# fakufaku/diffusion-separation

Hardware: AMD Instinct MI355X
Metric: separated utterances/sec (4 s, 8 kHz, 2-spk, N=30 PC steps) (higher is better)
Workload: dtype f16; 1 GPU; configs[1]: 2-spk N=30 PC sampler (+1 ald2 corrector step), batch=16 x 4.0 s @ 8 kHz per GPU and step, NCSN++ nf=64 random-init, 60 NFE/step; 4 consecutive steps (batches) in flight per GPU; batch_per_gpu=16, samples=32000, N=30, corrector_steps=1, nf=64, graph=True, batches_in_flight=4

## Files before the change

### diffusion-separation_amd/csrc/common.h

```cpp
#pragma once
#include <hip/hip_runtime.h>
#include <stdint.h>
#include <stdio.h>

#include <string>

typedef uint16_t bf16_t;
typedef __attribute__((ext_vector_type(16))) float f32x16;
typedef __attribute__((ext_vector_type(8))) __bf16 bf16x8;

#define DS_F32 0
#define DS_BF16 1
#define DS_F32_SPLIT 2
#define DS_MAX_SRC 4

void ds_set_error(const std::string& s);
#define DS_CHECK(cond, msg)                                                            \
  do {                                                                                 \
    if (!(cond)) {                                                                     \
      ds_set_error(std::string(__FILE__) + ":" + std::to_string(__LINE__) + ": " + (msg)); \
      return 1;                                                                        \
    }                                                                                  \
  } while (0)
#define DS_HIP(expr)                                                                   \
// ... 138 lines not shown
}
__device__ inline float wave_max(float v) {
#pragma unroll
  for (int o = 32; o > 0; o >>= 1) v = fmaxf(v, __shfl_xor(v, o, 64));
  return v;
}

static inline int cdiv(long a, long b) { return (int)((a + b - 1) / b); }

struct ConvArgs {
  const void* x; long x_bs; int ldx;
  const void* x2; long x2_bs; int ldx2;
  int C1;
  const void* w; long w_bs;
  int w_chunked;
  const void* w_frag; const void* sw_frag;
  const void* ident_frag;
  const void* sx; long sx_bs; int ldsx;
  const void* sx2; long sx2_bs; int ldsx2; int sC1; int sCin;
  const void* sw; int sw_chunked;
  const float* gn_scale;
  const float* gn_shift; int gn_act;
  const float* bias;
  const float* bias_b; int bias_b_ld;
  int bias_mode;
  const float* div_b;
  const void* res; long res_bs; int ldr;
  float out_scale;
  void* y; long y_bs; int ldy;
  long long* stats_acc;
  const long long* gn_acc1; const long long* gn_acc2; const float* gn_gamma; const float* gn_beta;
  int gn_groups; float gn_inv_count; float gn_eps;
  int B, H, W;
  int Cin, Cout, taps;
  int dtype;
  int split;
  unsigned opts;
};
#define DS_OPT_NO_RW 1u
#define DS_OPT_NO_RW128 2u
#define DS_OPT_RW_SMALL 4u
#define DS_OPT_NO_RW_RES 8u
#define DS_OPT_NO_ATTN_FUSED 64u
#define DS_OPT_NO_SPLIT256 128u
#define DS_OPT_NO_STFT_FUSED 256u
#define DS_OPT_RW_QUARTER 1024u
#define DS_OPT_RW_BIG_HALF 2048u
#define DS_OPT_RW_HALF 512u
#define DS_OPT_NO_SW 4096u
#define DS_OPT_NO_SW_RW 8192u
#define DS_OPT_NO_SW_ROWS4 32768u
#define DS_OPT_SW_ROWS4 65536u
#define DS_OPT_NO_SWS 16384u
#define DS_OPT_NO_WFRAG 32u
unsigned ds_default_opts();
int ds_num_cus();
enum { DS_CLS_CONV_N64 = 0, DS_CLS_CONV_N32, DS_CLS_CONV_8X8, DS_CLS_GEMM_N64, DS_CLS_GEMM_N32, DS_CLS_GEMM_8X8, DS_CLS_WS,
       DS_CLS_SMALL, DS_CLS_RW, DS_CLS_ATTN, DS_CLS_SW, DS_CLS_SWS, DS_NCLS };
enum class ConvRoute { GENERIC, WS, THIN_IN, THIN_OUT, SMALL, RW, SW, SWS };
struct ConvPlan {
  ConvRoute route;
  int cls;
  int tile;
  int sw_rows;
  bool rw_ok;
  bool skip_ok;
};
ConvPlan ds_conv_plan(const ConvArgs& a);
int ds_launch_conv(const ConvArgs& a, hipStream_t st);
int ds_launch_conv(const ConvArgs& a, const ConvPlan& p, hipStream_t st);
const char* ds_last_conv_kernel();
void ds_set_last_conv_kernel(const char* name);
int ds_conv_chunk(int taps, int dtype);
__host__ __device__ inline long ds_rw_frag_index(int co, int tap, int ch, int taps, int Cout) {
  return (((((long)(ch / 64) * taps + tap) * 4 + (ch % 64) / 16) * (Cout / 32) + co / 32) * 64 + ((ch % 16) / 8) * 32 + co % 32) * 8 + ch % 8;
}
inline bool ds_rw_frag_shape(int taps, int Cin, int Cout) {
  return (Cout == 64 || Cout == 128) && (Cin == 64 || Cin == 128) && (taps == 1 || !(Cout == 128 && Cin == 64));
}
bool ds_conv_rw_supported(const ConvArgs& a);
int ds_launch_conv_rw(const ConvArgs& a, hipStream_t st);
inline bool ds_sw_frag_shape(int taps, int Cin, int Cout) { return (Cout == 64 || Cout == 128 || Cout == 256) && Cin % 64 == 0 && Cin >= 64 && Cin <= 512; }
bool ds_conv_sw_supported(const ConvArgs& a);
int ds_launch_conv_sw(const ConvArgs& a, int rows, hipStream_t st);
__host__ __device__ inline long ds_sws_frag_index(int co, int tap, int ch, int taps, int Cout, int plane) {
  return ((((((long)(ch / 32) * taps + tap) * 2 + (ch % 32) / 16) * 2 + plane) * (Cout / 32) + co / 32) * 64 + ((ch % 16) / 8) * 32 + co % 32) * 8 + ch % 8;
}
inline bool ds_sws_frag_shape(int taps, int Cin, int Cout) { return (Cout == 64 || Cout == 128 || Cout == 256) && Cin % 64 == 0 && Cin >= 64 && Cin <= 256; }
bool ds_conv_sws_supported(const ConvArgs& a);
int ds_launch_conv_sws(const ConvArgs& a, hipStream_t st);
bool ds_conv_ws_supported(const ConvArgs& a);
int ds_launch_conv_ws(const ConvArgs& a, hipStream_t st);
bool ds_conv_thin_in_supported(const ConvArgs& a);
int ds_launch_conv_thin_in(const ConvArgs& a, hipStream_t st);
bool ds_conv_thin_out_supported(const ConvArgs& a);
int ds_launch_conv_thin_out(const ConvArgs& a, hipStream_t st);
bool ds_conv_small_supported(const ConvArgs& a);
int ds_launch_conv_small(const ConvArgs& a, hipStream_t st);

struct AttnFusedArgs {
  const void* x; long x_bs; int ldx;
  const long long* gn_acc; const float* gn_gamma; const float* gn_beta; int gn_groups; float gn_inv_count; float gn_eps;
  const float* gn_scale; const float* gn_shift;
  const void* wqk; const void* wv; const void* wo;
  const float* bqk; const float* bv; const float* bo;
  void* y; long y_bs; int ldy;
  long long* stats;
  int B, L, C;
};
bool ds_attn_fused_eligible(int dtype, int channels, int L);
int ds_launch_attn_fused(const AttnFusedArgs& a, hipStream_t st);

long ds_gn_workspace_bytes(int B, int H, int W, int C);
int ds_launch_gn_stats(const void* x, int ldx, const void* x2, int ldx2, int C1, int B, int H, int W, int C, int groups,
                       float eps, const float* gamma, const float* beta, void* ws, float* scale, float* shift,
                       int dtype, hipStream_t st);
int ds_launch_gn_finalize_acc(const long long* a1, int C1, const long long* a2, int C2, int B, long npix, int groups,
                              float eps, const float* gamma, const float* beta, float* scale, float* shift,
                              hipStream_t st);
enum class GnRoute { APPLY = 1, BLOCK2X2, DOWN_STRIP, DOWN_TILED, UP_TILED };
struct GnPlan { GnRoute route; int rs; };
bool ds_gn_route_runs(GnRoute r, int mode, bool affine, int dtype, int H, int W, int C, int ldx, int ldy, int ldxr, bool has_xr);
GnPlan ds_gn_route(int mode, bool affine, int dtype, int B, int H, int W, int C, int ldx, int ldy, int ldxr, bool has_xr, int cus);
const char* ds_gn_kernel_name(const GnPlan& p, int mode, bool affine, int dtype);
int ds_launch_gn_apply(const void* x, int ldx, const float* scale, const float* shift, int C, void* y, int ldy,
                       void* xr, int ldxr, int B, int H, int W, int act, int mode, int dtype, hipStream_t st);
int ds_launch_gn_apply(const GnPlan& p, const void* x, int ldx, const float* scale, const float* shift, int C, void* y, int ldy,
                       void* xr, int ldxr, int B, int H, int W, int act, int mode, int dtype, hipStream_t st);
int ds_launch_concat(const void* a, int lda, int Ca, const void* b, int ldb, int Cb, void* y, int ldy, long npix,
                     int dtype, hipStream_t st);
int ds_launch_softmax(const void* x, void* y, long rows, int L, int ld, int dtype, hipStream_t st);

long ds_stft_workspace_bytes(int B, int S, long T, int n_fft, int hop);
long ds_istft_workspace_bytes(int B, int S, long T, int n_fft, int hop);
int ds_launch_stft_pack(const float* xt, const float* mix, void* y, int B, int S, long T, int n_fft, int hop,
                        float exponent, float factor, int W, int Cpad, int shift, int dtype, const float* tab,
                        float* ws, hipStream_t st, int split = 0);
int ds_launch_istft(const void* x, float* out, int B, int S, long T, int n_fft, int hop, float exponent, float factor,
                    int W, int Cpad, int dtype, const float* tab, float* ws, hipStream_t st, int split = 0,
                    const float* ow = nullptr, const float* ob = nullptr, const float* tdiv = nullptr, int ow_cin = 0);
int ds_build_stft_table(int n_fft, float** dev_tab);

struct SdeP { int kind; int ndim; float d_lambda, sigma_min, sigma_max; };
__device__ inline float sde_g_of_t(const SdeP& s, float t) {
  const float r = s.sigma_max / s.sigma_min;
  return s.sigma_min * powf(r, t) * sqrtf(2.0f * logf(r));
}
__device__ inline void mix_eig(const SdeP& s, float t, float& ev1, float& ev2) {
  const float r = s.sigma_max / s.sigma_min;
  const float logsig = logf(r);
  const float mult = s.sigma_min * s.sigma_min;
  const float srp = powf(r, 2.0f * t);
  ev1 = mult * (srp - 1.0f);
  const float ex = expf(-2.0f * s.d_lambda * t);
  const float denom = 1.0f + s.d_lambda / logsig;
  ev2 = mult * (srp - ex) / denom;
}
__device__ inline void philox_round(uint32_t& c0, uint32_t& c1, uint32_t& c2, uint32_t& c3, uint32_t k0, uint32_t k1) {
  const uint64_t p0 = (uint64_t)0xD2511F53u * c0;
  const uint64_t p1 = (uint64_t)0xCD9E8D57u * c2;
  const uint32_t n0 = (uint32_t)(p1 >> 32) ^ c1 ^ k0;
  const uint32_t n1 = (uint32_t)p1;
  const uint32_t n2 = (uint32_t)(p0 >> 32) ^ c3 ^ k1;
  const uint32_t n3 = (uint32_t)p0;
  c0 = n0; c1 = n1; c2 = n2; c3 = n3;
}
__device__ inline void philox_randn4(uint64_t q, uint64_t seed, uint64_t sid, float* v) {
  uint32_t c0 = (uint32_t)q, c1 = (uint32_t)(q >> 32), c2 = (uint32_t)sid, c3 = (uint32_t)(sid >> 32);
  uint32_t k0 = (uint32_t)seed, k1 = (uint32_t)(seed >> 32);
#pragma unroll
  for (int r = 0; r < 10; ++r) {
    philox_round(c0, c1, c2, c3, k0, k1);
    k0 += 0x9E3779B9u;
    k1 += 0xBB67AE85u;
  }
  const float u0 = ((float)(c0 >> 8) + 0.5f) * (1.0f / 16777216.0f);
  const float u1 = ((float)(c1 >> 8) + 0.5f) * (1.0f / 16777216.0f);
  const float u2 = ((float)(c2 >> 8) + 0.5f) * (1.0f / 16777216.0f);
  const float u3 = ((float)(c3 >> 8) + 0.5f) * (1.0f / 16777216.0f);
  const float r0 = sqrtf(-2.0f * logf(u0)), r1 = sqrtf(-2.0f * logf(u2));
  sincosf(6.28318530718f * u1, &v[1], &v[0]);
// ... 62 lines not shown
```

### diffusion-separation_amd/csrc/engine.hip

```cpp
#include "engine_host.h"

static thread_local std::string g_err;
void ds_set_error(const std::string& s) { g_err = s; }
extern "C" const char* diffsep_last_error(void) { return g_err.c_str(); }
extern "C" const char* diffsep_version(void) {
#ifdef DS_HALF_F16
    return "diffsep-hip 0.3 (gfx950, 16-bit storage f16)";
#else
    return "diffsep-hip 0.3 (gfx950, 16-bit storage bf16)";
#endif
}

static const struct { const char* name; const char* env; unsigned bit; } kOpts[] = {
    {"no_rw", "DIFFSEP_NO_RW", DS_OPT_NO_RW},
    {"no_rw128", "DIFFSEP_NO_RW128", DS_OPT_NO_RW128},
    {"rw_small", "DIFFSEP_RW_SMALL", DS_OPT_RW_SMALL},
    {"no_rw_res", "DIFFSEP_NO_RW_RES", DS_OPT_NO_RW_RES},
    {"no_wfrag", nullptr, DS_OPT_NO_WFRAG},
    {"no_attn_fused", nullptr, DS_OPT_NO_ATTN_FUSED},
    {"no_stft_fused", "DIFFSEP_NO_STFT_FUSED", DS_OPT_NO_STFT_FUSED},
    {"rw_half", "DIFFSEP_RW_HALF", DS_OPT_RW_HALF},
    {"rw_quarter", "DIFFSEP_RW_QUARTER", DS_OPT_RW_QUARTER},
    {"rw_big_half", "DIFFSEP_RW_BIG_HALF", DS_OPT_RW_BIG_HALF},
    {"no_split256", nullptr, DS_OPT_NO_SPLIT256},
    {"no_sw", "DIFFSEP_NO_SW", DS_OPT_NO_SW},
    {"no_sws", "DIFFSEP_NO_SWS", DS_OPT_NO_SWS},
    {"no_sw_rows4", "DIFFSEP_NO_SW_ROWS4", DS_OPT_NO_SW_ROWS4},
    {"sw_rows4", nullptr, DS_OPT_SW_ROWS4},
    {"no_sw_rw", "DIFFSEP_NO_SW_RW", DS_OPT_NO_SW_RW}};
static std::atomic<unsigned> g_opts{0};
static std::once_flag g_opts_once;
unsigned ds_default_opts() {
  std::call_once(g_opts_once, [] {
    for (const auto& o : kOpts) {
      const char* v = o.env ? getenv(o.env) : nullptr;
      if (v && *v && strcmp(v, "0") != 0) g_opts |= o.bit;
    }
  });
  return g_opts;
}
int ds_num_cus() {
  static std::atomic<int> cus[32];
  int dev = 0;
  if (hipGetDevice(&dev) != hipSuccess || dev < 0 || dev >= 32) dev = 0;
  int c = cus[dev].load(std::memory_order_relaxed);
  if (c <= 0) {
    hipDeviceProp_t prop;
    c = hipGetDeviceProperties(&prop, dev) == hipSuccess ? prop.multiProcessorCount : 0;
    if (c <= 0) c = 256;
    cus[dev].store(c, std::memory_order_relaxed);
  }
  return c;
}
static int opt_bit(const char* name, unsigned* bit) {
  for (const auto& o : kOpts)
    if (!strcmp(name, o.name)) { *bit = o.bit; return 0; }
  return 1;
}
extern "C" int32_t diffsep_set_option(const char* name, int64_t value) {
  DS_CHECK(name, "set_option: null name");
  unsigned bit = 0;
  if (opt_bit(name, &bit)) { ds_set_error(std::string("set_option: unknown option '") + name + "'"); return 1; }
  ds_default_opts();
  if (value) g_opts.fetch_or(bit); else g_opts.fetch_and(~bit);
  return 0;
}

static Tn cat_view(const Tn& a, const Tn& b) {
  Tn t = a;
  t.C = a.C + b.C; t.C1 = a.C; t.p2 = b.p; t.ld2 = b.ld;
  t.sa2 = b.sa;
  return t;
}

static void* e_alloc(diffsep_engine* e, size_t bytes) {
  const size_t a = (e->top + 255) & ~(size_t)255;
  e->top = a + bytes;
  if (e->dry) return (void*)(uintptr_t)(a + 256);
  if (e->dbg_alloc) fprintf(stderr, "[diffsep alloc] %zu %zu\n", a, bytes);
  return e->arena + a;
}
static long long* e_alloc_stats(diffsep_engine* e, size_t bytes) {
// ... 90 lines not shown
  DS_CHECK(!a.sx || p.skip_ok, "internal: fused skip conv on an unsupported tile");
  if (c.want_stats && e->dbg_alloc && !e->dry)
    fprintf(stderr, "[diffsep stats] %ld Cin %d Cout %d taps %d HxW %dx%d res %d skip %d bias_b %d cfg %d\n",
            (long)((char*)y.sa - e->stats_ptr), a.Cin, c.Cout, c.taps, a.H, a.W, c.res != nullptr, c.skip != nullptr,
            c.bias_b != nullptr, p.cls);
  if (e->dry || ablated(e, a.H)) return 0;
  if (!e->prof) return ds_launch_conv(a, p, st);
  diffsep_engine::ProfRec r;
  r.flops = 2.0 * ((double)a.taps * a.Cin + (a.sx ? a.sCin : 0)) * a.Cout * (double)a.H * a.W * a.B;
  {
    const double esz = a.dtype == DS_F32 ? 4.0 : 2.0;
    r.bytes = esz * ((double)a.B * a.H * a.W *
                         ((double)a.Cin + a.Cout + (a.res ? a.Cout : 0) + (a.sx ? a.sCin : 0)) +
                     ((double)a.taps * a.Cin + (a.sx ? a.sCin : 0)) * a.Cout);
  }
  r.cls = p.cls;
  r.B = a.B; r.H = a.H; r.W = a.W; r.Cin = a.Cin; r.Cout = a.Cout; r.taps = a.taps; r.sCin = a.sx ? a.sCin : 0; r.res = a.res != nullptr;
  const int rc = prof_launch(e, st, r, [&]() { return ds_launch_conv(a, p, st); });
  e->prof_recs.back().kernel = ds_last_conv_kernel();
  return rc;
}

static int gn_stats(diffsep_engine* e, const Tn& x, const float* gamma, const float* beta, int B, GnAff& aff,
                    hipStream_t st, bool lazy = false) {
  const int groups = gn_group_count(x.C);
  aff = GnAff();
  const bool have_acc = x.sa && (!x.p2 || x.sa2);
  if (have_acc && lazy && x.C <= 512) {
    aff.acc1 = x.sa; aff.acc2 = x.sa2; aff.gamma = gamma; aff.beta = beta; aff.groups = groups;
    aff.inv_count = gn_inv_count((long)x.H * x.W, x.C, groups);
    return 0;
  }
  aff.scale = e_f32(e, (size_t)B * x.C);
  aff.shift = e_f32(e, (size_t)B * x.C);
  if (have_acc) {
    if (e->dry || (e->ablate & 16u)) return 0;
    return ds_launch_gn_finalize_acc(x.sa, x.p2 ? x.C1 : x.C, x.sa2, x.p2 ? x.C - x.C1 : 0, B, (long)x.H * x.W, groups,
                                     1e-6f, gamma, beta, aff.scale, aff.shift, st);
  }
  void* ws = e_alloc(e, (size_t)ds_gn_workspace_bytes(B, x.H, x.W, x.C));
  if (e->dry) return 0;
  return ds_launch_gn_stats(x.p, x.ld, x.p2, x.ld2, x.C1, B, x.H, x.W, x.C, groups, 1e-6f, gamma, beta, ws, aff.scale,
                            aff.shift, e->cfg.dtype, st);
}
static int gn_apply(diffsep_engine* e, const Tn& x, const GnAff* aff, const Tn* y, const Tn* xr, int B, int act,
                    int mode, hipStream_t st) {
  if (e->dry || (e->ablate & 8u)) return 0;
  const double esz = e->cfg.dtype == DS_F32 ? 4.0 : 2.0, nin = (double)B * x.H * x.W * x.C;
  const double fo = mode == 1 ? 4.0 : (mode == 2 ? 0.25 : 1.0);
  const double bytes = esz * nin * (1.0 + fo * ((y ? 1 : 0) + (xr ? 1 : 0)));
  const char* name = mode == 1 ? (aff ? "gn_fir_up (GroupNorm + SiLU + FIR x2 up of act and raw)" : "fir_up (pyramid)")
                               : (mode == 2 ? (aff ? "gn_fir_down (GroupNorm + SiLU + FIR x2 down of act and raw)" : "fir_down (pyramid)")
                                            : "gn_apply (GroupNorm affine + SiLU)");
  return prof_launch(e, st, hbm_rec(name, bytes, B, x.H, x.W, x.C), [&]() {
    return ds_launch_gn_apply(x.p, x.ld, aff ? aff->scale : nullptr, aff ? aff->shift : nullptr, x.C, y ? y->p : nullptr,
                              y ? y->ld : 0, xr ? xr->p : nullptr, xr ? xr->ld : 0, B, x.H, x.W, act, mode, e->cfg.dtype,
                              st);
  });
}

static const float kInvSqrt2 = 0.70710678118654752440f;

static int conv1_folded_skip(diffsep_engine* e, const Module& m, const Tn& h1, const Tn& skip_src, const GnAff& a1, Tn& out,
                             int B, hipStream_t st) {
  const SkipConv sk = {&skip_src, PK(e, m.pk2), weight_chunk(9, m.in_ch, m.in_c1, e->cfg.dtype), PKF(e, m.pf2)};
  Conv c(h1, PK(e, m.pk1), m.out_ch, 9);
  c.w_frag = PKF(e, m.pf1); c.gn = &a1; c.skip = &sk; c.scale = kInvSqrt2; c.want_stats = true;
  c.bias = P(e, m.conv1_b); c.bias_b = P(e, m.conv2_b);
  return conv(e, c, out, B, st);
}

int res_block(diffsep_engine* e, const Module& m, const Tn& x, const float* temb_proj, int B, Tn& out,
              hipStream_t st) {
  DS_CHECK(x.C == m.in_ch, "internal: resblock channel mismatch");
  const int mode = m.up ? 1 : (m.down ? 2 : 0);
  const int Ho = m.up ? 2 * x.H : (m.down ? x.H / 2 : x.H);
  const int Wo = m.up ? 2 * x.W : (m.down ? x.W / 2 : x.W);
  GnAff a0, a1;
  const float* temb = temb_proj + m.temb_off;
  if (e->cfg.dtype == DS_BF16 && mode == 0 && x.p2 && m.pf0a >= 0 && x.C1 == 128 && x.sa && x.sa2 &&
      x.H >= ((e->opts & DS_OPT_NO_SW) ? 128 : 256) && !(e->opts & (DS_OPT_NO_SPLIT256 | DS_OPT_NO_WFRAG))) {
    Tn xa = x, xb = x;
    xa.C = 128; xa.p2 = nullptr; xa.C1 = 0; xa.ld2 = 0; xa.sa2 = nullptr;
    xb.p = x.p2; xb.ld = x.ld2; xb.C = 128; xb.p2 = nullptr; xb.C1 = 0; xb.ld2 = 0; xb.sa = x.sa2; xb.sa2 = nullptr;
    GnAff ga, gb;
    ga.acc1 = xa.sa; ga.gamma = P(e, m.gn0_w); ga.beta = P(e, m.gn0_b);
    ga.groups = gn_group_count(x.C) / 2;
    ga.inv_count = gn_inv_count((long)x.H * x.W, x.C, gn_group_count(x.C));
    gb = ga; gb.acc1 = xb.sa; gb.gamma = ga.gamma + 128; gb.beta = ga.beta + 128;
    Conv c0a(xa, PK(e, m.pk0), m.out_ch, 9);
    c0a.w_frag = PKF(e, m.pf0a); c0a.gn = &ga; c0a.bias = P(e, m.conv0_b); c0a.bias_b = temb; c0a.bias_b_ld = e->arch.dense_total;
    Tn h1p; h1p.C = h1p.ld = m.out_ch; h1p.H = Ho; h1p.W = Wo;
    ConvArgs half = conv_args(e, c0a, h1p, B); half.opts &= ~DS_OPT_RW_SMALL;
    if (ds_conv_plan(half).rw_ok) {
      h1p = e_tensor(e, B, Ho, Wo, m.out_ch);
      Tn h1 = e_tensor(e, B, Ho, Wo, m.out_ch);
      const long half0 = 4L * 9 * m.out_ch * 32;
      if (conv(e, c0a, h1p, B, st)) return 1;
      Conv c0b(xb, PK(e, m.pk0 + half0), m.out_ch, 9);
      c0b.w_frag = PKF(e, m.pf0b); c0b.gn = &gb; c0b.res = &h1p; c0b.want_stats = true;
      if (conv(e, c0b, h1, B, st)) return 1;
      if (gn_stats(e, h1, P(e, m.gn1_w), P(e, m.gn1_b), B, a1, st, true)) return 1;
      out = e_tensor(e, B, Ho, Wo, m.out_ch);
      if (!(e->opts & DS_OPT_NO_SW) && m.pf2 >= 0) return conv1_folded_skip(e, m, h1, x, a1, out, B, st);
      Tn outp = e_tensor(e, B, Ho, Wo, m.out_ch);
      const SkipConv sk = {&xa, PK(e, m.pk2), weight_chunk(9, 128, 0, e->cfg.dtype), PKF(e, m.pf2a)};
      Conv c1(h1, PK(e, m.pk1), m.out_ch, 9);
      c1.w_frag = PKF(e, m.pf1); c1.gn = &a1; c1.skip = &sk; c1.bias = P(e, m.conv1_b); c1.bias_b = P(e, m.conv2_b);
      if (conv(e, c1, outp, B, st)) return 1;
      Conv c2b(xb, PK(e, m.pk2b), m.out_ch, 1);
      c2b.res = &outp; c2b.scale = kInvSqrt2; c2b.want_stats = true;
      return conv(e, c2b, out, B, st);
    }
  }
  if (gn_stats(e, x, P(e, m.gn0_w), P(e, m.gn0_b), B, a0, st, mode == 0)) return 1;
  Tn h1 = e_tensor(e, B, Ho, Wo, m.out_ch);
  Tn xr = x, h0m;
  if (mode) {
    DS_CHECK(x.p2 == nullptr, "internal: resampling block on a concat view");
    h0m = e_tensor(e, B, Ho, Wo, m.in_ch);
    xr = e_tensor(e, B, Ho, Wo, m.in_ch);
    if (gn_apply(e, x, &a0, &h0m, &xr, B, 1, mode, st)) return 1;
  }
  if (!m.has_conv2) DS_CHECK(xr.p2 == nullptr, "internal: identity skip on a concat view");
  Conv c0(mode ? h0m : x, PK(e, m.pk0), m.out_ch, 9);
  c0.w_frag = PKF(e, m.pf0); c0.gn = mode ? nullptr : &a0; c0.want_stats = true;
  c0.bias = P(e, m.conv0_b); c0.bias_b = temb; c0.bias_b_ld = e->arch.dense_total;
  if (conv(e, c0, h1, B, st)) return 1;
  if (gn_stats(e, h1, P(e, m.gn1_w), P(e, m.gn1_b), B, a1, st, true)) return 1;
  out = e_tensor(e, B, Ho, Wo, m.out_ch);
  if (m.has_conv2 && fuse_skip(m)) return conv1_folded_skip(e, m, h1, xr, a1, out, B, st);
  Tn skip = xr;
  if (m.has_conv2) {
    skip = e_tensor(e, B, Ho, Wo, m.out_ch);
    Conv c2(xr, PK(e, m.pk2), m.out_ch, 1);
    c2.bias = P(e, m.conv2_b);
    if (conv(e, c2, skip, B, st)) return 1;
  }
  Conv c1(h1, PK(e, m.pk1), m.out_ch, 9);
  c1.w_frag = PKF(e, m.pf1); c1.ident_frag = m.has_conv2 ? nullptr : PKF(e, m.pf_id);
  c1.gn = &a1; c1.bias = P(e, m.conv1_b); c1.res = &skip; c1.scale = kInvSqrt2; c1.want_stats = true;
  return conv(e, c1, out, B, st);
}

int attention_core(const Tn& q, const void* k, const void* vt, const Tn& o, int B, void* scores, void* probs, int dtype,
                   hipStream_t st, int split) {
  const int L = q.W, C = q.C, Lp = rup8(L);
  Tn s = q, p = q;
  s.p = scores; p.p = probs; s.ld = p.ld = Lp; p.C = Lp;
  ConvArgs a;
  memset(&a, 0, sizeof(a));
  a.dtype = dtype; a.split = split; a.B = B; a.taps = 1; a.bias_mode = 0;
  conv_input(a, q);
  a.w = k; a.w_bs = (long)L * C;
  conv_output(a, s);
  a.Cout = L;
  a.out_scale = 1.0f / sqrtf((float)C);
  if (ds_launch_conv(a, st)) return 1;
  if (ds_launch_softmax(scores, probs, (long)B * L, L, Lp, dtype, st)) return 1;
  conv_input(a, p);
  a.w = vt; a.w_bs = (long)C * Lp;
  conv_output(a, o);
  a.Cout = C;
  a.out_scale = 1.f;
  return ds_launch_conv(a, st);
}

int attn_block(diffsep_engine* e, const Module& m, const Tn& x, int B, Tn& out, hipStream_t st) {
// ... 19 lines not shown
    diffsep_engine::ProfRec r;
    r.flops = (double)B * (6.0 * L * C * C + 4.0 * (double)L * L * C);
    r.bytes = (double)e->esz * (2.0 * B * L * C + 3.0 * C * C);
    r.cls = DS_CLS_ATTN; r.B = B; r.H = x.H; r.W = x.W; r.Cin = C; r.Cout = C; r.taps = 1; r.res = 1;
    r.kernel = "attn_fused_kernel";
    return prof_launch(e, st, r, [&]() { return ds_launch_attn_fused(a, st); });
  }
  GnAff a0;
  if (gn_stats(e, x, P(e, m.gn0_w), P(e, m.gn0_b), B, a0, st)) return 1;
  Tn h = e_tensor(e, B, x.H, x.W, C);
  if (gn_apply(e, x, &a0, &h, nullptr, B, 0, 0, st)) return 1;
  Tn q = e_tensor(e, B, x.H, x.W, C), k = e_tensor(e, B, x.H, x.W, C);
  Conv cq(h, PK(e, m.pk_nin[0]), C, 1), ck(h, PK(e, m.pk_nin[1]), C, 1);
  cq.bias = P(e, m.nin_b[0]); ck.bias = P(e, m.nin_b[1]);
  if (conv(e, cq, q, B, st) || conv(e, ck, k, B, st)) return 1;
  void* vt = e_alloc(e, (size_t)B * C * Lp * e->esz);
  void* scores = e_alloc(e, (size_t)B * L * Lp * e->esz);
  void* probs = e_alloc(e, (size_t)B * L * Lp * e->esz);
  Tn o = e_tensor(e, B, x.H, x.W, C);
  out = e_tensor(e, B, x.H, x.W, C);
  if (!e->dry && !ablated(e, x.H)) {
    Tn wv, vtn;
    wv.p = const_cast<void*>(PK(e, m.pk_nin[2])); wv.C = wv.ld = C; wv.H = 1; wv.W = C;
    vtn.p = vt; vtn.ld = Lp; vtn.H = 1; vtn.W = C;
    ConvArgs a;
    memset(&a, 0, sizeof(a));
    a.dtype = e->cfg.dtype; a.split = e->split; a.B = B; a.taps = 1; a.out_scale = 1.f;
    conv_input(a, wv);
    a.x_bs = 0;
    a.w = h.p; a.w_bs = (long)L * C;
    a.bias = P(e, m.nin_b[2]); a.bias_mode = 1;
    conv_output(a, vtn);
    a.Cout = L;
    if (ds_launch_conv(a, st)) return 1;
    Tn qv = q, ov = o;
    qv.H = ov.H = 1; qv.W = ov.W = L;
    if (attention_core(qv, k.p, vt, ov, B, scores, probs, e->cfg.dtype, st, e->split)) return 1;
  }
  Conv co(o, PK(e, m.pk_nin[3]), C, 1);
  co.bias = P(e, m.nin_b[3]); co.res = &x; co.scale = kInvSqrt2; co.want_stats = true;
  return conv(e, co, out, B, st);
}

static int net_forward(diffsep_engine* e, const Tn& x0, const float* t, const Tn& y, int B, hipStream_t st,
                       Tn* pyr_out = nullptr) {
  const Arch& A = e->arch;
  const diffsep_model_config& c = e->cfg;
  const int nf = c.nf;
  size_t mi = 0;
  float* emb = e_f32(e, (size_t)B * 2 * nf);
  float* t1 = e_f32(e, (size_t)B * 4 * nf);
  float* temb = e_f32(e, (size_t)B * 4 * nf);
  float* proj = e_f32(e, (size_t)B * A.dense_total);
  const Module& mf = A.mods[mi++];
  const Module& l1 = A.mods[mi++];
  const Module& l2 = A.mods[mi++];
  if (!e->dry) {
    if (ds_launch_fourier(t, P(e, mf.w0), emb, B, nf, st)) return 1;
    if (ds_launch_linear(emb, P(e, l1.w0), P(e, l1.b0), t1, B, 2 * nf, 4 * nf, 0, st)) return 1;
    if (ds_launch_linear(t1, P(e, l2.w0), P(e, l2.b0), temb, B, 4 * nf, 4 * nf, 1, st)) return 1;
    if (ds_launch_linear_t(temb, e->d_dense_w, e->d_dense_b, proj, B, 4 * nf, A.dense_total, 1, st)) return 1;
  }
  const Module& cin = A.mods[mi++];
  std::vector<Tn> hs;
  {
    Tn h = e_tensor(e, B, x0.H, x0.W, nf);
    Conv ci(x0, PK(e, cin.pk0), nf, 9);
    ci.bias = P(e, cin.b0); ci.want_stats = true;
    if (conv(e, ci, h, B, st)) return 1;
    hs.push_back(h);
  }
  Tn pyr_in = x0;
  const int L = c.n_levels;
  Tn h;
  for (int i = 0; i < L; ++i) {
    for (int k = 0; k < c.num_res_blocks; ++k) {
      if (res_block(e, A.mods[mi++], hs.back(), proj, B, h, st)) return 1;
      if (h.H == c.attn_resolution) {
        DS_CHECK(mi < A.mods.size() && A.mods[mi].kind == MK_ATTN, "attention placement mismatch (image height)");
        Tn ha;
        if (attn_block(e, A.mods[mi++], h, B, ha, st)) return 1;
        h = ha;
      }
      hs.push_back(h);
    }
    if (i != L - 1) {
      if (res_block(e, A.mods[mi++], hs.back(), proj, B, h, st)) return 1;
      Tn pd = e_tensor(e, B, pyr_in.H / 2, pyr_in.W / 2, pyr_in.C);
      if (gn_apply(e, pyr_in, nullptr, nullptr, &pd, B, 0, 2, st)) return 1;
      pyr_in = pd;
      const Module& cm = A.mods[mi++];
      DS_CHECK(cm.kind == MK_COMBINE, "internal: expected Combine");
      Tn hc = e_tensor(e, B, h.H, h.W, h.C);
      Conv cc(pyr_in, PK(e, cm.pk0), h.C, 1);
      cc.bias = P(e, cm.b0); cc.res = &h; cc.want_stats = true;
      if (conv(e, cc, hc, B, st)) return 1;
      hs.push_back(hc);
    }
  }
  h = hs.back();
  Tn t2;
  if (res_block(e, A.mods[mi++], h, proj, B, t2, st)) return 1;
  if (attn_block(e, A.mods[mi++], t2, B, h, st)) return 1;
  if (res_block(e, A.mods[mi++], h, proj, B, t2, st)) return 1;
  h = t2;

  Tn pyramid;
  bool have_pyr = false;
  for (int i = L - 1; i >= 0; --i) {
    for (int k = 0; k < c.num_res_blocks + 1; ++k) {
      const Tn s = hs.back();
      hs.pop_back();
      const Tn cat = cat_view(h, s);
      Tn hn2;
      if (res_block(e, A.mods[mi++], cat, proj, B, hn2, st)) return 1;
      h = hn2;
    }
    if (h.H == c.attn_resolution) {
      DS_CHECK(mi < A.mods.size() && A.mods[mi].kind == MK_ATTN, "attention placement mismatch (image height)");
      Tn ha;
      if (attn_block(e, A.mods[mi++], h, B, ha, st)) return 1;
      h = ha;
    }
    const Module& g = A.mods[mi++];
    const Module& cv = A.mods[mi++];
    DS_CHECK(g.kind == MK_GN && cv.kind == MK_CONV3, "internal: expected pyramid GN + conv");
    hipStream_t sp = st;
    GnAff ga;
    if (gn_stats(e, h, P(e, g.w0), P(e, g.b0), B, ga, sp, true)) return 1;
    Tn pnew = e_tensor(e, B, h.H, h.W, A.cpad_in);
    Conv cp(h, PK(e, cv.pk0), A.chan_in, 9);
    cp.bias = P(e, cv.b0); cp.gn = &ga;
    Tn pu;
    if (have_pyr) {
      pu = e_tensor(e, B, h.H, h.W, A.cpad_in);
      if (gn_apply(e, pyramid, nullptr, nullptr, &pu, B, 0, 1, sp)) return 1;
      cp.res = &pu;
    }
    if (conv(e, cp, pnew, B, sp)) return 1;
    pyramid = pnew;
    have_pyr = true;
    if (i != 0) {
      Tn hu;
      if (res_block(e, A.mods[mi++], h, proj, B, hu, st)) return 1;
      h = hu;
    }
  }
  DS_CHECK(hs.empty() && mi == A.mods.size(), "internal: module walk did not consume all modules");
  if (pyr_out) { *pyr_out = pyramid; return 0; }
  Tn yy = y;
  Conv co(pyramid, PK(e, A.pk_out), A.chan_out, 1);
  co.bias = P(e, A.out_b); co.div_b = t;
  return conv(e, co, yy, B, st);
}

static int score_forward_impl(diffsep_engine* e, const float* xt, const float* t, const float* mix, float* out, int B,
                              long T, hipStream_t st) {
  const diffsep_model_config& c = e->cfg;
  const int W = diffsep_padded_frames(&c, T), H = c.n_fft / 2 + 1, S = c.num_sources;
  e->top = e->fwd_base;
  e->tracked.clear();
  if (stats_begin(e, st)) return 1;
  Tn x0 = e_tensor(e, B, H, W, e->arch.cpad_in);
  Tn y = e_tensor(e, B, H, W, e->arch.cpad_out);
  const int dft_split = e->split || c.dtype == DS_BF16;
  float* ws_f = (float*)e_alloc(e, (size_t)ds_stft_workspace_bytes(B, S, T, c.n_fft, c.hop));
  float* frames = (float*)e_alloc(e, (size_t)ds_istft_workspace_bytes(B, S, T, c.n_fft, c.hop));
  const double esz_t = c.dtype == DS_F32 ? 4.0 : 2.0;
  if (!e->dry && !(e->ablate & 128u))
    if (prof_launch(e, st, hbm_rec("stft (frame + real-DFT GEMM + compress / pack)",
                                   4.0 * B * (S + 1) * (double)T + esz_t * B * H * (double)W * e->arch.cpad_in, B, H, W, e->arch.cpad_in), [&]() {
          return ds_launch_stft_pack(xt, mix, x0.p, B, S, T, c.n_fft, c.hop, c.spec_abs_exponent, c.spec_factor, W,
                                     e->arch.cpad_in, 1, c.dtype, e->d_tab, ws_f, st, dft_split);
        }))
      return 1;
  Tn pyr;
  if (net_forward(e, x0, t, y, B, st, &pyr)) return 1;
  if (!e->dry && !(e->ablate & 128u))
    if (prof_launch(e, st, hbm_rec("istft (unpack / decompress + inverse-DFT GEMM + overlap-add)",
                                   esz_t * B * H * (double)W * pyr.ld + 4.0 * B * S * (double)T, B, H, W, pyr.ld), [&]() {
          return ds_launch_istft(pyr.p, out, B, S, T, c.n_fft, c.hop, c.spec_abs_exponent, c.spec_factor, W, pyr.ld, c.dtype,
                                 e->d_tab, frames, st, dft_split, P(e, e->arch.out_w), P(e, e->arch.out_b), t, e->arch.chan_in);
        }))
      return 1;
  return 0;
}

static void destroy_graph(diffsep_engine::GraphRec& r) {
  if (r.x) hipGraphExecDestroy(r.x);
  if (r.g) hipGraphDestroy(r.g);
  r.x = nullptr; r.g = nullptr;
}
static void drop_graph(diffsep_engine* e) {
  for (auto& kv : e->graphs) destroy_graph(kv.second);
  e->graphs.clear();
  e->cur_graph = nullptr;
}

static void layout_state(diffsep_engine* e, int B, long T) {
  const size_t nst = (size_t)B * e->cfg.num_sources * T;
  e->top = 0;
  e->st_x = (float*)e_alloc(e, nst * 4);
  e->st_xm = (float*)e_alloc(e, nst * 4);
  e->st_score = (float*)e_alloc(e, nst * 4);
  e->st_noise = (float*)e_alloc(e, nst * 4);
  e->st_t = (float*)e_alloc(e, (size_t)B * 4);
  e->st_mix = (float*)e_alloc(e, (size_t)B * T * 4);
  e->st_smix = (float*)e_alloc(e, (size_t)B * T * 4);
  e->st_ts = (float*)e_alloc(e, 4096 * (size_t)B * 4);
  e->st_lang = (float*)e_alloc(e, 16 * (size_t)B + 64);
  e->st_lens = (int*)e_alloc(e, (size_t)B * 4);
  e->st_seeds = (unsigned long long*)e_alloc(e, (size_t)B * 8);
}

int ensure_plan(diffsep_engine* e, int B, long T, hipStream_t st) {
  if (e->planB == B && e->planT == T && e->arena) return 0;
  DS_CHECK(B >= 1 && T >= 1, "empty batch or signal");
  e->cur_graph = nullptr;
  e->planB = -1;
  e->planT = -1;
  e->dry = true;
  layout_state(e, B, T);
  e->fwd_base = (e->top + 255) & ~(size_t)255;
  const int rc = score_forward_impl(e, nullptr, nullptr, nullptr, nullptr, B, T, st);
  e->dry = false;
  if (rc) return 1;
  const size_t need = e->top + e->stats_need + 8192;
  if (need > e->cap) {
    DS_HIP(hipStreamSynchronize(st));
    drop_graph(e);
    if (e->arena) DS_HIP(hipFree(e->arena));
    e->tracked.clear();
    e->arena = nullptr;
    e->cap = 0;
    const size_t grown = e->had_arena ? need + need / 4 : need;
    DS_HIP(hipMalloc((void**)&e->arena, grown));
    e->cap = grown;
    e->had_arena = true;
  }
  DS_HIP(hipMemsetAsync(e->arena, 0, e->cap, st));
  layout_state(e, B, T);
  e->planB = B;
  e->planT = T;
  {
    auto it = e->graphs.find(std::make_pair(B, T));
    if (it != e->graphs.end()) {
      e->cur_graph = &it->second;
      it->second.used = ++e->graph_tick;
    }
  }
  e->ts_dev.clear();
  e->warmed = true;
  return 0;
}

int run_nfe(diffsep_engine* e, int B, long T, hipStream_t st) {
  if (e->use_graph && e->warmed && !e->prof) {
    if (!e->cur_graph) {
      DS_HIP(hipStreamBeginCapture(st, hipStreamCaptureModeThreadLocal));
      const int rc = score_forward_impl(e, e->st_x, e->st_t, e->st_mix, e->st_score, B, T, st);
      diffsep_engine::GraphRec r{nullptr, nullptr, 0};
      const hipError_t ce = hipStreamEndCapture(st, &r.g);
      if (rc || ce != hipSuccess || !r.g) {
        destroy_graph(r);
        e->use_graph = 0;
        if (rc) return 1;
      } else {
        const hipError_t ie = hipGraphInstantiate(&r.x, r.g, nullptr, nullptr, 0);
        if (ie != hipSuccess) destroy_graph(r);
        DS_HIP(ie);
        if ((int)e->graphs.size() >= e->graph_cap) {
          const hipError_t se = hipDeviceSynchronize();
          if (se != hipSuccess) destroy_graph(r);
          DS_HIP(se);
          while ((int)e->graphs.size() >= e->graph_cap) {
            auto lru = e->graphs.begin();
            for (auto it = e->graphs.begin(); it != e->graphs.end(); ++it)
              if (it->second.used < lru->second.used) lru = it;
            destroy_graph(lru->second);
            e->graphs.erase(lru);
          }
        }
        r.used = ++e->graph_tick;
        e->cur_graph = &(e->graphs[std::make_pair(B, (long)T)] = r);
      }
    }
    if (e->cur_graph) {
      DS_HIP(hipGraphLaunch(e->cur_graph->x, st));
      return 0;
    }
  }
  const int rc = score_forward_impl(e, e->st_x, e->st_t, e->st_mix, e->st_score, B, T, st);
  e->warmed = true;
  return rc;
}

extern "C" int32_t diffsep_engine_create(const diffsep_model_config* cfg, const float* weights_host, int64_t n_floats,
                                         diffsep_engine** out) {
  DS_CHECK(cfg && weights_host && out, "engine_create: null argument");
  DS_CHECK(cfg->dtype == DS_F32 || cfg->dtype == DS_BF16 || cfg->dtype == DS_F32_SPLIT,
           "engine_create: dtype must be DIFFSEP_F32, DIFFSEP_BF16 or DIFFSEP_F32_SPLIT");
  std::unique_ptr<diffsep_engine> e(new diffsep_engine());
  e->cfg = *cfg;
  const DtypeSplit ds = split_dtype(cfg->dtype);
  e->cfg.dtype = ds.dtype; e->split = ds.split;
  if (build_arch(e->cfg, e->arch, e->cfg.dtype == DS_BF16 ? 1 : (e->split ? 2 : 0))) return 1;
  const Arch& A = e->arch;
  if (upload_weights(e.get(), weights_host, n_floats, "engine_create: weight blob")) return 1;
  e->weight_bytes = (int64_t)A.total * 4 + (int64_t)A.pack_total * e->esz + (int64_t)A.dense_total * (4 * cfg->nf + 1) * 4;
  if (ds_build_stft_table(cfg->n_fft, &e->d_tab)) return 1;
  if (const char* sv = getenv("DIFFSEP_DBG_ALLOC")) e->dbg_alloc = atoi(sv) != 0;
  e->opts = ds_default_opts();
  DS_HIP(hipEventCreateWithFlags(&e->ev_in, hipEventDisableTiming));
  DS_HIP(hipEventCreateWithFlags(&e->ev_out, hipEventDisableTiming));
  *out = e.release();
  return 0;
}

diffsep_engine::~diffsep_engine() {
  drop_graph(this);
  hipFree(d_blob); hipFree(d_pack); hipFree(d_dense_w); hipFree(d_dense_b); hipFree(d_attn_b); hipFree(d_tab);
  hipFree(arena); hipFree(ode_buf);
  if (own) hipStreamDestroy(own);
  if (ev_in) hipEventDestroy(ev_in);
  if (ev_out) hipEventDestroy(ev_out);
  for (auto& r : prof_recs) { hipEventDestroy(r.a); hipEventDestroy(r.b); }
  for (hipEvent_t v : ev_pool) hipEventDestroy(v);
}
extern "C" void diffsep_engine_destroy(diffsep_engine* e) { delete e; }
extern "C" int32_t diffsep_engine_reserve(diffsep_engine* e, int32_t B, int64_t T, void* stream) {
  DS_CHECK(e && B >= 1 && T >= 1, "reserve: bad argument");
  hipStream_t st = (hipStream_t)stream;
  if (ensure_plan(e, B, T, st)) return 1;
  DS_HIP(hipStreamSynchronize(st));
  return 0;
}
__global__ __launch_bounds__(256) void absmax_kernel(const void* __restrict__ p, long n, int f32, unsigned* __restrict__ out) {
  float m = 0.f;
  unsigned bad = 0;
  for (long i = (long)blockIdx.x * 256 + threadIdx.x; i < n; i += (long)gridDim.x * 256) {
    const float v = f32 ? reinterpret_cast<const float*>(p)[i] : h2f(reinterpret_cast<const bf16_t*>(p)[i]);
    if (v != v || fabsf(v) > 3.0e38f) ++bad; else m = fmaxf(m, fabsf(v));
  }
  atomicMax(out, __float_as_uint(m));
  if (bad) atomicAdd(out + 1, bad);
}
extern "C" int32_t diffsep_engine_debug_absmax(diffsep_engine* e, double* out, int32_t cap, int32_t* n) {
  DS_CHECK(e && n, "debug_absmax: null argument");
  *n = (int32_t)e->tracked.size();
  if (!out || cap <= 0) return 0;
  const int cnt = *n < cap ? *n : cap;
  unsigned* d = nullptr;
  DS_HIP(hipMalloc(&d, (size_t)cnt * 8 + 8));
  DS_HIP(hipMemset(d, 0, (size_t)cnt * 8 + 8));
  for (int i = 0; i < cnt; ++i) {
    const auto& t = e->tracked[i];
    long nb = (t.n + 255) / 256;
    if (nb > 1024) nb = 1024;
    hipLaunchKernelGGL(absmax_kernel, dim3((unsigned)nb), dim3(256), 0, nullptr, t.p, t.n, e->cfg.dtype == DS_F32 ? 1 : 0, d + 2 * i);
  }
  std::vector<unsigned> hbuf((size_t)cnt * 2);
  DS_HIP(hipDeviceSynchronize());
  DS_HIP(hipMemcpy(hbuf.data(), d, (size_t)cnt * 8, hipMemcpyDeviceToHost));
  hipFree(d);
  for (int i = 0; i < cnt; ++i) {
    float m;
    memcpy(&m, &hbuf[2 * i], 4);
    out[4 * i] = m; out[4 * i + 1] = hbuf[2 * i + 1]; out[4 * i + 2] = e->tracked[i].H; out[4 * i + 3] = e->tracked[i].C;
  }
  return 0;
}
extern "C" int32_t diffsep_engine_debug_arena(const diffsep_engine* e, void** base, int64_t* bytes, int64_t* fwd_base) {
  DS_CHECK(e && base && bytes && fwd_base, "debug_arena: null argument");
  *base = e->arena; *bytes = (int64_t)e->cap; *fwd_base = (int64_t)e->fwd_base;
  return 0;
}
extern "C" int64_t diffsep_engine_device_bytes(const diffsep_engine* e) {
  return e ? e->weight_bytes + (int64_t)e->cap + (int64_t)e->ode_cap : 0;
}
extern "C" int32_t diffsep_engine_set_graph(diffsep_engine* e, int32_t enable) {
  DS_CHECK(e, "null engine");
  e->use_graph = enable;
  if (!enable) drop_graph(e);
  return 0;
}

extern "C" int32_t diffsep_engine_set_option(diffsep_engine* e, const char* name, int64_t value) {
  DS_CHECK(e && name, "engine_set_option: null argument");
  unsigned bit = 0;
  if (!strcmp(name, "graph_cache")) {
    DS_CHECK(value >= 1 && value <= 4096, "engine_set_option: graph_cache must be in [1, 4096]");
    e->graph_cap = (int)value;
  } else if (!strcmp(name, "ablate")) {
    e->ablate = (unsigned)value;
  } else if (!strcmp(name, "dbg_alloc")) {
    e->dbg_alloc = value != 0;
    return 0;
  } else if (!strcmp(name, "no_stft_fused")) {
    ds_set_error("engine_set_option: 'no_stft_fused' is a process-level option (diffsep_set_option / DIFFSEP_NO_STFT_FUSED)");
    return 1;
  } else if (!strcmp(name, "track_tensors")) {
    e->track_tensors = value != 0;
    e->tracked.clear();
    return 0;
  } else if (!opt_bit(name, &bit)) {
    e->opts = value ? (e->opts | bit) : (e->opts & ~bit);
  } else {
    ds_set_error(std::string("engine_set_option: unknown option '") + name + "'");
    return 1;
  }
  DS_HIP(hipDeviceSynchronize());
  drop_graph(e);
  e->planB = -1;
  e->planT = -1;
  return 0;
}
extern "C" int64_t diffsep_engine_get_option(const diffsep_engine* e, const char* name) {
  if (!e || !name) return -1;
  unsigned bit = 0;
  if (!strcmp(name, "graph_cache")) return e->graph_cap;
  if (!strcmp(name, "graphs_cached")) return (int64_t)e->graphs.size();
  if (!strcmp(name, "ablate")) return e->ablate;
  if (!opt_bit(name, &bit)) return (e->opts & bit) ? 1 : 0;
  return -1;
}

extern "C" int32_t diffsep_engine_profile_begin(diffsep_engine* e) {
  DS_CHECK(e, "null engine");
  e->prof = true;
  e->prof_recs.clear();
  return 0;
}
static_assert(DS_NCLS == DIFFSEP_NUM_KERNEL_CLASSES, "header and engine agree on the number of kernel classes");
extern "C" int32_t diffsep_num_kernel_classes(void) { return DS_NCLS; }
extern "C" int32_t diffsep_engine_profile_end(diffsep_engine* e, double* flops, double* ms, int64_t* launches,
                                               double* bytes) {
  return diffsep_engine_profile_end_n(e, DS_NCLS, flops, ms, launches, bytes, nullptr);
}
extern "C" int32_t diffsep_engine_profile_end_n(diffsep_engine* e, int32_t n_classes, double* flops, double* ms,
                                                 int64_t* launches, double* bytes, int32_t* n_written) {
  DS_CHECK(e && flops && ms && launches && n_classes >= 0, "profile_end: null argument");
  DS_HIP(hipDeviceSynchronize());
  const int ncls = n_classes < DS_NCLS ? n_classes : DS_NCLS;
  if (n_written) *n_written = ncls;
  for (int i = 0; i < ncls; ++i) { flops[i] = 0; ms[i] = 0; launches[i] = 0; if (bytes) bytes[i] = 0; }
  e->prof_done.clear();
  for (auto& r : e->prof_recs) {
    float t = 0.f;
    hipEventElapsedTime(&t, r.a, r.b);
    r.ms = t;
    e->prof_done.push_back(r);
    if (r.cls >= 0 && r.cls < ncls) {
      flops[r.cls] += r.flops;
      if (bytes) bytes[r.cls] += r.bytes;
      ms[r.cls] += t;
      launches[r.cls] += 1;
    }
    e->ev_pool.push_back(r.a);
    e->ev_pool.push_back(r.b);
  }
  e->prof_recs.clear();
  e->prof = false;
  return 0;
}

extern "C" int32_t diffsep_engine_profile_records(diffsep_engine* e, diffsep_prof_record* out, int32_t cap, int32_t* n) {
  DS_CHECK(e && n, "profile_records: null argument");
  *n = (int32_t)e->prof_done.size();
  if (!out) return 0;
  for (int i = 0; i < *n && i < cap; ++i) {
    const auto& r = e->prof_done[i];
    diffsep_prof_record& o = out[i];
    memset(&o, 0, sizeof(o));
    snprintf(o.kernel, sizeof(o.kernel), "%s", r.kernel ? r.kernel : "");
    o.B = r.B; o.H = r.H; o.W = r.W; o.Cin = r.Cin; o.Cout = r.Cout; o.taps = r.taps; o.skip_cin = r.sCin; o.has_res = r.res;
// ... 38 lines not shown
```

### diffusion-separation_amd/csrc/engine_host.h

```cpp
#pragma once
#include <math.h>
#include <stdlib.h>
#include <string.h>

#include <atomic>
#include <map>
#include <memory>
#include <mutex>
#include <string>
#include <utility>
#include <vector>

#include "../../include/diffsep_hip.h"
#include "common.h"

#pragma GCC visibility push(hidden)

struct PRef { long off = -1; long numel = 0; };
struct ParamInfo { std::string name; int ndim; int64_t shape[4]; long off; };

enum ModKind { MK_FOURIER, MK_LINEAR, MK_CONV3, MK_RES, MK_ATTN, MK_COMBINE, MK_GN };

struct Module {
  ModKind kind;
// ... 172 lines not shown
}
static inline void conv_residual(ConvArgs& a, const Tn& r) { a.res = r.p; a.res_bs = image_bs(r, r.ld); a.ldr = r.ld; }
static inline void conv_output(ConvArgs& a, const Tn& y) { a.y = y.p; a.y_bs = image_bs(y, y.ld); a.ldy = y.ld; }

struct PinnedStage {
  char* p = nullptr;
  size_t cap = 0;
  hipEvent_t ev = nullptr;
  bool rec = false;
  PinnedStage() = default;
  PinnedStage(const PinnedStage&) = delete;
  ~PinnedStage() { if (ev) hipEventDestroy(ev); if (p) hipHostFree(p); }
  int wait() { if (rec) DS_HIP(hipEventSynchronize(ev)); return 0; }
  template <typename T>
  int acquire(size_t n, T** out) {
    if (wait()) return 1;
    if (n > cap) {
      if (p) DS_HIP(hipHostFree(p));
      p = nullptr;
      cap = 0;
      const size_t grown = n < 4096 ? 4096 : n;
      DS_HIP(hipHostMalloc((void**)&p, grown * sizeof(T), hipHostMallocDefault));
      cap = grown;
    }
    if (!ev) DS_HIP(hipEventCreateWithFlags(&ev, hipEventDisableTiming));
    *out = reinterpret_cast<T*>(p);
    return 0;
  }
  int record(hipStream_t st) { DS_HIP(hipEventRecord(ev, st)); rec = true; return 0; }
};

struct diffsep_engine {
  diffsep_engine() = default;
  diffsep_engine(const diffsep_engine&) = delete;
  ~diffsep_engine();
  diffsep_model_config cfg;
  Arch arch;
  int esz = 4;
  float* d_blob = nullptr;
  char* d_pack = nullptr;
  float* d_dense_w = nullptr;
  float* d_dense_b = nullptr;
  float* d_attn_b = nullptr;
  float* d_tab = nullptr;
  char* arena = nullptr;
  size_t cap = 0, top = 0, fwd_base = 0;
  size_t stats_need = 0, stats_used = 0;
  char* stats_ptr = nullptr;
  bool dry = false;
  int planB = -1;
  long planT = -1;
  float *st_x = nullptr, *st_xm = nullptr, *st_score = nullptr, *st_t = nullptr, *st_noise = nullptr,
        *st_ts = nullptr, *st_mix = nullptr, *st_smix = nullptr, *st_lang = nullptr;
  int* st_lens = nullptr;
  unsigned long long* st_seeds = nullptr;
  PinnedStage ext_pin;
  struct GraphRec { hipGraph_t g; hipGraphExec_t x; uint64_t used; };
  std::map<std::pair<int, long>, GraphRec> graphs;
  GraphRec* cur_graph = nullptr;
  int graph_cap = 12;
  uint64_t graph_tick = 0;
  int use_graph = 1;
  unsigned opts = 0;
  unsigned ablate = 0;
  bool warmed = false;
  int64_t weight_bytes = 0;
  hipStream_t own = nullptr;
  hipEvent_t ev_in = nullptr, ev_out = nullptr;
  PinnedStage ts_pin;
  std::vector<float> ts_dev;
  int ts_B = 0;
  bool had_arena = false;
  bool dbg_alloc = false;
  bool track_tensors = false;
  struct Tracked { void* p; long n; int H, W, C; };
  std::vector<Tracked> tracked;
  int split = 0;
  bool prof = false;
  struct ProfRec {
    hipEvent_t a = nullptr, b = nullptr; double flops = 0.0, bytes = 0.0; int cls = -1; const char* kernel = nullptr;
    int B = 0, H = 0, W = 0, Cin = 0, Cout = 0, taps = 0, sCin = 0, res = 0; float ms = 0.f;
  };
  std::vector<ProfRec> prof_done;
  std::vector<ProfRec> prof_recs;
  std::vector<hipEvent_t> ev_pool;
  char* ode_buf = nullptr;
  size_t ode_cap = 0;
  PinnedStage ode_pin;
};

static inline hipEvent_t prof_event(diffsep_engine* e) {
  if (!e->ev_pool.empty()) { hipEvent_t v = e->ev_pool.back(); e->ev_pool.pop_back(); return v; }
  hipEvent_t v = nullptr;
  hipEventCreate(&v);
  return v;
}
template <typename F>
static int prof_launch(diffsep_engine* e, hipStream_t st, diffsep_engine::ProfRec r, F&& body) {
  if (!e->prof) return body();
  r.a = prof_event(e); r.b = prof_event(e);
  hipEventRecord(r.a, st);
  const int rc = body();
  hipEventRecord(r.b, st);
  e->prof_recs.push_back(r);
  return rc;
}
static inline diffsep_engine::ProfRec hbm_rec(const char* name, double bytes, int B, int H, int W, int C) {
  diffsep_engine::ProfRec r;
  r.kernel = name; r.bytes = bytes; r.B = B; r.H = H; r.W = W; r.Cin = C;
  return r;
}

struct StreamScope {
  diffsep_engine* e; hipStream_t user; hipStream_t st;
  StreamScope(diffsep_engine* e_, void* s) : e(e_), user((hipStream_t)s), st((hipStream_t)s) {
    if (!user) {
      if (!e->own) hipStreamCreateWithFlags(&e->own, hipStreamNonBlocking);
      st = e->own;
      hipEventRecord(e->ev_in, nullptr);
      hipStreamWaitEvent(st, e->ev_in, 0);
    }
  }
  ~StreamScope() {
    if (!user) {
      hipEventRecord(e->ev_out, st);
      hipStreamWaitEvent(nullptr, e->ev_out, 0);
    }
  }
};

int upload_weights(diffsep_engine* e, const float* weights_host, int64_t n_floats, const char* what);
float* e_f32(diffsep_engine* e, size_t n);
int stats_begin(diffsep_engine* e, hipStream_t st);
int res_block(diffsep_engine* e, const Module& m, const Tn& x, const float* temb_proj, int B, Tn& out, hipStream_t st);
int attn_block(diffsep_engine* e, const Module& m, const Tn& x, int B, Tn& out, hipStream_t st);
int attention_core(const Tn& q, const void* k, const void* vt, const Tn& o, int B, void* scores, void* probs, int dtype,
                   hipStream_t st, int split = 0);
int ensure_plan(diffsep_engine* e, int B, long T, hipStream_t st);
int run_nfe(diffsep_engine* e, int B, long T, hipStream_t st);
int ds_launch_mask_tail(float* v, int B, int rows, long T, const int* lens, hipStream_t st);

#pragma GCC visibility pop
```

### diffusion-separation_amd/csrc/norm.hip

```cpp
#include <stdlib.h>

#include "conv_device.h"

template <typename T>
__global__ __launch_bounds__(256) void gn_stats_kernel(const T* __restrict__ x, int ldx, const T* __restrict__ x2,
                                                       int ldx2, int C1, long npix, int C, long ppb,
                                                       double* __restrict__ part) {
  __shared__ double sh[4096];
  const int ncg = C >> 3;
  const int npl = 256 / ncg;
  const int tid = threadIdx.x;
  const int cg = tid % ncg, pl = tid / ncg;
  const int b = blockIdx.y;
  const long p0 = (long)blockIdx.x * ppb;
  long p1 = p0 + ppb;
  if (p1 > npix) p1 = npix;
  double s[8], ss[8];
#pragma unroll
  for (int j = 0; j < 8; ++j) { s[j] = 0.0; ss[j] = 0.0; }
  if (pl < npl) {
    const bool second = x2 != nullptr && cg * 8 >= C1;
    const int ld = second ? ldx2 : ldx;
    const T* xb = second ? x2 + (long)b * npix * ldx2 + (cg * 8 - C1) : x + (long)b * npix * ldx + cg * 8;
    for (long p = p0 + pl; p < p1; p += npl) {
// ... 86 lines not shown
    if (var < 0.0) var = 0.0;
    const float sc = (float)(1.0 / sqrt(var + (double)eps)) * (gamma ? gamma[c] : 1.f);
    scale[(long)b * C + c] = sc;
    shift[(long)b * C + c] = (beta ? beta[c] : 0.f) - (float)mean * sc;
  }
}

int ds_launch_gn_finalize_acc(const long long* a1, int C1, const long long* a2, int C2, int B, long npix, int groups,
                              float eps, const float* gamma, const float* beta, float* scale, float* shift,
                              hipStream_t st) {
  const int C = C1 + C2;
  DS_CHECK(C % groups == 0 && groups > 0, "groupnorm(acc): bad group count");
  const double inv_count = (double)(float)(1.0 / ((double)npix * (double)(C / groups)));
  hipLaunchKernelGGL(gn_finalize_acc_kernel, dim3(B), dim3(256), 0, st, a1, C1, a2, C2, groups, inv_count, eps, gamma,
                     beta, scale, shift);
  DS_LAUNCH_CHECK();
  return 0;
}

long ds_gn_workspace_bytes(int B, int H, int W, int C) {
  const long npix = (long)H * W;
  long nblk = cdiv(npix, 64);
  if (nblk > 64) nblk = 64;
  return (long)B * nblk * C * 2 * 8 + 256;
}

int ds_launch_gn_stats(const void* x, int ldx, const void* x2, int ldx2, int C1, int B, int H, int W, int C, int groups,
                       float eps, const float* gamma, const float* beta, void* ws, float* scale, float* shift,
                       int dtype, hipStream_t st) {
  DS_CHECK(!x2 || (C1 % 8 == 0 && C1 > 0 && C1 < C), "groupnorm: bad concat split");
  DS_CHECK(C % 8 == 0 && C <= 1024 && C >= 8, "groupnorm: C must be a multiple of 8 in [8,1024]");
  DS_CHECK(groups > 0 && groups <= 256 && C % groups == 0, "groupnorm: bad group count");
  DS_CHECK((C >> 3) <= 256, "groupnorm: C too large");
  const long npix = (long)H * W;
  long nblk = cdiv(npix, 64);
  if (nblk > 64) nblk = 64;
  const long ppb = (npix + nblk - 1) / nblk;
  double* part = reinterpret_cast<double*>(ws);
  dim3 grid((unsigned)nblk, (unsigned)B);
  if (dtype == DS_F32)
    hipLaunchKernelGGL(gn_stats_kernel<float>, grid, dim3(256), 0, st, (const float*)x, ldx, (const float*)x2, ldx2,
                       C1, npix, C, ppb, part);
  else
    hipLaunchKernelGGL(gn_stats_kernel<bf16_t>, grid, dim3(256), 0, st, (const bf16_t*)x, ldx, (const bf16_t*)x2, ldx2,
                       C1, npix, C, ppb, part);
  DS_LAUNCH_CHECK();
  const double count = (double)npix * (double)(C / groups);
  hipLaunchKernelGGL(gn_finalize_kernel, dim3(B), dim3(256), 0, st, part, (int)nblk, C, groups, count, eps, gamma, beta,
                     scale, shift);
  DS_LAUNCH_CHECK();
  return 0;
}

template <typename T, int MODE, bool AFFINE>
__global__ __launch_bounds__(256) void gn_apply_kernel(const T* __restrict__ x, int ldx,
                                                       const float* __restrict__ scale,
                                                       const float* __restrict__ shift, int C, T* __restrict__ y,
                                                       int ldy, T* __restrict__ xr, int ldxr, int B, int H, int W,
                                                       int act) {
  const int Ho = MODE == 1 ? 2 * H : (MODE == 2 ? H / 2 : H);
  const int Wo = MODE == 1 ? 2 * W : (MODE == 2 ? W / 2 : W);
  const int ncg = C >> 3;
  const long total = (long)B * Ho * Wo * ncg;
  for (long i = (long)blockIdx.x * 256 + threadIdx.x; i < total; i += (long)gridDim.x * 256) {
    const int cg = (int)(i % ncg);
    long r = i / ncg;
    const int ox = (int)(r % Wo);
    r /= Wo;
    const int oy = (int)(r % Ho);
    const int b = (int)(r / Ho);
    float sc[8], sf[8];
    if (AFFINE) {
#pragma unroll
      for (int j = 0; j < 8; ++j) {
        sc[j] = scale[(long)b * C + cg * 8 + j];
        sf[j] = shift[(long)b * C + cg * 8 + j];
      }
    }
    const T* xb = x + (long)b * H * W * ldx + cg * 8;
    float ah[8], ax[8];
#pragma unroll
    for (int j = 0; j < 8; ++j) { ah[j] = 0.f; ax[j] = 0.f; }
    if (MODE == 0) {
      float f[8];
      load8<T>(xb + ((long)oy * W + ox) * ldx, f);
#pragma unroll
      for (int j = 0; j < 8; ++j) {
        float v = f[j] * sc[j] + sf[j];
        ah[j] = act ? silu_t<T>(v) : v;
      }
    } else {
      constexpr int NT = MODE == 2 ? 4 : 2;
      int iy0, ix0;
      float wy[4], wx[4];
      if (MODE == 2) {
        iy0 = 2 * oy - 1; ix0 = 2 * ox - 1;
        wy[0] = wx[0] = 0.125f; wy[1] = wx[1] = 0.375f; wy[2] = wx[2] = 0.375f; wy[3] = wx[3] = 0.125f;
      } else {
        const int ay = oy & 1, axp = ox & 1;
        iy0 = (oy >> 1) - 1 + ay; ix0 = (ox >> 1) - 1 + axp;
        wy[0] = ay ? 0.75f : 0.25f; wy[1] = ay ? 0.25f : 0.75f;
        wx[0] = axp ? 0.75f : 0.25f; wx[1] = axp ? 0.25f : 0.75f;
        wy[2] = wy[3] = wx[2] = wx[3] = 0.f;
      }
#pragma unroll
      for (int a = 0; a < NT; ++a) {
        const int iy = iy0 + a;
        if (iy < 0 || iy >= H) continue;
#pragma unroll
        for (int c = 0; c < NT; ++c) {
          const int ix = ix0 + c;
          if (ix < 0 || ix >= W) continue;
          const float wgt = wy[a] * wx[c];
          float f[8];
          load8<T>(xb + ((long)iy * W + ix) * ldx, f);
#pragma unroll
          for (int j = 0; j < 8; ++j) {
            ax[j] += wgt * f[j];
            if (AFFINE) {
              float v = f[j] * sc[j] + sf[j];
              v = act ? silu_t<T>(v) : v;
              ah[j] += wgt * v;
            }
          }
        }
      }
    }
    const long opix = ((long)b * Ho + oy) * Wo + ox;
    if (AFFINE) store8<T>(y + opix * ldy + cg * 8, ah);
    if (MODE != 0 && xr) store8<T>(xr + opix * ldxr + cg * 8, ax);
  }
}

template <typename T, int MODE>
__global__ __launch_bounds__(256) void gn_resample2x2_kernel(const T* __restrict__ x, int ldx,
                                                             const float* __restrict__ scale,
                                                             const float* __restrict__ shift, int C, T* __restrict__ y,
                                                             int ldy, T* __restrict__ xr, int ldxr, int B, int H, int W,
                                                             int act) {
  constexpr int NR = MODE == 1 ? 3 : 6;
  const int Hb = MODE == 1 ? H : H / 4, Wb = MODE == 1 ? W : W / 4;
  const int Ho = MODE == 1 ? 2 * H : H / 2, Wo = MODE == 1 ? 2 * W : W / 2;
  const int ncg = C >> 3;
  const long total = (long)B * Hb * Wb * ncg;
  for (long i = (long)blockIdx.x * 256 + threadIdx.x; i < total; i += (long)gridDim.x * 256) {
    const int cg = (int)(i % ncg);
    long r = i / ncg;
    const int bx = (int)(r % Wb);
    r /= Wb;
    const int by = (int)(r % Hb);
    const int b = (int)(r / Hb);
    float sc[8], sf[8];
#pragma unroll
    for (int j = 0; j < 8; ++j) {
      sc[j] = scale[(long)b * C + cg * 8 + j];
      sf[j] = shift[(long)b * C + cg * 8 + j];
    }
    const T* xb = x + (long)b * H * W * ldx + cg * 8;
    const int iy0 = MODE == 1 ? by - 1 : 4 * by - 1, ix0 = MODE == 1 ? bx - 1 : 4 * bx - 1;
    float oh[2][2][8], ox[2][2][8];
#pragma unroll
    for (int a = 0; a < 2; ++a)
#pragma unroll
      for (int c = 0; c < 2; ++c)
#pragma unroll
        for (int j = 0; j < 8; ++j) { oh[a][c][j] = 0.f; ox[a][c][j] = 0.f; }
#pragma unroll
    for (int ri = 0; ri < NR; ++ri) {
      const int iy = iy0 + ri;
      if (iy < 0 || iy >= H) continue;
      float hh[2][8], hx[2][8];
#pragma unroll
      for (int c = 0; c < 2; ++c)
#pragma unroll
        for (int j = 0; j < 8; ++j) { hh[c][j] = 0.f; hx[c][j] = 0.f; }
#pragma unroll
      for (int ci = 0; ci < NR; ++ci) {
        const int ix = ix0 + ci;
        const float w0 = MODE == 1 ? (ci == 0 ? 0.25f : (ci == 1 ? 0.75f : 0.f))
                                   : (ci == 0 || ci == 3 ? 0.125f : (ci == 1 || ci == 2 ? 0.375f : 0.f));
        const float w1 = MODE == 1 ? (ci == 1 ? 0.75f : (ci == 2 ? 0.25f : 0.f))
                                   : (ci == 2 || ci == 5 ? 0.125f : (ci == 3 || ci == 4 ? 0.375f : 0.f));
        if (ix < 0 || ix >= W) continue;
        float f[8];
        load8<T>(xb + ((long)iy * W + ix) * ldx, f);
#pragma unroll
        for (int j = 0; j < 8; ++j) {
          float v = f[j] * sc[j] + sf[j];
          v = act ? silu_t<T>(v) : v;
          if (w0 != 0.f) { hh[0][j] = fmaf(w0, v, hh[0][j]); hx[0][j] = fmaf(w0, f[j], hx[0][j]); }
          if (w1 != 0.f) { hh[1][j] = fmaf(w1, v, hh[1][j]); hx[1][j] = fmaf(w1, f[j], hx[1][j]); }
        }
      }
      const float v0 = MODE == 1 ? (ri == 0 ? 0.25f : (ri == 1 ? 0.75f : 0.f))
                                 : (ri == 0 || ri == 3 ? 0.125f : (ri == 1 || ri == 2 ? 0.375f : 0.f));
      const float v1 = MODE == 1 ? (ri == 1 ? 0.75f : (ri == 2 ? 0.25f : 0.f))
                                 : (ri == 2 || ri == 5 ? 0.125f : (ri == 3 || ri == 4 ? 0.375f : 0.f));
#pragma unroll
      for (int c = 0; c < 2; ++c)
#pragma unroll
        for (int j = 0; j < 8; ++j) {
          if (v0 != 0.f) { oh[0][c][j] = fmaf(v0, hh[c][j], oh[0][c][j]); ox[0][c][j] = fmaf(v0, hx[c][j], ox[0][c][j]); }
          if (v1 != 0.f) { oh[1][c][j] = fmaf(v1, hh[c][j], oh[1][c][j]); ox[1][c][j] = fmaf(v1, hx[c][j], ox[1][c][j]); }
        }
    }
#pragma unroll
    for (int a = 0; a < 2; ++a)
#pragma unroll
      for (int c = 0; c < 2; ++c) {
        const long opix = ((long)b * Ho + 2 * by + a) * Wo + 2 * bx + c;
        store8<T>(y + opix * ldy + cg * 8, oh[a][c]);
        if (xr) store8<T>(xr + opix * ldxr + cg * 8, ox[a][c]);
      }
  }
}


template <int RS>
__global__ __launch_bounds__(256) void gn_fir_down_strip_kernel(const bf16_t* __restrict__ x, int ldx,
                                                                const float* __restrict__ scale,
                                                                const float* __restrict__ shift, int C,
                                                                bf16_t* __restrict__ y, int ldy, bf16_t* __restrict__ xr,
                                                                int ldxr, int B, int H, int W, int act) {
  const int Ho = H / 2, Wo = W / 2, ncg = C >> 3, ntx = Wo / 2, nst = (Ho + RS - 1) / RS;
  const long total = (long)B * nst * ntx * ncg;
  const long i = (long)blockIdx.x * 256 + threadIdx.x;
  if (i >= total) return;
  const int cg = (int)(i % ncg);
  long r = i / ncg;
  const int tx = (int)(r % ntx);
  r /= ntx;
  const int st = (int)(r % nst), b = (int)(r / nst);
  float sc[8], sf[8];
  {
    const float4 s0 = *reinterpret_cast<const float4*>(scale + (long)b * C + cg * 8), s1 = *reinterpret_cast<const float4*>(scale + (long)b * C + cg * 8 + 4);
    const float4 h0 = *reinterpret_cast<const float4*>(shift + (long)b * C + cg * 8), h1 = *reinterpret_cast<const float4*>(shift + (long)b * C + cg * 8 + 4);
    sc[0] = s0.x; sc[1] = s0.y; sc[2] = s0.z; sc[3] = s0.w; sc[4] = s1.x; sc[5] = s1.y; sc[6] = s1.z; sc[7] = s1.w;
    sf[0] = h0.x; sf[1] = h0.y; sf[2] = h0.z; sf[3] = h0.w; sf[4] = h1.x; sf[5] = h1.y; sf[6] = h1.z; sf[7] = h1.w;
  }
  const bf16_t* xb = x + (long)b * H * W * ldx + cg * 8;
  const int ix0 = 4 * tx - 1, oy0 = st * RS, iy0 = 2 * oy0 - 1;
  bool cok[6];
#pragma unroll
  for (int c = 0; c < 6; ++c) cok[c] = ix0 + c >= 0 && ix0 + c < W;
  auto load_row = [&](int iy, uint4 (&raw)[6]) __attribute__((always_inline)) {
    const bool rok = iy >= 0 && iy < H;
#pragma unroll
    for (int c = 0; c < 6; ++c)
      raw[c] = (rok && cok[c]) ? *reinterpret_cast<const uint4*>(xb + ((long)iy * W + ix0 + c) * ldx) : make_uint4(0, 0, 0, 0);
  };
  auto hrow = [&](int iy, const uint4 (&raw)[6], float (&ha)[2][8], float (&hx)[2][8]) __attribute__((always_inline)) {
    const bool rok = iy >= 0 && iy < H;
#pragma unroll
    for (int q = 0; q < 2; ++q)
#pragma unroll
      for (int j = 0; j < 8; ++j) { ha[q][j] = 0.f; hx[q][j] = 0.f; }
#pragma unroll
    for (int c = 0; c < 6; ++c) {
      float f[8];
      f[0] = h_lo(raw[c].x); f[1] = h_hi(raw[c].x); f[2] = h_lo(raw[c].y); f[3] = h_hi(raw[c].y);
      f[4] = h_lo(raw[c].z); f[5] = h_hi(raw[c].z); f[6] = h_lo(raw[c].w); f[7] = h_hi(raw[c].w);
      const bool ok = rok && cok[c];
      const float w0 = c == 0 || c == 3 ? 0.125f : (c == 1 || c == 2 ? 0.375f : 0.f);
      const float w1 = c == 2 || c == 5 ? 0.125f : (c == 3 || c == 4 ? 0.375f : 0.f);
#pragma unroll
      for (int j = 0; j < 8; ++j) {
        float v = fmaf(f[j], sc[j], sf[j]);
        v = act ? silu_t<bf16_t>(v) : v;
        v = ok ? v : 0.f;
        if (w0 != 0.f) { ha[0][j] = fmaf(w0, v, ha[0][j]); hx[0][j] = fmaf(w0, f[j], hx[0][j]); }
        if (w1 != 0.f) { ha[1][j] = fmaf(w1, v, ha[1][j]); hx[1][j] = fmaf(w1, f[j], hx[1][j]); }
      }
    }
  };
  float pa[2][8], px[2][8], qa[2][8], qx[2][8];
#pragma unroll
  for (int q = 0; q < 2; ++q)
#pragma unroll
    for (int j = 0; j < 8; ++j) { pa[q][j] = 0.f; px[q][j] = 0.f; qa[q][j] = 0.f; qx[q][j] = 0.f; }
  uint4 cur[6], nxt[6];
  load_row(iy0, cur);
#pragma unroll
  for (int k = 0; k < 2 * RS + 2; ++k) {
    if (k + 1 < 2 * RS + 2) load_row(iy0 + k + 1, nxt);
    float ha[2][8], hx[2][8];
    hrow(iy0 + k, cur, ha, hx);
    const float wq = (k & 1) ? 0.375f : 0.125f, wp = (k & 1) ? 0.125f : 0.375f;
#pragma unroll
    for (int q = 0; q < 2; ++q)
#pragma unroll
      for (int j = 0; j < 8; ++j) {
        qa[q][j] = (k & 1) ? fmaf(wq, ha[q][j], qa[q][j]) : wq * ha[q][j];
        qx[q][j] = (k & 1) ? fmaf(wq, hx[q][j], qx[q][j]) : wq * hx[q][j];
        pa[q][j] = fmaf(wp, ha[q][j], pa[q][j]);
        px[q][j] = fmaf(wp, hx[q][j], px[q][j]);
      }
    if (k & 1) {
      const int oy = oy0 + (k >> 1) - 1;
      if (k >= 3 && oy < Ho) {
#pragma unroll
        for (int q = 0; q < 2; ++q) {
          const long opix = ((long)b * Ho + oy) * Wo + 2 * tx + q;
          store8<bf16_t>(y + opix * ldy + cg * 8, pa[q]);
          if (xr) store8<bf16_t>(xr + opix * ldxr + cg * 8, px[q]);
        }
      }
#pragma unroll
      for (int q = 0; q < 2; ++q)
#pragma unroll
        for (int j = 0; j < 8; ++j) { pa[q][j] = qa[q][j]; px[q][j] = qx[q][j]; }
    }
#pragma unroll
    for (int c = 0; c < 6; ++c) cur[c] = nxt[c];
  }
}

#ifdef DS_HALF_F16
#ifndef FD_MINW
#define FD_MINW 1
#endif
template <int RS>
__global__ __launch_bounds__(256, FD_MINW) void gn_fir_down_tiled_kernel(const bf16_t* __restrict__ x, int ldx,
                                                                const float* __restrict__ scale,
                                                                const float* __restrict__ shift, int C,
                                                                bf16_t* __restrict__ y, int ldy, bf16_t* __restrict__ xr,
                                                                int ldxr, int B, int H, int W, int act, int tiles_x, int strips) {
  constexpr int CP = 144, NCOL = 34, TB = NCOL * CP;
  __shared__ __attribute__((aligned(16))) char sm[2][2][TB];
  const int tid = threadIdx.x, cg = tid & 7, col = tid >> 3;
  const int ncgb = C >> 6;
  int bid = blockIdx.x;
  const int cgb = bid % ncgb; bid /= ncgb;
  const int tx = bid % tiles_x; bid /= tiles_x;
  const int st = bid % strips;
  const int b = bid / strips;
  const int ch0 = cgb * 64 + cg * 8;
  const int Ho = H >> 1, Wo = W >> 1;
  float sc[8], sf[8];
  {
    const float4 s0 = *reinterpret_cast<const float4*>(scale + (long)b * C + ch0), s1 = *reinterpret_cast<const float4*>(scale + (long)b * C + ch0 + 4);
    const float4 h0 = *reinterpret_cast<const float4*>(shift + (long)b * C + ch0), h1 = *reinterpret_cast<const float4*>(shift + (long)b * C + ch0 + 4);
    sc[0] = s0.x; sc[1] = s0.y; sc[2] = s0.z; sc[3] = s0.w; sc[4] = s1.x; sc[5] = s1.y; sc[6] = s1.z; sc[7] = s1.w;
    sf[0] = h0.x; sf[1] = h0.y; sf[2] = h0.z; sf[3] = h0.w; sf[4] = h1.x; sf[5] = h1.y; sf[6] = h1.z; sf[7] = h1.w;
  }
  const bf16_t* xb = x + (long)b * H * W * ldx + ch0;
  const int ix = 32 * tx + col;
  const bool halo = tid < 16;
  const int hix = 32 * tx + (tid < 8 ? -1 : 32);
  const bool hok = halo && hix >= 0 && hix < W;
  const int iy0 = 2 * st * RS - 1;
  constexpr int NR = 2 * RS + 2;
  auto load_row = [&](int iy, uint4& v, uint4& hv) __attribute__((always_inline)) {
    const bool rok = iy >= 0 && iy < H;
    v = rok ? *reinterpret_cast<const uint4*>(xb + ((long)iy * W + ix) * ldx) : make_uint4(0, 0, 0, 0);
    hv = (rok && hok) ? *reinterpret_cast<const uint4*>(xb + ((long)iy * W + hix) * ldx) : make_uint4(0, 0, 0, 0);
  };
  auto silu2 = [&](unsigned w, int d) __attribute__((always_inline)) {
    float z0 = fmaf(h_lo(w), sc[2 * d], sf[2 * d]), z1 = fmaf(h_hi(w), sc[2 * d + 1], sf[2 * d + 1]);
    if (act) { z0 = silu_t<bf16_t>(z0); z1 = silu_t<bf16_t>(z1); }
    return pack_h2(z0, z1);
  };
  auto activate = [&](const uint4& v, bool ok) __attribute__((always_inline)) {
    uint4 a;
    a.x = silu2(v.x, 0); a.y = silu2(v.y, 1); a.z = silu2(v.z, 2); a.w = silu2(v.w, 3);
    if (!ok) a = make_uint4(0, 0, 0, 0);
    return a;
  };
  const int tensor = tid >> 7, ocol = (tid >> 3) & 15;
  bf16_t* const out = tensor ? xr : y;
  const int ldo = tensor ? ldxr : ldy;
  float P[8], Q[8];
#pragma unroll
  for (int j = 0; j < 8; ++j) { P[j] = 0.f; Q[j] = 0.f; }
  auto do_row = [&](int k, const uint4& cur, const uint4& hcur, bool odd) __attribute__((always_inline)) {
    const int iy = iy0 + k;
    const bool rok = iy >= 0 && iy < H;
    char* rowb = &sm[odd][0][0];
    {
      const uint4 a = activate(cur, rok);
      *reinterpret_cast<uint4*>(rowb + (col + 1) * CP + cg * 16) = a;
      *reinterpret_cast<uint4*>(rowb + TB + (col + 1) * CP + cg * 16) = cur;
      if (halo) {
        const uint4 ha = activate(hcur, rok && hok);
        const int hc = tid < 8 ? 0 : NCOL - 1;
        *reinterpret_cast<uint4*>(rowb + hc * CP + cg * 16) = ha;
        *reinterpret_cast<uint4*>(rowb + TB + hc * CP + cg * 16) = hcur;
      }
    }
    __syncthreads();
    {
      const char* src = rowb + tensor * TB + (2 * ocol) * CP + cg * 16;
      float hsum[8];
#pragma unroll
      for (int j = 0; j < 8; ++j) hsum[j] = 0.f;
#pragma unroll
      for (int t = 0; t < 4; ++t) {
        const uint4 v = *reinterpret_cast<const uint4*>(src + t * CP);
        const float w = (t == 0 || t == 3) ? 0.125f : 0.375f;
        hsum[0] = fmaf(w, h_lo(v.x), hsum[0]); hsum[1] = fmaf(w, h_hi(v.x), hsum[1]);
        hsum[2] = fmaf(w, h_lo(v.y), hsum[2]); hsum[3] = fmaf(w, h_hi(v.y), hsum[3]);
        hsum[4] = fmaf(w, h_lo(v.z), hsum[4]); hsum[5] = fmaf(w, h_hi(v.z), hsum[5]);
        hsum[6] = fmaf(w, h_lo(v.w), hsum[6]); hsum[7] = fmaf(w, h_hi(v.w), hsum[7]);
      }
      const float wq = odd ? 0.375f : 0.125f, wp = odd ? 0.125f : 0.375f;
#pragma unroll
      for (int j = 0; j < 8; ++j) {
        Q[j] = odd ? fmaf(wq, hsum[j], Q[j]) : wq * hsum[j];
        P[j] = fmaf(wp, hsum[j], P[j]);
      }
      if (odd) {
        const int oy = st * RS + (k >> 1) - 1;
        if (k >= 3 && oy < Ho && out) {
          const long opix = ((long)b * Ho + oy) * Wo + 16 * tx + ocol;
          store8<bf16_t>(out + opix * ldo + ch0, P);
        }
#pragma unroll
        for (int j = 0; j < 8; ++j) P[j] = Q[j];
      }
    }
  };
  uint4 r0, r1, r2, r3, h0, h1, h2, h3;
  load_row(iy0, r0, h0);
  load_row(iy0 + 1, r1, h1);
  load_row(iy0 + 2, r2, h2);
  for (int k = 0; k < NR; k += 4) {
    if (k + 3 < NR) load_row(iy0 + k + 3, r3, h3);
    do_row(k, r0, h0, false);
    if (k + 1 >= NR) break;
    if (k + 4 < NR) load_row(iy0 + k + 4, r0, h0);
    do_row(k + 1, r1, h1, true);
    if (k + 2 >= NR) break;
    if (k + 5 < NR) load_row(iy0 + k + 5, r1, h1);
    do_row(k + 2, r2, h2, false);
    if (k + 3 >= NR) break;
    if (k + 6 < NR) load_row(iy0 + k + 6, r2, h2);
    do_row(k + 3, r3, h3, true);
  }
}
#endif

#ifndef UP_MINW
#define UP_MINW 1
#endif
template <typename T>
__global__ __launch_bounds__(256, UP_MINW) void gn_resample_up_tiled_kernel(const T* __restrict__ x, int ldx,
                                                                   const float* __restrict__ scale,
                                                                   const float* __restrict__ shift, int C,
                                                                   T* __restrict__ y, int ldy, T* __restrict__ xr,
                                                                   int ldxr, int B, int H, int W, int act, int tiles_x,
                                                                   int tiles_y) {
  constexpr int TH_ = 4, TW_ = 8, CG = 8;
  constexpr int IH = TH_ + 2, IW = TW_ + 2;
  constexpr int RAWB = 8 * (int)sizeof(T);
  constexpr int PITCH = 32 + RAWB;
  extern __shared__ __attribute__((aligned(16))) char sm[];
  const int tid = threadIdx.x;
  const int ncgb = (C >> 3) / CG;
  int bid = blockIdx.x;
  const int cgb = bid % ncgb; bid /= ncgb;
  const int tx = bid % tiles_x; bid /= tiles_x;
  const int ty = bid % tiles_y;
  const int b = bid / tiles_y;
  const int cg = tid & 7;
  const int ch0 = (cgb * CG + cg) * 8;
  float sc[8], sf[8];
#pragma unroll
  for (int j = 0; j < 8; ++j) {
    sc[j] = scale[(long)b * C + ch0 + j];
    sf[j] = shift[(long)b * C + ch0 + j];
  }
  const int iy0 = ty * TH_ - 1, ix0 = tx * TW_ - 1;
  const T* xb = x + (long)b * H * W * ldx + ch0;
  for (int i = tid; i < IH * IW * CG; i += 256) {
    const int pix = i >> 3;
    const int r = pix / IW, c = pix - r * IW;
    const int iy = iy0 + r, ix = ix0 + c;
    char* dst = sm + (pix * CG + cg) * PITCH;
    float v[8];
    if (iy >= 0 && iy < H && ix >= 0 && ix < W) {
      const T* src = xb + ((long)iy * W + ix) * ldx;
      float f[8];
      load8<T>(src, f);
#pragma unroll
      for (int j = 0; j < 8; ++j) {
        const float u = f[j] * sc[j] + sf[j];
        v[j] = act ? silu_t<T>(u) : u;
      }
      *reinterpret_cast<uint4*>(dst + 32) = reinterpret_cast<const uint4*>(src)[0];
      if (sizeof(T) == 4) *reinterpret_cast<uint4*>(dst + 48) = reinterpret_cast<const uint4*>(src)[1];
    } else {
#pragma unroll
      for (int j = 0; j < 8; ++j) v[j] = 0.f;
      *reinterpret_cast<uint4*>(dst + 32) = make_uint4(0, 0, 0, 0);
      if (sizeof(T) == 4) *reinterpret_cast<uint4*>(dst + 48) = make_uint4(0, 0, 0, 0);
    }
    *reinterpret_cast<float4*>(dst) = make_float4(v[0], v[1], v[2], v[3]);
    *reinterpret_cast<float4*>(dst + 16) = make_float4(v[4], v[5], v[6], v[7]);
  }
  __syncthreads();
  const int p = tid >> 3, py = p / TW_, px = p - py * TW_;
  const int iy = ty * TH_ + py, ix = tx * TW_ + px;
  if (iy >= H || ix >= W) return;
  float oh[2][2][8], ox[2][2][8];
#pragma unroll
  for (int a = 0; a < 2; ++a)
#pragma unroll
    for (int c = 0; c < 2; ++c)
#pragma unroll
      for (int j = 0; j < 8; ++j) { oh[a][c][j] = 0.f; ox[a][c][j] = 0.f; }
#pragma unroll
  for (int ri = 0; ri < 3; ++ri) {
    float hh[2][8], hx[2][8];
#pragma unroll
    for (int c = 0; c < 2; ++c)
#pragma unroll
      for (int j = 0; j < 8; ++j) { hh[c][j] = 0.f; hx[c][j] = 0.f; }
#pragma unroll
    for (int ci = 0; ci < 3; ++ci) {
      const float w0 = ci == 0 ? 0.25f : (ci == 1 ? 0.75f : 0.f), w1 = ci == 1 ? 0.75f : (ci == 2 ? 0.25f : 0.f);
      const char* src = sm + (((py + ri) * IW + px + ci) * CG + cg) * PITCH;
      const float4 a0 = *reinterpret_cast<const float4*>(src), a1 = *reinterpret_cast<const float4*>(src + 16);
      const float a[8] = {a0.x, a0.y, a0.z, a0.w, a1.x, a1.y, a1.z, a1.w};
      float f[8];
      load8<T>(reinterpret_cast<const T*>(src + 32), f);
#pragma unroll
      for (int j = 0; j < 8; ++j) {
        if (w0 != 0.f) { hh[0][j] = fmaf(w0, a[j], hh[0][j]); hx[0][j] = fmaf(w0, f[j], hx[0][j]); }
        if (w1 != 0.f) { hh[1][j] = fmaf(w1, a[j], hh[1][j]); hx[1][j] = fmaf(w1, f[j], hx[1][j]); }
      }
    }
    const float v0 = ri == 0 ? 0.25f : (ri == 1 ? 0.75f : 0.f), v1 = ri == 1 ? 0.75f : (ri == 2 ? 0.25f : 0.f);
#pragma unroll
    for (int c = 0; c < 2; ++c)
#pragma unroll
      for (int j = 0; j < 8; ++j) {
        if (v0 != 0.f) { oh[0][c][j] = fmaf(v0, hh[c][j], oh[0][c][j]); ox[0][c][j] = fmaf(v0, hx[c][j], ox[0][c][j]); }
        if (v1 != 0.f) { oh[1][c][j] = fmaf(v1, hh[c][j], oh[1][c][j]); ox[1][c][j] = fmaf(v1, hx[c][j], ox[1][c][j]); }
      }
  }
  const int Ho = 2 * H, Wo = 2 * W;
#pragma unroll
  for (int a = 0; a < 2; ++a)
#pragma unroll
    for (int c = 0; c < 2; ++c) {
      const long opix = ((long)b * Ho + 2 * iy + a) * Wo + 2 * ix + c;
      store8<T>(y + opix * ldy + ch0, oh[a][c]);
      if (xr) store8<T>(xr + opix * ldxr + ch0, ox[a][c]);
    }
}

template <typename T>
static constexpr int gn_resample_up_tiled_lds() { return 6 * 10 * 8 * (32 + 8 * (int)sizeof(T)); }

bool ds_gn_route_runs(GnRoute r, int mode, bool aff, int dtype, int H, int W, int C, int ldx, int ldy, int ldxr, bool has_xr) {
  const bool h16 = dtype != DS_F32;
  switch (r) {
    case GnRoute::APPLY: return true;
    case GnRoute::BLOCK2X2: return aff && (mode == 1 || (mode == 2 && H % 4 == 0 && W % 4 == 0));
    case GnRoute::DOWN_STRIP: return h16 && aff && mode == 2 && H % 2 == 0 && W % 4 == 0;
    case GnRoute::DOWN_TILED:
#if defined(DS_HALF_F16) && !defined(DS_NO_FIR_TILED)
      return h16 && aff && mode == 2 && H % 2 == 0 && W % 32 == 0 && C % 64 == 0 && ldx % 8 == 0 && ldy % 8 == 0 && (!has_xr || ldxr % 8 == 0);
#else
      return false;
#endif
    case GnRoute::UP_TILED: return aff && mode == 1 && C % 64 == 0;
  }
  return false;
}

#ifndef FD_RS_MAX
#define FD_RS_MAX 8
#endif

GnPlan ds_gn_route(int mode, bool aff, int dtype, int B, int H, int W, int C, int ldx, int ldy, int ldxr, bool has_xr, int cus) {
  const long tot2 = (mode == 1 ? (long)B * H * W : (long)B * (H / 4) * (W / 4)) * (C >> 3);
  auto runs = [&](GnRoute r) { return ds_gn_route_runs(r, mode, aff, dtype, H, W, C, ldx, ldy, ldxr, has_xr); };
  if (runs(GnRoute::UP_TILED) && tot2 >= 262144) return {GnRoute::UP_TILED, 0};
  if (dtype != DS_F32) {
    if (runs(GnRoute::DOWN_TILED) && (long)B * H * W * C >= (1l << 21)) {
      const int Ho_ = H / 2, tiles_x = W / 32, ncgb = C / 64;
      if (cus <= 0) cus = ds_num_cus();
      int rs = FD_RS_MAX;
      while (rs > 4 && (long)B * tiles_x * cdiv(Ho_, rs) * ncgb < 2 * cus) rs >>= 1;
      return {GnRoute::DOWN_TILED, rs};
    }
    if (runs(GnRoute::DOWN_STRIP) && tot2 >= 131072) {
      const long per_row = (long)B * (W / 4) * (C >> 3);
      return {GnRoute::DOWN_STRIP, per_row * cdiv(H / 2, 8) >= 131072 ? 8 : 4};
    }
  }
  if (runs(GnRoute::BLOCK2X2) && (mode == 1 || tot2 >= 131072)) return {GnRoute::BLOCK2X2, 0};
  return {GnRoute::APPLY, 0};
}

const char* ds_gn_kernel_name(const GnPlan& p, int mode, bool aff, int dtype) {
  const bool f32 = dtype == DS_F32;
  switch (p.route) {
    case GnRoute::UP_TILED: return f32 ? "gn_resample_up_tiled_kernel<f32>" : "gn_resample_up_tiled_kernel<" DS_HALF_NAME ">";
    case GnRoute::DOWN_TILED: return p.rs == 16 ? "gn_fir_down_tiled_kernel<16>" : (p.rs == 8 ? "gn_fir_down_tiled_kernel<8>" : "gn_fir_down_tiled_kernel<4>");
    case GnRoute::DOWN_STRIP: return p.rs == 8 ? "gn_fir_down_strip_kernel<8>" : "gn_fir_down_strip_kernel<4>";
    case GnRoute::BLOCK2X2:
      if (mode == 1) return f32 ? "gn_resample2x2_kernel<f32,1>" : "gn_resample2x2_kernel<" DS_HALF_NAME ",1>";
      return f32 ? "gn_resample2x2_kernel<f32,2>" : "gn_resample2x2_kernel<" DS_HALF_NAME ",2>";
    case GnRoute::APPLY:
      if (mode == 0) return aff ? "gn_apply_kernel<0,affine>" : "gn_apply_kernel<0,raw>";
      if (mode == 1) return aff ? "gn_apply_kernel<1,affine>" : "gn_apply_kernel<1,raw>";
      return aff ? "gn_apply_kernel<2,affine>" : "gn_apply_kernel<2,raw>";
  }
  return "";
}

template <typename T>
static int gn_launch_typed(const GnPlan& p, const void* x, int ldx, const float* scale, const float* shift, int C, void* y, int ldy,
                           void* xr, int ldxr, int B, int H, int W, int act, int mode, hipStream_t st) {
  const int Ho = mode == 1 ? 2 * H : (mode == 2 ? H / 2 : H);
  const int Wo = mode == 1 ? 2 * W : (mode == 2 ? W / 2 : W);
  const long total = (long)B * Ho * Wo * (C >> 3);
  long nb = (total + 255) / 256;
  if (nb > 16384) nb = 16384;
  if (nb < 1) nb = 1;
  const bool aff = scale != nullptr;
  const long tot2 = (mode == 1 ? (long)B * H * W : (long)B * (H / 4) * (W / 4)) * (C >> 3);
  if (p.route == GnRoute::UP_TILED) {
    const int th = cdiv(H, 4), tw = cdiv(W, 8);
    const long nblk = (long)B * th * tw * (C / 64);
    DS_FUNC_LDS_ONCE((gn_resample_up_tiled_kernel<T>), gn_resample_up_tiled_lds<T>());
    hipLaunchKernelGGL((gn_resample_up_tiled_kernel<T>), dim3((unsigned)nblk), dim3(256), gn_resample_up_tiled_lds<T>(), st,
                       (const T*)x, ldx, scale, shift, C, (T*)y, ldy, (T*)xr, ldxr, B, H, W, act, tw, th);
    DS_LAUNCH_CHECK();
    ds_set_last_conv_kernel(sizeof(T) == 4 ? "gn_resample_up_tiled_kernel<f32>" : "gn_resample_up_tiled_kernel<" DS_HALF_NAME ">");
    return 0;
  }
  if constexpr (sizeof(T) == 2) {
#if defined(DS_HALF_F16) && !defined(DS_NO_FIR_TILED)
    if (p.route == GnRoute::DOWN_TILED) {
      const int Ho_ = H / 2, tiles_x = W / 32, ncgb = C / 64, rs = p.rs;
      const int strips = cdiv(Ho_, rs);
      const unsigned nblk = (unsigned)((long)B * tiles_x * strips * ncgb);
#define FD(RS_)                                                                                                                          \
  do {                                                                                                                                   \
    hipLaunchKernelGGL((gn_fir_down_tiled_kernel<RS_>), dim3(nblk), dim3(256), 0, st, (const bf16_t*)x, ldx, scale, shift, C, (bf16_t*)y, \
                       ldy, (bf16_t*)xr, ldxr, B, H, W, act, tiles_x, strips);                                                           \
    ds_set_last_conv_kernel("gn_fir_down_tiled_kernel<" #RS_ ">");                                                                       \
  } while (0)
      if (rs == 16) FD(16); else if (rs == 8) FD(8); else FD(4);
#undef FD
      DS_LAUNCH_CHECK();
      return 0;
    }
#endif
    if (p.route == GnRoute::DOWN_STRIP) {
      const long per_row = (long)B * (W / 4) * (C >> 3);
      if (p.rs == 8) {
        constexpr int RS = 8;
        const long tot3 = per_row * cdiv(H / 2, RS);
        hipLaunchKernelGGL((gn_fir_down_strip_kernel<RS>), dim3((unsigned)cdiv(tot3, 256)), dim3(256), 0, st, (const bf16_t*)x, ldx, scale,
                           shift, C, (bf16_t*)y, ldy, (bf16_t*)xr, ldxr, B, H, W, act);
        ds_set_last_conv_kernel("gn_fir_down_strip_kernel<8>");
      } else {
        constexpr int RS = 4;
        const long tot3 = per_row * cdiv(H / 2, RS);
        hipLaunchKernelGGL((gn_fir_down_strip_kernel<RS>), dim3((unsigned)cdiv(tot3, 256)), dim3(256), 0, st, (const bf16_t*)x, ldx, scale,
                           shift, C, (bf16_t*)y, ldy, (bf16_t*)xr, ldxr, B, H, W, act);
        ds_set_last_conv_kernel("gn_fir_down_strip_kernel<4>");
      }
      DS_LAUNCH_CHECK();
      return 0;
    }
  }
  DS_CHECK(p.route == GnRoute::BLOCK2X2 || p.route == GnRoute::APPLY, "gn_apply: internal: route without a kernel for this type");
  if (p.route == GnRoute::BLOCK2X2) {
    long nb2 = (tot2 + 255) / 256;
    if (nb2 > 16384) nb2 = 16384;
    if (nb2 < 1) nb2 = 1;
    if (mode == 1) {
      hipLaunchKernelGGL((gn_resample2x2_kernel<T, 1>), dim3((unsigned)nb2), dim3(256), 0, st, (const T*)x, ldx, scale,
                         shift, C, (T*)y, ldy, (T*)xr, ldxr, B, H, W, act);
      ds_set_last_conv_kernel(sizeof(T) == 4 ? "gn_resample2x2_kernel<f32,1>" : "gn_resample2x2_kernel<" DS_HALF_NAME ",1>");
    } else {
      hipLaunchKernelGGL((gn_resample2x2_kernel<T, 2>), dim3((unsigned)nb2), dim3(256), 0, st, (const T*)x, ldx, scale,
                         shift, C, (T*)y, ldy, (T*)xr, ldxr, B, H, W, act);
      ds_set_last_conv_kernel(sizeof(T) == 4 ? "gn_resample2x2_kernel<f32,2>" : "gn_resample2x2_kernel<" DS_HALF_NAME ",2>");
    }
    DS_LAUNCH_CHECK();
    return 0;
  }
#define GA(M, A, N)                                                                                                  \
  do {                                                                                                               \
    hipLaunchKernelGGL((gn_apply_kernel<T, M, A>), dim3((unsigned)nb), dim3(256), 0, st, (const T*)x, ldx, scale, shift, \
                       C, (T*)y, ldy, (T*)xr, ldxr, B, H, W, act);                                                   \
    ds_set_last_conv_kernel("gn_apply_kernel<" #M "," N ">");                                                        \
  } while (0)
  if (mode == 0) { if (aff) GA(0, true, "affine"); else GA(0, false, "raw"); }
  else if (mode == 1) { if (aff) GA(1, true, "affine"); else GA(1, false, "raw"); }
  else { if (aff) GA(2, true, "affine"); else GA(2, false, "raw"); }
#undef GA
  DS_LAUNCH_CHECK();
  return 0;
}

int ds_launch_gn_apply(const GnPlan& p, const void* x, int ldx, const float* scale, const float* shift, int C, void* y, int ldy,
                       void* xr, int ldxr, int B, int H, int W, int act, int mode, int dtype, hipStream_t st) {
  DS_CHECK(C % 8 == 0, "gn_apply: C must be a multiple of 8");
  DS_CHECK(mode >= 0 && mode <= 2, "gn_apply: bad resample mode");
  DS_CHECK(mode != 2 || (H % 2 == 0 && W % 2 == 0), "gn_apply: FIR down needs even H, W");
  DS_CHECK(scale != nullptr || (mode != 0 && xr != nullptr), "gn_apply: nothing to do");
  DS_CHECK(ds_gn_route_runs(p.route, mode, scale != nullptr, dtype, H, W, C, ldx, ldy, ldxr, xr != nullptr),
           "gn_apply: the routed kernel cannot run this shape");
  if (dtype == DS_F32) return gn_launch_typed<float>(p, x, ldx, scale, shift, C, y, ldy, xr, ldxr, B, H, W, act, mode, st);
  return gn_launch_typed<bf16_t>(p, x, ldx, scale, shift, C, y, ldy, xr, ldxr, B, H, W, act, mode, st);
}

int ds_launch_gn_apply(const void* x, int ldx, const float* scale, const float* shift, int C, void* y, int ldy,
                       void* xr, int ldxr, int B, int H, int W, int act, int mode, int dtype, hipStream_t st) {
  const GnPlan p = ds_gn_route(mode, scale != nullptr, dtype, B, H, W, C, ldx, ldy, ldxr, xr != nullptr,  0);
  return ds_launch_gn_apply(p, x, ldx, scale, shift, C, y, ldy, xr, ldxr, B, H, W, act, mode, dtype, st);
}

template <typename T>
__global__ __launch_bounds__(256) void concat_kernel(const T* __restrict__ a, int lda, int Ca, const T* __restrict__ b,
                                                     int ldb, int Cb, T* __restrict__ y, int ldy, long npix) {
  const int ncg = (Ca + Cb) >> 3, nca = Ca >> 3;
  const long total = npix * ncg;
  for (long i = (long)blockIdx.x * 256 + threadIdx.x; i < total; i += (long)gridDim.x * 256) {
    const int cg = (int)(i % ncg);
    const long p = i / ncg;
    const T* src = cg < nca ? a + p * lda + cg * 8 : b + p * ldb + (cg - nca) * 8;
    T* dst = y + p * ldy + cg * 8;
    if (sizeof(T) == 4) {
      reinterpret_cast<uint4*>(dst)[0] = reinterpret_cast<const uint4*>(src)[0];
      reinterpret_cast<uint4*>(dst)[1] = reinterpret_cast<const uint4*>(src)[1];
    } else {
      reinterpret_cast<uint4*>(dst)[0] = reinterpret_cast<const uint4*>(src)[0];
    }
  }
}

int ds_launch_concat(const void* a, int lda, int Ca, const void* b, int ldb, int Cb, void* y, int ldy, long npix,
                     int dtype, hipStream_t st) {
  DS_CHECK(Ca % 8 == 0 && Cb % 8 == 0, "concat: channels must be multiples of 8");
  const long total = npix * ((Ca + Cb) >> 3);
  long nb = (total + 255) / 256;
  if (nb > 16384) nb = 16384;
  if (nb < 1) nb = 1;
  if (dtype == DS_F32)
    hipLaunchKernelGGL(concat_kernel<float>, dim3((unsigned)nb), dim3(256), 0, st, (const float*)a, lda, Ca,
                       (const float*)b, ldb, Cb, (float*)y, ldy, npix);
  else
    hipLaunchKernelGGL(concat_kernel<bf16_t>, dim3((unsigned)nb), dim3(256), 0, st, (const bf16_t*)a, lda, Ca,
                       (const bf16_t*)b, ldb, Cb, (bf16_t*)y, ldy, npix);
  DS_LAUNCH_CHECK();
  return 0;
}

template <typename T>
__global__ __launch_bounds__(256) void softmax_kernel(const T* __restrict__ x, T* __restrict__ y, long rows, int L,
                                                      int ld) {
  const int lane = threadIdx.x & 63;
  const long row = (long)blockIdx.x * 4 + (threadIdx.x >> 6);
  if (row >= rows) return;
  const T* xr = x + row * ld;
  T* yr = y + row * ld;
  float mx = -INFINITY;
  for (int j = lane; j < L; j += 64) mx = fmaxf(mx, Elt<T>::ld(xr + j));
  mx = wave_max(mx);
  float sum = 0.f;
  for (int j = lane; j < L; j += 64) sum += exp_t<T>(Elt<T>::ld(xr + j) - mx);
  sum = wave_sum(sum);
  const float inv = 1.0f / sum;
// ... 18 lines not shown
```

### diffusion-separation_amd/csrc/sampler.hip

```cpp
#include "engine_host.h"

static void linspace_f32(float start, float end, int n, float* out) {
  if (n == 1) { out[0] = start; return; }
  const float step = (end - start) / (float)(n - 1);
  const int half = n / 2;
  for (int i = 0; i < n; ++i) out[i] = (i < half) ? (start + step * (float)i) : (end - step * (float)(n - 1 - i));
}

__global__ __launch_bounds__(256) void mask_tail_kernel(float* __restrict__ v, int rows, long T,
                                                        const int* __restrict__ lens) {
  const long t = (long)blockIdx.x * 256 + threadIdx.x;
  const int b = blockIdx.y;
  if (t >= T || t < lens[b]) return;
  for (int r = 0; r < rows; ++r) v[((long)b * rows + r) * T + t] = 0.f;
}

int ds_launch_mask_tail(float* v, int B, int rows, long T, const int* lens, hipStream_t st) {
  hipLaunchKernelGGL(mask_tail_kernel, dim3(cdiv(T, 256), B), dim3(256), 0, st, v, rows, T, lens);
  DS_LAUNCH_CHECK();
  return 0;
}

static int check_sde(const diffsep_engine* e, const diffsep_sde_config* sde, const char* who) {
  const std::string w(who);
// ... 18 lines not shown
  if (check_sde(e, sde, "pc_sample")) return 1;
  DS_CHECK(smp->N >= 1 && smp->N <= 4096, "pc_sample: N must be in [1,4096]");
  DS_CHECK(smp->predictor == DIFFSEP_PRED_REVERSE_DIFFUSION || smp->predictor == DIFFSEP_PRED_EULER_MARUYAMA ||
               smp->predictor == DIFFSEP_PRED_NONE,
           "pc_sample: predictor must be reverse_diffusion, euler_maruyama or none");
  DS_CHECK(smp->corrector == DIFFSEP_CORR_ALD2 || smp->corrector == DIFFSEP_CORR_NONE ||
               smp->corrector == DIFFSEP_CORR_ALD || smp->corrector == DIFFSEP_CORR_LANGEVIN,
           "pc_sample: corrector must be ald2, ald, langevin or none");
  DS_CHECK(smp->corrector != DIFFSEP_CORR_ALD || sde->kind == DIFFSEP_SDE_MIX,
           "pc_sample: the 'ald' corrector supports MixSDE only (sdes/correctors.py:64-67)");
  const int64_t* lengths = ext ? ext->lengths_host : nullptr;
  const uint64_t* seeds = ext ? ext->seeds_host : nullptr;
  diffsep_engine* tail = (ext && (ext->tail_steps > 0 || ext->head_steps > 0)) ? ext->tail_engine : nullptr;
  const int tail_steps = tail ? ext->tail_steps : 0;
  const int head_steps = tail ? ext->head_steps : 0;
  if (tail) {
    DS_CHECK(tail != e, "pc_sample: the tail engine must be a different engine");
    diffsep_model_config a = e->cfg, b2 = tail->cfg;
    a.dtype = b2.dtype = 0;
    DS_CHECK(memcmp(&a, &b2, sizeof(a)) == 0, "pc_sample: the tail engine must have the same architecture");
  }
  DS_CHECK(!lengths || smp->corrector != DIFFSEP_CORR_LANGEVIN,
           "pc_sample: the 'langevin' corrector couples the batch entries; it cannot run on a mixed-length batch");
  DS_CHECK(!seeds || !noise, "pc_sample: per-utterance seeds are for device noise (noise == NULL)");
  if (lengths) {
    const int Wp = diffsep_padded_frames(&e->cfg, T);
    for (int b = 0; b < B; ++b) {
      DS_CHECK(lengths[b] >= 1 && lengths[b] <= T, "pc_sample: utterance length outside [1, T]");
      DS_CHECK(diffsep_padded_frames(&e->cfg, lengths[b]) == Wp,
               "pc_sample: every utterance of a mixed-length batch must have the padded frame count of T");
    }
  }
  StreamScope sc_(e, stream);
  hipStream_t st = sc_.st;
  const int S = e->cfg.num_sources, N = smp->N;
  const int csteps = smp->corrector == DIFFSEP_CORR_NONE ? 0 : smp->corrector_steps;
  if (ensure_plan(e, B, T, st)) return 1;
  if (tail && ensure_plan(tail, B, T, st)) return 1;
  const size_t nst = (size_t)B * S * T;
  const SdeP sp = to_sdep(sde);
  std::vector<float> ts(N);
  if (timesteps_host) for (int i = 0; i < N; ++i) ts[i] = timesteps_host[i];
  else linspace_f32(1.0f, smp->eps, N, ts.data());
  if (e->ts_dev != ts || e->ts_B != B) {
    const size_t nrow = (size_t)N * B;
    float* pin;
    if (e->ts_pin.acquire(nrow, &pin)) return 1;
    for (int i = 0; i < N; ++i) for (int b = 0; b < B; ++b) pin[(size_t)i * B + b] = ts[i];
    DS_HIP(hipMemcpyAsync(e->st_ts, pin, nrow * 4, hipMemcpyHostToDevice, st));
    if (e->ts_pin.record(st)) return 1;
    e->ts_dev = ts;
    e->ts_B = B;
  }
  DS_HIP(hipMemcpyAsync(e->st_mix, mix_norm, (size_t)B * T * 4, hipMemcpyDeviceToDevice, st));
  const int* lens = nullptr;
  if (lengths || seeds) {
    char* pin;
    if (e->ext_pin.acquire((size_t)B * 16, &pin)) return 1;
    unsigned long long* ps = reinterpret_cast<unsigned long long*>(pin);
    int* pl = reinterpret_cast<int*>(pin + (size_t)B * 8);
    for (int b = 0; b < B; ++b) {
      ps[b] = seeds ? seeds[b] : seed + 0x9E3779B97F4A7C15ull * (unsigned long long)b;
      pl[b] = lengths ? (int)lengths[b] : (int)T;
    }
    DS_HIP(hipMemcpyAsync(e->st_seeds, ps, (size_t)B * 8, hipMemcpyHostToDevice, st));
    DS_HIP(hipMemcpyAsync(e->st_lens, pl, (size_t)B * 4, hipMemcpyHostToDevice, st));
    if (e->ext_pin.record(st)) return 1;
    if (lengths) {
      lens = e->st_lens;
      hipLaunchKernelGGL(mask_tail_kernel, dim3(cdiv(T, 256), B), dim3(256), 0, st, e->st_mix, 1, (long)T, lens);
      DS_LAUNCH_CHECK();
    }
  }
  const bool batch_rng = !noise && (seeds || lengths);

  long draw = 0;
  auto next_noise = [&](const float** z) -> int {
    if (noise) { *z = noise + (size_t)draw * nst; }
    else {
      if (prof_launch(e, st, hbm_rec("randn (Philox4x32-10 + Box-Muller)", 4.0 * nst, B, 1, (int)T, S), [&]() {
            return batch_rng ? ds_launch_randn_batch(e->st_noise, B, S, T, (const uint64_t*)e->st_seeds, e->st_lens, (uint64_t)draw, st)
                             : ds_launch_randn(e->st_noise, (long)nst, seed, (uint64_t)draw, st);
          }))
        return 1;
      *z = e->st_noise;
    }
    ++draw;
    return 0;
  };
  const float* z = nullptr;
  if (next_noise(&z)) return 1;
  const float* smix = nullptr;
  if (mixture_scale(e, sde, B, T, st, &smix)) return 1;
  if (ds_launch_sde_prior(sp, e->st_mix, z, e->st_x, B, S, T, smix, st, lens)) return 1;
  DS_HIP(hipMemcpyAsync(e->st_xm, e->st_x, nst * 4, hipMemcpyDeviceToDevice, st));
  bool tail_ready = false;
  const float* score = e->st_score;
  auto eval_score = [&](int i) -> int {
    if (tail && (i >= N - tail_steps || i < head_steps)) {
      if (!tail_ready) {
        DS_HIP(hipMemcpyAsync(tail->st_mix, e->st_mix, (size_t)B * T * 4, hipMemcpyDeviceToDevice, st));
        tail_ready = true;
      }
      DS_HIP(hipMemcpyAsync(tail->st_x, e->st_x, nst * 4, hipMemcpyDeviceToDevice, st));
      DS_HIP(hipMemcpyAsync(tail->st_t, e->st_t, (size_t)B * 4, hipMemcpyDeviceToDevice, st));
      score = tail->st_score;
      return run_nfe(tail, B, T, st);
    }
    score = e->st_score;
    return run_nfe(e, B, T, st);
  };
  for (int i = 0; i < N; ++i) {
    DS_HIP(hipMemcpyAsync(e->st_t, e->st_ts + (size_t)i * B, (size_t)B * 4, hipMemcpyDeviceToDevice, st));
    for (int k = 0; k < csteps; ++k) {
      if (eval_score(i)) return 1;
      if (next_noise(&z)) return 1;
      if (smp->corrector == DIFFSEP_CORR_LANGEVIN) {
        if (ds_launch_langevin(smp->snr, e->st_x, score, z, e->st_x, e->st_xm, B, (long)S * T, e->st_lang, st))
          return 1;
      } else if (prof_launch(e, st, hbm_rec("sde_corrector (ald2 update)", 4.0 * nst * 5.0, B, 1, (int)T, S), [&]() {
                   return ds_launch_sde_corrector(sp, smp->snr, e->st_x, e->st_t, score, z, e->st_x, e->st_xm, B, S, T,
                                                  smix, smp->corrector == DIFFSEP_CORR_ALD ? 1 : 0, st, lens);
                 })) {
        return 1;
      }
    }
    if (smp->predictor != DIFFSEP_PRED_NONE) {
      if (eval_score(i)) return 1;
      if (next_noise(&z)) return 1;
      if (prof_launch(e, st, hbm_rec("sde_predictor (reverse-diffusion update)", 4.0 * nst * 5.0, B, 1, (int)T, S), [&]() {
            return ds_launch_sde_predictor(sp, N, e->st_x, e->st_t, score, z, e->st_x, e->st_xm, B, S, T, smix, 0, st, lens);
          }))
        return 1;
    } else {
      DS_HIP(hipMemcpyAsync(e->st_xm, e->st_x, nst * 4, hipMemcpyDeviceToDevice, st));
    }
  }
  DS_HIP(hipMemcpyAsync(out, smp->denoise ? e->st_xm : e->st_x, nst * 4, hipMemcpyDeviceToDevice, st));
  if (nfe_out) *nfe_out = N * (csteps + 1);
  return 0;
}

extern "C" int32_t diffsep_pc_sample(diffsep_engine* e, const diffsep_sde_config* sde, const diffsep_sampler_config* smp,
                                     const float* mix_norm, float* out, int32_t B, int64_t T, const float* noise,
                                     uint64_t seed, const float* timesteps_host, int32_t* nfe_out, void* stream) {
  return diffsep_pc_sample_ex(e, sde, smp, nullptr, mix_norm, out, B, T, noise, seed, timesteps_host, nfe_out, stream);
}

extern "C" int32_t diffsep_ode_sample(diffsep_engine* e, const diffsep_sde_config* sde, const diffsep_ode_config* oc,
                                      const float* mix_norm, const float* x_init, const float* noise, uint64_t seed,
                                      float* out, int32_t B, int64_t T, diffsep_ode_info* info, void* stream) {
  DS_CHECK(e && sde && oc && mix_norm && out, "ode_sample: null argument");
  if (check_sde(e, sde, "ode_sample")) return 1;
  DS_CHECK(B >= 1 && T >= 1, "ode_sample: empty batch");
  DS_CHECK(!(x_init && noise), "ode_sample: x_init and noise are alternatives");
  double Ab[DS_ODE_MAX_K * DS_ODE_MAX_K], Bb[DS_ODE_MAX_K], Cb[DS_ODE_MAX_K], Eb[DS_ODE_MAX_K + 1];
  int ns = 0, eorder = 0;
  DS_CHECK(ds_ode_tableau(oc->method, nullptr, nullptr, nullptr, nullptr, &ns, &eorder) == 0,
           "ode_sample: method must be DIFFSEP_ODE_RK45 or DIFFSEP_ODE_RK23 (DOP853 / Radau / BDF / LSODA are not implemented)");
  {
    double A0[6 * 6];
    ds_ode_tableau(oc->method, A0, Bb, Cb, Eb, nullptr, nullptr);
    for (int i = 0; i < ns; ++i) for (int j = 0; j < ns; ++j) Ab[i * DS_ODE_MAX_K + j] = A0[i * ns + j];
  }
  const double eps = oc->eps;
  DS_CHECK(eps > 0.0 && eps < 1.0, "ode_sample: eps must be in (0, 1)");
// ... 186 lines not shown
```

### diffusion-separation_amd/csrc/unit.hip

```cpp
#include "engine_host.h"

extern "C" int32_t diffsep_time_embedding(const float* t, const float* fourier_w, const float* w1, const float* b1,
                                          const float* w2, const float* b2, float* temb, int32_t B, int32_t nf,
                                          void* workspace, int64_t workspace_bytes, void* stream) {
  DS_CHECK(t && fourier_w && w1 && b1 && w2 && b2 && temb && workspace, "time_embedding: null pointer");
  DS_CHECK(B >= 1 && nf >= 8 && nf % 8 == 0, "time_embedding: bad B / nf");
  DS_CHECK(workspace_bytes >= (int64_t)B * 6 * nf * 4, "time_embedding: workspace too small");
  hipStream_t st = (hipStream_t)stream;
  float* emb = (float*)workspace;
  float* t1 = emb + (size_t)B * 2 * nf;
  if (ds_launch_fourier(t, fourier_w, emb, B, nf, st)) return 1;
  if (ds_launch_linear(emb, w1, b1, t1, B, 2 * nf, 4 * nf, 0, st)) return 1;
  return ds_launch_linear(t1, w2, b2, temb, B, 4 * nf, 4 * nf, 1, st);
}

extern "C" int32_t diffsep_upfirdn2d(const void* x, void* y, int32_t B, int32_t H, int32_t W, int32_t C, int32_t ldx,
                                     int32_t ldy, int32_t up, int32_t dtype, void* stream) {
  DS_CHECK(x && y, "upfirdn2d: null pointer");
  return ds_launch_gn_apply(x, ldx, nullptr, nullptr, C, nullptr, 0, y, ldy, B, H, W, 0, up ? 1 : 2, dtype,
                            (hipStream_t)stream);
}

extern "C" int32_t diffsep_groupnorm_act(const void* x, const float* gamma, const float* beta, void* y, void* xr,
                                         int32_t B, int32_t H, int32_t W, int32_t C, int32_t ldx, int32_t ldy,
// ... 1 lines not shown
                                         int32_t dtype, void* workspace, int64_t workspace_bytes, void* stream) {
  DS_CHECK(x && y && workspace, "groupnorm: null pointer");
  const long wsb = (ds_gn_workspace_bytes(B, H, W, C) + 255) & ~255L;
  DS_CHECK(workspace_bytes >= wsb + 2L * B * C * 4, "groupnorm: workspace too small");
  float* scale = (float*)((char*)workspace + wsb);
  float* shift = scale + (long)B * C;
  hipStream_t st = (hipStream_t)stream;
  if (ds_launch_gn_stats(x, ldx, nullptr, 0, C, B, H, W, C, groups, eps, gamma, beta, workspace, scale, shift, dtype, st))
    return 1;
  return ds_launch_gn_apply(x, ldx, scale, shift, C, y, ldy, xr, ldxr, B, H, W, act, resample, dtype, st);
}

static int gn_forced_plan(int route, GnPlan* p) {
  switch (route) {
    case DIFFSEP_GN_APPLY: *p = {GnRoute::APPLY, 0}; return 0;
    case DIFFSEP_GN_BLOCK2X2: *p = {GnRoute::BLOCK2X2, 0}; return 0;
    case DIFFSEP_GN_DOWN_STRIP4: *p = {GnRoute::DOWN_STRIP, 4}; return 0;
    case DIFFSEP_GN_DOWN_STRIP8: *p = {GnRoute::DOWN_STRIP, 8}; return 0;
    case DIFFSEP_GN_DOWN_TILED4: *p = {GnRoute::DOWN_TILED, 4}; return 0;
    case DIFFSEP_GN_DOWN_TILED8: *p = {GnRoute::DOWN_TILED, 8}; return 0;
    case DIFFSEP_GN_UP_TILED: *p = {GnRoute::UP_TILED, 0}; return 0;
  }
  return 1;
}
static int gn_unit_shape(int32_t B, int32_t H, int32_t W, int32_t C, int32_t ldx, int32_t ldy, int32_t ldxr, bool has_y, bool has_xr,
                         int32_t mode, int32_t dtype) {
  DS_CHECK(dtype == DS_F32 || dtype == DS_BF16, "gn_apply: bad dtype");
  DS_CHECK(B >= 1 && H >= 1 && W >= 1 && C >= 8 && C % 8 == 0, "gn_apply: bad shape (C a multiple of 8)");
  DS_CHECK(mode >= 0 && mode <= 2 && (mode != 2 || (H % 2 == 0 && W % 2 == 0)), "gn_apply: bad resample mode (FIR down needs even H, W)");
  const int al = dtype == DS_F32 ? 4 : 8;
  DS_CHECK(ldx >= C && ldx % al == 0, "gn_apply: ldx must be >= C and a multiple of 16 bytes");
  DS_CHECK(!has_y || (ldy >= C && ldy % al == 0), "gn_apply: ldy must be >= C and a multiple of 16 bytes");
  DS_CHECK(!has_xr || (ldxr >= C && ldxr % al == 0), "gn_apply: ldxr must be >= C and a multiple of 16 bytes");
  return 0;
}
extern "C" int32_t diffsep_gn_apply(const void* x, const float* scale, const float* shift, void* y, void* xr, int32_t B, int32_t H,
                                    int32_t W, int32_t C, int32_t ldx, int32_t ldy, int32_t ldxr, int32_t act, int32_t mode,
                                    int32_t dtype, int32_t route, void* stream) {
  DS_CHECK(x && (scale != nullptr) == (shift != nullptr), "gn_apply: null pointer (scale and shift come together)");
  DS_CHECK((scale != nullptr) == (y != nullptr), "gn_apply: y is written with a table and only with one");
  DS_CHECK(scale || (mode != 0 && xr), "gn_apply: nothing to do");
  DS_CHECK(mode != 0 || !xr, "gn_apply: xr is the resampled raw tensor (mode 1 / 2)");
  if (gn_unit_shape(B, H, W, C, ldx, ldy, ldxr, y != nullptr, xr != nullptr, mode, dtype)) return 1;
  hipStream_t st = (hipStream_t)stream;
  if (route == DIFFSEP_GN_AUTO)
    return ds_launch_gn_apply(x, ldx, scale, shift, C, y, ldy, xr, ldxr, B, H, W, act, mode, dtype, st);
  GnPlan p;
  DS_CHECK(!gn_forced_plan(route, &p), "gn_apply: unknown route code");
  DS_CHECK(ds_gn_route_runs(p.route, mode, scale != nullptr, dtype, H, W, C, ldx, ldy, ldxr, xr != nullptr),
           "gn_apply: the forced kernel's shape preconditions do not hold (2 x 2 blocks: table, up or H % 4 == W % 4 == 0 down; strips: "
           "16-bit, table, down, W % 4 == 0; row tiles: half-precision build, 16-bit, table, down, W % 32 == 0, C % 64 == 0, ld % 8 == 0; "
           "up tiles: table, up, C % 64 == 0)");
  return ds_launch_gn_apply(p, x, ldx, scale, shift, C, y, ldy, xr, ldxr, B, H, W, act, mode, dtype, st);
}
extern "C" const char* diffsep_gn_route_name(int32_t mode, int32_t affine, int32_t dtype, int32_t B, int32_t H, int32_t W, int32_t C,
                                             int32_t ldx, int32_t ldy, int32_t ldxr, int32_t has_xr, int32_t cus) {
  if (gn_unit_shape(B, H, W, C, ldx, ldy, ldxr, affine != 0, has_xr != 0, mode, dtype)) return nullptr;
  const GnPlan p = ds_gn_route(mode, affine != 0, dtype, B, H, W, C, ldx, ldy, ldxr, has_xr != 0, cus);
  return ds_gn_kernel_name(p, mode, affine != 0, dtype);
}

static Tn view(const void* p, int H, int W, int C, int ld) {
  Tn t;
  t.p = const_cast<void*>(p); t.H = H; t.W = W; t.C = C; t.ld = ld;
  return t;
}

extern "C" int32_t diffsep_groupnorm_stats(const void* x, const void* x2, int32_t C1, const float* gamma,
                                           const float* beta, float* scale, float* shift, int32_t B, int32_t H,
                                           int32_t W, int32_t C, int32_t ldx, int32_t ldx2, int32_t groups, float eps,
                                           int32_t dtype, void* workspace, int64_t workspace_bytes, void* stream) {
  DS_CHECK(x && scale && shift && workspace, "groupnorm_stats: null pointer");
  DS_CHECK(workspace_bytes >= ds_gn_workspace_bytes(B, H, W, C), "groupnorm_stats: workspace too small");
  return ds_launch_gn_stats(x, ldx, x2, ldx2, x2 ? C1 : C, B, H, W, C, groups, eps, gamma, beta, workspace, scale, shift,
                            dtype, (hipStream_t)stream);
}

extern "C" int32_t diffsep_conv2d_fused(const void* x, const void* x2, int32_t C1, const float* gn_scale,
                                        const float* gn_shift, int32_t gn_act, const void* w, const float* bias,
                                        const float* bias_b, const void* res, void* y, int32_t B, int32_t H, int32_t W,
                                        int32_t Cin, int32_t Cout, int32_t ksize, int32_t ldx, int32_t ldx2,
                                        int32_t ldr, int32_t ldy, float out_scale, int32_t dtype, int64_t* stats,
                                        int32_t w_chunk, const int64_t* gn_acc1, const int64_t* gn_acc2,
                                        const float* gn_gamma, const float* gn_beta, int32_t gn_groups, void* stream) {
  DS_CHECK(ksize == 1 || ksize == 3, "conv2d: ksize must be 1 or 3");
  ConvArgs a;
  memset(&a, 0, sizeof(a));
  a.opts = ds_default_opts();
  a.stats_acc = (long long*)stats;
  if (gn_acc1) {
    DS_CHECK(gn_groups > 0 && Cin % gn_groups == 0, "conv2d: bad GroupNorm group count");
    a.gn_acc1 = (const long long*)gn_acc1; a.gn_acc2 = (const long long*)gn_acc2; a.gn_gamma = gn_gamma;
    a.gn_beta = gn_beta; a.gn_groups = gn_groups; a.gn_eps = 1e-6f;
    a.gn_inv_count = gn_inv_count((long)H * W, Cin, gn_groups);
  }
  a.w_chunked = w_chunk;
  Tn xin = view(x, H, W, Cin, ldx);
  xin.p2 = const_cast<void*>(x2); xin.ld2 = ldx2; xin.C1 = C1;
  conv_input(a, xin);
  a.gn_scale = gn_scale; a.gn_shift = gn_shift; a.gn_act = gn_act;
  a.w = w; a.w_bs = 0;
  a.bias = bias; a.bias_b = bias_b; a.bias_b_ld = Cout; a.bias_mode = 0;
  conv_residual(a, view(res, H, W, Cout, ldr));
  a.out_scale = out_scale;
  conv_output(a, view(y, H, W, Cout, ldy));
  a.B = B; a.Cout = Cout; a.taps = ksize == 3 ? 9 : 1;
// ... 354 lines not shown
```

### diffusion-separation_amd/diffsep_amd/_lib.py

```python
import ctypes as C
import os

_HERE = os.path.dirname(os.path.abspath(__file__))
LIB_PATH = os.environ.get("DIFFSEP_LIB", os.path.join(os.path.dirname(_HERE), "libdiffsep_hip.so"))
LIB_PATHS = {"bf16": LIB_PATH, "f16": os.environ.get("DIFFSEP_LIB_F16", os.path.join(os.path.dirname(_HERE), "libdiffsep_hip_f16.so"))}

F32, BF16 = 0, 1
F32_SPLIT = 2
F16 = 3
SDE_MIX, SDE_PRIORMIX = 0, 1
PRED_REVERSE_DIFFUSION, PRED_EULER_MARUYAMA, PRED_NONE = 0, 1, 2
CORR_ALD2, CORR_NONE, CORR_ALD, CORR_LANGEVIN = 0, 1, 2, 3


class ModelConfig(C.Structure):
    _fields_ = [("nf", C.c_int32), ("num_sources", C.c_int32), ("n_levels", C.c_int32), ("ch_mult", C.c_int32 * 8),
                ("num_res_blocks", C.c_int32), ("attn_resolution", C.c_int32), ("n_fft", C.c_int32),
                ("hop", C.c_int32), ("spec_abs_exponent", C.c_float), ("spec_factor", C.c_float),
                ("dtype", C.c_int32)]


class SdeConfig(C.Structure):
    _fields_ = [("kind", C.c_int32), ("ndim", C.c_int32), ("d_lambda", C.c_float), ("sigma_min", C.c_float),
                ("sigma_max", C.c_float), ("avg_len", C.c_int32)]
# ... 48 lines not shown
_lib = None

_P, _I, _L, _F, _U64 = C.c_void_p, C.c_int32, C.c_int64, C.c_float, C.c_uint64
_SIGS = {
    "diffsep_last_error": (C.c_char_p, []),
    "diffsep_version": (C.c_char_p, []),
    "diffsep_param_count": (_I, [C.POINTER(ModelConfig)]),
    "diffsep_param_info": (_I, [C.POINTER(ModelConfig), _I, C.c_char_p, _I, C.POINTER(_L), C.POINTER(_I),
                                C.POINTER(_L)]),
    "diffsep_param_total": (_L, [C.POINTER(ModelConfig)]),
    "diffsep_engine_create": (_I, [C.POINTER(ModelConfig), _P, _L, C.POINTER(_P)]),
    "diffsep_engine_destroy": (None, [_P]),
    "diffsep_engine_device_bytes": (_L, [_P]),
    "diffsep_engine_reserve": (_I, [_P, _I, _L, _P]),
    "diffsep_engine_debug_absmax": (_I, [_P, C.POINTER(C.c_double), _I, C.POINTER(_I)]),
    "diffsep_engine_debug_arena": (_I, [_P, C.POINTER(_P), C.POINTER(_L), C.POINTER(_L)]),
    "diffsep_num_frames": (_I, [C.POINTER(ModelConfig), _L]),
    "diffsep_padded_frames": (_I, [C.POINTER(ModelConfig), _L]),
    "diffsep_score_forward": (_I, [_P, _P, _P, _P, _P, _I, _L, _P]),
    "diffsep_backbone_forward": (_I, [_P, _P, _P, _P, _I, _I, _P]),
    "diffsep_pc_sample": (_I, [_P, C.POINTER(SdeConfig), C.POINTER(SamplerConfig), _P, _P, _I, _L, _P, _U64, _P,
                               C.POINTER(_I), _P]),
    "diffsep_pc_sample_ex": (_I, [_P, C.POINTER(SdeConfig), C.POINTER(SamplerConfig), C.POINTER(SamplerExt), _P, _P, _I,
                                  _L, _P, _U64, _P, C.POINTER(_I), _P]),
    "diffsep_ode_sample": (_I, [_P, C.POINTER(SdeConfig), C.POINTER(OdeConfig), _P, _P, _P, _U64, _P, _I, _L,
                                C.POINTER(OdeInfo), _P]),
    "diffsep_ode_tableau": (_I, [_I, _P, _P, _P, _P, C.POINTER(_I), C.POINTER(_I)]),
    "diffsep_ode_stage_update": (_I, [C.POINTER(SdeConfig), _P, _P, _P, _P, _P, _P, _P, _I, _I, C.c_double, _P, _P, _I,
                                      _I, _L, _P]),
    "diffsep_ode_error_norm": (_I, [C.POINTER(SdeConfig), _P, _P, _P, _P, _P, _P, _P, _P, _I, _I, C.c_double,
                                    C.c_double, C.c_double, _P, _I, _I, _L, _P, _L, _P]),
    "diffsep_engine_set_graph": (_I, [_P, _I]),
    "diffsep_set_option": (_I, [C.c_char_p, _L]),
    "diffsep_engine_set_option": (_I, [_P, C.c_char_p, _L]),
    "diffsep_engine_get_option": (_L, [_P, C.c_char_p]),
    "diffsep_engine_profile_begin": (_I, [_P]),
    "diffsep_engine_profile_end": (_I, [_P, C.POINTER(C.c_double), C.POINTER(C.c_double), C.POINTER(_L),
                                        C.POINTER(C.c_double)]),
    "diffsep_engine_profile_end_n": (_I, [_P, _I, C.POINTER(C.c_double), C.POINTER(C.c_double), C.POINTER(_L),
                                          C.POINTER(C.c_double), C.POINTER(_I)]),
    "diffsep_num_kernel_classes": (_I, []),
    "diffsep_engine_profile_records": (_I, [_P, C.POINTER(ProfRecord), _I, C.POINTER(_I)]),
    "diffsep_time_embedding": (_I, [_P, _P, _P, _P, _P, _P, _P, _I, _I, _P, _L, _P]),
    "diffsep_upfirdn2d": (_I, [_P, _P, _I, _I, _I, _I, _I, _I, _I, _I, _P]),
    "diffsep_groupnorm_act": (_I, [_P, _P, _P, _P, _P, _I, _I, _I, _I, _I, _I, _I, _I, _F, _I, _I, _I, _P, _L, _P]),
    "diffsep_conv2d": (_I, [_P, _P, _P, _P, _P, _P, _I, _I, _I, _I, _I, _I, _I, _I, _I, _F, _I, _P]),
    "diffsep_groupnorm_stats": (_I, [_P, _P, _I, _P, _P, _P, _P, _I, _I, _I, _I, _I, _I, _I, _F, _I, _P, _L, _P]),
    "diffsep_conv2d_fused": (_I, [_P, _P, _I, _P, _P, _I, _P, _P, _P, _P, _P, _I, _I, _I, _I, _I, _I, _I, _I, _I, _I, _F,
                                  _I, _P, _I, _P, _P, _P, _P, _I, _P]),
    "diffsep_conv2d_chunk": (_I, [_I, _I]),
    "diffsep_last_conv_kernel": (C.c_char_p, []),
    "diffsep_gn_finalize_acc": (_I, [_P, _I, _P, _I, _I, _L, _I, _F, _P, _P, _P, _P, _P]),
    "diffsep_gn_apply": (_I, [_P, _P, _P, _P, _P, _I, _I, _I, _I, _I, _I, _I, _I, _I, _I, _I, _P]),
    "diffsep_gn_route_name": (C.c_char_p, [_I, _I, _I, _I, _I, _I, _I, _I, _I, _I, _I, _I]),
    "diffsep_conv3x3_streamed": (_I, [_P, _P, _I, _P, _P, _P, _P, _P, _P, _P, _I, _I, _P, _P, _I, _I, _I, _I, _I, _F, _I, _P, _P,
                                      _P, _P, _P, _P, _P, _I, _P]),
    "diffsep_conv3x3_regweight": (_I, [_P, _P, _I, _P, _P, _P, _I, _P, _P, _P, _P, _I, _I, _P, _P, _P, _I, _I, _I, _I, _I, _F, _I, _P,
                                       _P]),
    "diffsep_attn_fused": (_I, [_P, _P, _P, _P, _I, _P, _P, _P, _P, _P, _P, _P, _P, _P, _P, _I, _I, _I, _P]),
    "diffsep_frag_index": (_L, [_I, _I, _I, _I, _I]),
    "diffsep_frag_index_split": (_L, [_I, _I, _I, _I, _I, _I]),
    "diffsep_resblock_forward": (_I, [_I, _I, _I, _I, _I, _I, _P, _L, _P, _P, _P, _I, _I, _I, _P]),
    "diffsep_attnblock_forward": (_I, [_I, _I, _P, _L, _P, _P, _I, _I, _I, _P]),
    "diffsep_attention": (_I, [_P, _P, _P, _P, _I, _I, _I, _I, _I, _P, _L, _P]),
    "diffsep_stft_pack": (_I, [_P, _P, _P, _I, _I, _L, _I, _I, _F, _F, _I, _I, _I, _I, _P, _L, _P]),
    "diffsep_istft_unpack": (_I, [_P, _P, _I, _I, _L, _I, _I, _F, _F, _I, _I, _I, _P, _L, _P]),
    "diffsep_stft_pack_ex": (_I, [_P, _P, _P, _I, _I, _L, _I, _I, _F, _F, _I, _I, _I, _I, _P, _L, _P, _I]),
    "diffsep_istft_unpack_ex": (_I, [_P, _P, _I, _I, _L, _I, _I, _F, _F, _I, _I, _I, _P, _L, _P, _I, _P, _P, _P, _I]),
    "diffsep_sde_sigma_mix": (_I, [_P, _P, _I, _L, _I, _P]),
    "diffsep_sde_prior": (_I, [C.POINTER(SdeConfig), _P, _P, _P, _I, _I, _L, _P, _P]),
    "diffsep_sde_corrector_update": (_I, [C.POINTER(SdeConfig), _F, _P, _P, _P, _P, _P, _P, _I, _I, _L, _P, _I, _P]),
    "diffsep_sde_predictor_update": (_I, [C.POINTER(SdeConfig), _I, _P, _P, _P, _P, _P, _P, _I, _I, _L, _P, _I, _P]),
    "diffsep_sde_coefficients": (_I, [C.POINTER(SdeConfig), _P, _P, _P, _P, _P, _I, _I, _L, _F, _F, _P]),
    "diffsep_sde_mean": (_I, [C.POINTER(SdeConfig), _P, _P, _P, _I, _I, _L, _P]),
    "diffsep_sde_std": (_I, [C.POINTER(SdeConfig), _P, _P, _P, _I, _I, _L, _P]),
    "diffsep_sde_mult_std": (_I, [_P, _P, _P, _I, _I, _L, _I, _P]),
    "diffsep_sde_mult_std_inv": (_I, [_P, _P, _P, _I, _I, _L, _I, _P]),
    "diffsep_sde_perturb": (_I, [C.POINTER(SdeConfig), _P, _P, _P, _P, _P, _P, _I, _P, _U64, _U64, _P, _P, _I, _I, _L, _P]),
    "diffsep_score_loss_workspace_bytes": (_L, [_I, _I, _L]),
    "diffsep_score_loss_reduce": (_I, [C.POINTER(SdeConfig), _P, _P, _P, _P, _P, _P, _P, _I, _P, _P, _P, _P, _I, _I, _L, _P,
                                       _L, _P]),
    "diffsep_score_loss": (_I, [_P, C.POINTER(SdeConfig), C.POINTER(LossConfig), _P, _P, _P, _P, _P, _U64, _P, _P, _P, _P, _P,
                                _P, _I, _L, _P, _L, _P]),
    "diffsep_score_loss_validate": (_I, [C.POINTER(ModelConfig), C.POINTER(LossConfig), _I, _L, _P, _L]),
    "diffsep_sde_reverse_drift": (_I, [_P, _P, _P, _P, _I, _L, _I, _I, _P]),
    "diffsep_sde_langevin_update": (_I, [_F, _P, _P, _P, _P, _P, _I, _L, _P, _L, _P]),
    "diffsep_normalize_batch": (_I, [_P, _P, _P, _P, _I, _L, _P]),
    "diffsep_scale_output": (_I, [_P, _P, _I, _I, _L, _P]),
    "diffsep_gram": (_I, [_P, _P, _P, _I, _I, _L, _P]),
    "diffsep_stoi_workspace_bytes": (_L, [_I, _I, _L, _I]),
    "diffsep_stoi": (_I, [_P, _P, _P, _I, _I, _L, _P, _P, _I, _I, _P, _L, _P]),
    "diffsep_randn": (_I, [_P, _L, _U64, _U64, _P]),
    "diffsep_randn_batch": (_I, [_P, _I, _I, _L, _P, _P, _U64, _P]),
    "diffsep_convert": (_I, [_P, _P, _L, _I, _I, _P]),
}
EXPORTS = tuple(_SIGS.keys())


def lib(kind="bf16"):
    global _lib
    if _lib is None:
        _lib = {}
    if kind not in _lib:
        path = LIB_PATHS[kind]
        if not os.path.exists(path):
            raise DiffsepError(f"{path} not found: build it with __graft_entry__.build() or "
# ... 48 lines not shown
```

### diffusion-separation_amd/diffsep_amd/engine.py

```python
import ctypes as C

import numpy as np
import torch

from . import _lib
from ._lib import F32, BF16, F16, check, lib


def _stream_ptr(device=None):
    return C.c_void_p(torch.cuda.current_stream(device).cuda_stream)


def _ptr(t):
    return C.c_void_p(t.data_ptr()) if t is not None else C.c_void_p(0)


def _c_cfg(cfg):
    if cfg.dtype != F16:
        return cfg
    c2 = _lib.ModelConfig()
    C.memmove(C.byref(c2), C.byref(cfg), C.sizeof(cfg))
    c2.dtype = BF16
    return c2

# ... 25 lines not shown
        v = state[key]
        v = v.detach().cpu().numpy() if isinstance(v, torch.Tensor) else np.asarray(v)
        if tuple(v.shape) != shape:
            raise ValueError(f"parameter '{key}' has shape {tuple(v.shape)}, expected {shape}")
        blob[off:off + v.size] = v.astype(np.float32, copy=False).reshape(-1)
    return blob


class Engine:

    def __init__(self, cfg, weights_blob, device=None, lib_kind=None):
        if not torch.cuda.is_available():
            raise _lib.DiffsepError("no GPU visible: the separation engine has no CPU path")
        self.device = torch.device("cuda", torch.cuda.current_device()) if device is None else torch.device(device)
        self.kind = _lib.half_kind(cfg.dtype) if lib_kind is None else lib_kind
        if cfg.dtype in (F16, BF16) and self.kind != _lib.half_kind(cfg.dtype):
            raise _lib.DiffsepError("a 16-bit engine lives in the library build of its storage format")
        self._L = lib(self.kind)
        cfg = _c_cfg(cfg)
        self.cfg = cfg
        blob = np.ascontiguousarray(weights_blob, dtype=np.float32)
        self._h = C.c_void_p()
        with torch.cuda.device(self.device):
            check(self._L.diffsep_engine_create(C.byref(cfg), blob.ctypes.data_as(C.c_void_p), blob.size,
                                                C.byref(self._h)), self._L)
        self.S = cfg.num_sources

    def close(self):
        if getattr(self, "_h", None):
            self._L.diffsep_engine_destroy(self._h)
            self._h = None

    def __del__(self):
        try:
            self.close()
        except Exception:
            pass

    @property
    def dtype(self):
        return self.cfg.dtype

    def device_bytes(self):
        return int(self._L.diffsep_engine_device_bytes(self._h))

    def set_graph(self, enable):
        check(self._L.diffsep_engine_set_graph(self._h, int(bool(enable))), self._L)

    def set_option(self, name, value):
        check(self._L.diffsep_engine_set_option(self._h, str(name).encode(), int(value)), self._L)

    def get_option(self, name):
        return int(self._L.diffsep_engine_get_option(self._h, str(name).encode()))

    CONV_CLASSES = ("conv3x3_8x32xN64", "conv3x3_8x32xN32", "conv3x3_8x8xN64", "gemm1x1_256xN64", "gemm1x1_256xN32",
                    "gemm1x1_64xN64", "conv3x3_ws_64to64", "conv3x3_small_16couts", "conv3x3_rw_regweights", "attention_fused",
                    "conv3x3_sw_streamed", "conv3x3_sws_split")

    def profile_begin(self):
        check(self._L.diffsep_engine_profile_begin(self._h), self._L)

    def profile_end(self):
        nc = len(self.CONV_CLASSES)
        fl, ms, n, by = (C.c_double * nc)(), (C.c_double * nc)(), (C.c_int64 * nc)(), (C.c_double * nc)()
        nw = C.c_int32(0)
        check(self._L.diffsep_engine_profile_end_n(self._h, nc, fl, ms, n, by, C.byref(nw)), self._L)
        return {k: (fl[i], ms[i], int(n[i]), by[i]) for i, k in enumerate(self.CONV_CLASSES[:nw.value])}

    def profile_records(self):
        from ._lib import ProfRecord
        n = C.c_int32(0)
        check(self._L.diffsep_engine_profile_records(self._h, None, 0, C.byref(n)), self._L)
        buf = (ProfRecord * max(1, n.value))()
        check(self._L.diffsep_engine_profile_records(self._h, buf, n.value, C.byref(n)), self._L)
        return [dict(kernel=r.kernel.decode(), B=r.B, H=r.H, W=r.W, Cin=r.Cin, Cout=r.Cout, taps=r.taps,
                     skip_cin=r.skip_cin, has_res=bool(r.has_res), cls=r.cls, flops=r.flops, bytes=r.bytes, ms=r.ms)
                for r in buf[:n.value]]

    def padded_frames(self, T):
        return int(self._L.diffsep_padded_frames(C.byref(self.cfg), T))

    def bucket_length(self, W):
        return int(self.cfg.hop) * int(W) - (int(self.cfg.n_fft) - int(self.cfg.hop)) - 1

    def _f32(self, t):
        assert t.is_cuda and t.dtype == torch.float32, "device float32 tensor expected"
        return t.contiguous()

    def score(self, xt, t, mix):
        xt, t, mix = self._f32(xt), self._f32(t), self._f32(mix)
        B, S, T = xt.shape
        assert S == self.S and mix.shape == (B, 1, T) and t.shape == (B,)
        out = torch.empty_like(xt)
        with torch.cuda.device(self.device):
            check(self._L.diffsep_score_forward(self._h, _ptr(xt), _ptr(t), _ptr(mix), _ptr(out), B, T,
                                              _stream_ptr(self.device)), self._L)
        return out

    def reserve(self, B, T):
        with torch.cuda.device(self.device):
            check(self._L.diffsep_engine_reserve(self._h, int(B), int(T), _stream_ptr(self.device)), self._L)

    def debug_absmax(self):
        n = C.c_int32(0)
        check(self._L.diffsep_engine_debug_absmax(self._h, None, 0, C.byref(n)), self._L)
        buf = (C.c_double * (4 * max(1, n.value)))()
# ... 101 lines not shown
```

### diffusion-separation_amd/diffsep_amd/ops.py

```python
import ctypes as C
import math

import numpy as np
import torch

from ._lib import F32_SPLIT, F32, BF16, GN_ROUTES, ODE_WORKSPACE_BYTES, LossConfig, SdeConfig, SDE_MIX, check, lib
from .engine import _ptr, _stream_ptr


def _dt(t):
    if t.dtype == torch.float32:
        return F32
    if t.dtype in (torch.bfloat16, torch.float16):
        return BF16
    raise TypeError("float32, bfloat16 or float16 expected")


def _L(t):
    return lib("f16" if (t is not None and t.dtype == torch.float16) else "bf16")


def _dts(t, split):
    if split and t.dtype != torch.float32:
        raise TypeError("split products are a mode of fp32 tensors")
# ... 75 lines not shown
    return (y, st) if stats is not False else y


def conv3x3_regweight(x, wpacked, cout, x2=None, gn=None, bias=None, bias_b=None, skip=None, res=None, out_scale=1.0, stats=False,
                      w_chunk=0):
    B, H, W, C1 = x.shape
    Cin = C1 + (x2.shape[-1] if x2 is not None else 0)
    y = torch.zeros((B, H, W, cout), dtype=x.dtype, device=x.device)
    sc, sh = gn if gn is not None else (None, None)
    st = torch.zeros((B, cout, 2), dtype=torch.int64, device=x.device) if stats else None
    sx, sx2, sw = skip if skip is not None else (None, None, None)
    sC1 = sx.shape[-1] if sx is not None else 0
    sCin = sC1 + (sx2.shape[-1] if sx2 is not None else 0)
    check(_L(x).diffsep_conv3x3_regweight(_ptr(x), _ptr(x2), C1, _ptr(sc), _ptr(sh), _ptr(wpacked), w_chunk, _ptr(bias), _ptr(bias_b),
                                          _ptr(sx), _ptr(sx2), sC1, sCin, _ptr(sw), _ptr(res), _ptr(y), B, H, W, Cin, cout, out_scale,
                                          _dt(x), _ptr(st), _stream_ptr()), _L(x))
    return (y, st) if stats else y


def conv2d_chunk(ksize, dtype):
    return lib().diffsep_conv2d_chunk(ksize, F32 if dtype == torch.float32 else BF16)


def upfirdn2d(x, up):
    B, H, W, Cc = x.shape
    Ho, Wo = (2 * H, 2 * W) if up else (H // 2, W // 2)
    y = torch.empty((B, Ho, Wo, Cc), dtype=x.dtype, device=x.device)
    check(_L(x).diffsep_upfirdn2d(_ptr(x), _ptr(y), B, H, W, Cc, Cc, Cc, int(up), _dt(x), _stream_ptr()), _L(x))
    return y


def groupnorm_act(x, gamma, beta, groups, eps=1e-6, act=1, resample=0, want_xr=False):
    B, H, W, Cc = x.shape
    Ho, Wo = {0: (H, W), 1: (2 * H, 2 * W), 2: (H // 2, W // 2)}[resample]
    y = torch.empty((B, Ho, Wo, Cc), dtype=x.dtype, device=x.device)
    xr = torch.empty_like(y) if want_xr else None
    ws = torch.empty(B * 64 * Cc * 16 + 2 * B * Cc * 4 + 4096, dtype=torch.uint8, device=x.device)
    check(_L(x).diffsep_groupnorm_act(_ptr(x), _ptr(gamma), _ptr(beta), _ptr(y), _ptr(xr), B, H, W, Cc, Cc, Cc, Cc,
                                      groups, eps, act, resample, _dt(x), _ptr(ws), ws.numel(), _stream_ptr()), _L(x))
    return (y, xr) if want_xr else y


def gn_apply(x, scale, shift, act, resample, want_y=True, want_xr=False, route=None, pad=(0, 0, 0)):
    B, H, W, Cc = x.shape
    Ho, Wo = {0: (H, W), 1: (2 * H, 2 * W), 2: (H // 2, W // 2)}[resample]
    nan = float("nan")
    xb = torch.full((B, H, W, Cc + pad[0]), nan, dtype=x.dtype, device=x.device)
    xb[..., :Cc] = x
    yb = torch.full((B, Ho, Wo, Cc + pad[1]), nan, dtype=x.dtype, device=x.device) if want_y else None
    xrb = torch.full((B, Ho, Wo, Cc + pad[2]), nan, dtype=x.dtype, device=x.device) if want_xr else None
    check(_L(x).diffsep_gn_apply(_ptr(xb), _ptr(scale), _ptr(shift), _ptr(yb), _ptr(xrb), B, H, W, Cc, Cc + pad[0], Cc + pad[1],
                                 Cc + pad[2], int(act), resample, _dt(x), GN_ROUTES[route or "auto"], _stream_ptr()), _L(x))
    return (yb[..., :Cc] if want_y else None, xrb[..., :Cc] if want_xr else None, yb, xrb)


def gn_route_name(kind, resample, affine, dtype, B, H, W, C, pad=(0, 0, 0), has_xr=True, cus=256):
    l = lib(kind)
    name = l.diffsep_gn_route_name(resample, int(affine), F32 if dtype == torch.float32 else BF16, B, H, W, C, C + pad[0], C + pad[1],
                                   C + pad[2], int(has_xr), cus)
    if name is None:
        check(1, l)
    return name.decode()


def conv2d(x, wpacked, bias, cout, ksize, bias_b=None, res=None, out_scale=1.0, cout_pad=None):
    B, H, W, Cin = x.shape
    cp = cout if cout_pad is None else cout_pad
    y = torch.zeros((B, H, W, cp), dtype=x.dtype, device=x.device)
    check(_L(x).diffsep_conv2d(_ptr(x), _ptr(wpacked), _ptr(bias), _ptr(bias_b), _ptr(res), _ptr(y), B, H, W, Cin,
                               cout, ksize, Cin, res.shape[-1] if res is not None else 0, cp, out_scale, _dt(x),
                               _stream_ptr()), _L(x))
    return y


def groupnorm_stats(x, gamma, beta, groups, eps=1e-6, x2=None):
    B, H, W, C1 = x.shape
    Cc = C1 + (x2.shape[-1] if x2 is not None else 0)
    scale = torch.empty((B, Cc), dtype=torch.float32, device=x.device)
    shift = torch.empty_like(scale)
    ws = torch.empty(B * 64 * Cc * 16 + 4096, dtype=torch.uint8, device=x.device)
    check(_L(x).diffsep_groupnorm_stats(_ptr(x), _ptr(x2), C1, _ptr(gamma), _ptr(beta), _ptr(scale), _ptr(shift), B, H,
                                        W, Cc, C1, x2.shape[-1] if x2 is not None else 0, groups, eps, _dt(x), _ptr(ws),
                                        ws.numel(), _stream_ptr()), _L(x))
    return scale, shift


STAT_SUM_SCALE, STAT_SQ_SCALE = 2.0 ** 24, 2.0 ** 16


def conv2d_fused(x, wpacked, bias, cout, ksize, x2=None, gn=None, gn_act=1, bias_b=None, res=None, out_scale=1.0,
                 cout_pad=None, out=None, stats=False, w_chunk=0, gn_acc=None, split=False):
    B, H, W, C1 = x.shape
    Cin = C1 + (x2.shape[-1] if x2 is not None else 0)
    cp = cout if cout_pad is None else cout_pad
    y = torch.zeros((B, H, W, cp), dtype=x.dtype, device=x.device) if out is None else out
    sc, sh = gn if gn is not None else (None, None)
    st = None
    if stats is True:
        st = torch.zeros((B, cout, 2), dtype=torch.int64, device=x.device)
    elif stats is not False:
        st = stats
    a1, a2, gam, bet, grp = gn_acc if gn_acc is not None else (None, None, None, None, 0)
    check(_L(x).diffsep_conv2d_fused(_ptr(x), _ptr(x2), C1, _ptr(sc), _ptr(sh), gn_act, _ptr(wpacked), _ptr(bias),
                                     _ptr(bias_b), _ptr(res), _ptr(y), B, H, W, Cin, cout, ksize, C1,
                                     x2.shape[-1] if x2 is not None else 0, res.shape[-1] if res is not None else 0, cp,
                                     out_scale, _dts(x, split), _ptr(st), w_chunk, _ptr(a1), _ptr(a2), _ptr(gam), _ptr(bet), grp,
# ... 395 lines not shown
```

### include/diffsep_hip.h

```cpp
#ifndef DIFFSEP_HIP_H
#define DIFFSEP_HIP_H

#include <stdint.h>

#ifdef __cplusplus
extern "C" {
#endif

#define DIFFSEP_F32 0
#define DIFFSEP_BF16 1
#define DIFFSEP_F32_SPLIT 2

#define DIFFSEP_SDE_MIX 0
#define DIFFSEP_SDE_PRIORMIX 1

#define DIFFSEP_PRED_REVERSE_DIFFUSION 0
#define DIFFSEP_PRED_EULER_MARUYAMA 1
#define DIFFSEP_PRED_NONE 2

#define DIFFSEP_CORR_ALD2 0
#define DIFFSEP_CORR_NONE 1
#define DIFFSEP_CORR_ALD 2
#define DIFFSEP_CORR_LANGEVIN 3

// ... 123 lines not shown
  double flops, bytes;
  double ms;
} diffsep_prof_record;
int32_t diffsep_engine_profile_records(diffsep_engine* e, diffsep_prof_record* out, int32_t cap, int32_t* n);


int32_t diffsep_time_embedding(const float* t, const float* fourier_w, const float* w1, const float* b1, const float* w2,
                               const float* b2, float* temb, int32_t B, int32_t nf, void* workspace,
                               int64_t workspace_bytes, void* stream);

int32_t diffsep_upfirdn2d(const void* x, void* y, int32_t B, int32_t H, int32_t W, int32_t C, int32_t ldx,
                          int32_t ldy, int32_t up, int32_t dtype, void* stream);

int32_t diffsep_groupnorm_act(const void* x, const float* gamma, const float* beta, void* y, void* xr, int32_t B,
                              int32_t H, int32_t W, int32_t C, int32_t ldx, int32_t ldy, int32_t ldxr,
                              int32_t groups, float eps, int32_t act, int32_t resample, int32_t dtype,
                              void* workspace, int64_t workspace_bytes, void* stream);
int32_t diffsep_istft_unpack_ex(const void* x, float* out, int32_t B, int32_t S, int64_t T, int32_t n_fft,
                                int32_t hop, float exponent, float factor, int32_t W, int32_t Cpad, int32_t dtype,
                                void* workspace, int64_t workspace_bytes, void* stream, int32_t split, const float* ow,
                                const float* ob, const float* tdiv, int32_t ow_cin);

int32_t diffsep_conv2d(const void* x, const void* w, const float* bias, const float* bias_b, const void* res,
                       void* y, int32_t B, int32_t H, int32_t W, int32_t Cin, int32_t Cout, int32_t ksize,
                       int32_t ldx, int32_t ldr, int32_t ldy, float out_scale, int32_t dtype, void* stream);

int32_t diffsep_groupnorm_stats(const void* x, const void* x2, int32_t C1, const float* gamma, const float* beta,
                                float* scale, float* shift, int32_t B, int32_t H, int32_t W, int32_t C, int32_t ldx,
                                int32_t ldx2, int32_t groups, float eps, int32_t dtype, void* workspace,
                                int64_t workspace_bytes, void* stream);

int32_t diffsep_conv2d_fused(const void* x, const void* x2, int32_t C1, const float* gn_scale, const float* gn_shift,
                             int32_t gn_act, const void* w, const float* bias, const float* bias_b, const void* res,
                             void* y, int32_t B, int32_t H, int32_t W, int32_t Cin, int32_t Cout, int32_t ksize,
                             int32_t ldx, int32_t ldx2, int32_t ldr, int32_t ldy, float out_scale, int32_t dtype,
                             int64_t* stats, int32_t w_chunk, const int64_t* gn_acc1, const int64_t* gn_acc2,
                             const float* gn_gamma, const float* gn_beta, int32_t gn_groups, void* stream);
int32_t diffsep_conv2d_chunk(int32_t ksize, int32_t dtype);
const char* diffsep_last_conv_kernel(void);
int32_t diffsep_gn_finalize_acc(const int64_t* acc1, int32_t C1, const int64_t* acc2, int32_t C2, int32_t B, int64_t npix,
                                int32_t groups, float eps, const float* gamma, const float* beta, float* scale, float* shift,
                                void* stream);
#define DIFFSEP_GN_AUTO 0
#define DIFFSEP_GN_APPLY 1
#define DIFFSEP_GN_BLOCK2X2 2
#define DIFFSEP_GN_DOWN_STRIP4 3
#define DIFFSEP_GN_DOWN_STRIP8 4
#define DIFFSEP_GN_DOWN_TILED4 5
#define DIFFSEP_GN_DOWN_TILED8 6
#define DIFFSEP_GN_UP_TILED 7
int32_t diffsep_gn_apply(const void* x, const float* scale, const float* shift, void* y, void* xr, int32_t B, int32_t H, int32_t W,
                         int32_t C, int32_t ldx, int32_t ldy, int32_t ldxr, int32_t act, int32_t mode, int32_t dtype, int32_t route,
                         void* stream);
const char* diffsep_gn_route_name(int32_t mode, int32_t affine, int32_t dtype, int32_t B, int32_t H, int32_t W, int32_t C,
                                  int32_t ldx, int32_t ldy, int32_t ldxr, int32_t has_xr, int32_t cus);
int32_t diffsep_conv3x3_streamed(const void* x, const void* x2, int32_t C1, const float* gn_scale, const float* gn_shift,
                                 const void* w_frag, const float* bias, const float* bias_b, const void* sx, const void* sx2,
                                 int32_t sC1, int32_t sCin, const void* sw_frag, void* y, int32_t B, int32_t H, int32_t W,
                                 int32_t Cin, int32_t Cout, float out_scale, int32_t dtype, int64_t* stats, const void* res,
                                 const void* ident_frag, const int64_t* gn_acc1, const int64_t* gn_acc2, const float* gn_gamma,
                                 const float* gn_beta, int32_t gn_groups, void* stream);
int32_t diffsep_conv3x3_regweight(const void* x, const void* x2, int32_t C1, const float* gn_scale, const float* gn_shift,
                                  const void* w, int32_t w_chunk, const float* bias, const float* bias_b, const void* sx,
                                  const void* sx2, int32_t sC1, int32_t sCin, const void* sw, const void* res, void* y, int32_t B,
                                  int32_t H, int32_t W, int32_t Cin, int32_t Cout, float out_scale, int32_t dtype, int64_t* stats,
                                  void* stream);
int32_t diffsep_attn_fused(const void* x, const int64_t* gn_acc, const float* gn_gamma, const float* gn_beta, int32_t gn_groups,
                           const float* gn_scale, const float* gn_shift, const void* wqk, const void* wv, const void* wo,
                           const float* bqk, const float* bv, const float* bo, void* y, int64_t* stats, int32_t B, int32_t L,
                           int32_t C, void* stream);
int64_t diffsep_frag_index(int32_t cout, int32_t tap, int32_t cin, int32_t taps, int32_t Cout);
int64_t diffsep_frag_index_split(int32_t cout, int32_t tap, int32_t cin, int32_t taps, int32_t Cout, int32_t plane);

int32_t diffsep_resblock_forward(int32_t in_ch, int32_t out_ch, int32_t up, int32_t down, int32_t temb_dim,
                                 int32_t dtype, const float* params_host, int64_t n_floats, const void* x,
                                 const float* temb, void* y, int32_t B, int32_t H, int32_t W, void* stream);
int32_t diffsep_attnblock_forward(int32_t channels, int32_t dtype, const float* params_host, int64_t n_floats,
                                  const void* x, void* y, int32_t B, int32_t H, int32_t W, void* stream);

int32_t diffsep_attention(const void* q, const void* k, const void* vt, void* o, int32_t B, int32_t L, int32_t C,
                          int32_t ld, int32_t dtype, void* workspace, int64_t workspace_bytes, void* stream);

int32_t diffsep_stft_pack(const float* xt, const float* mix, void* y, int32_t B, int32_t S, int64_t T,
                          int32_t n_fft, int32_t hop, float exponent, float factor, int32_t W, int32_t Cpad,
                          int32_t centered_shift, int32_t dtype, void* workspace, int64_t workspace_bytes,
                          void* stream);
int32_t diffsep_stft_pack_ex(const float* xt, const float* mix, void* y, int32_t B, int32_t S, int64_t T,
                             int32_t n_fft, int32_t hop, float exponent, float factor, int32_t W, int32_t Cpad,
                             int32_t centered_shift, int32_t dtype, void* workspace, int64_t workspace_bytes,
                             void* stream, int32_t split);

int32_t diffsep_istft_unpack(const void* x, float* out, int32_t B, int32_t S, int64_t T, int32_t n_fft,
                             int32_t hop, float exponent, float factor, int32_t W, int32_t Cpad, int32_t dtype,
                             void* workspace, int64_t workspace_bytes, void* stream);

int32_t diffsep_sde_sigma_mix(const float* mix, float* sigma_mix, int32_t B, int64_t T, int32_t avg_len, void* stream);
int32_t diffsep_sde_prior(const diffsep_sde_config* sde, const float* y, const float* z, float* x, int32_t B,
                          int32_t S, int64_t T, const float* sigma_mix, void* stream);
int32_t diffsep_sde_corrector_update(const diffsep_sde_config* sde, float snr, const float* x, const float* t,
                                     const float* score, const float* z, float* x_out, float* x_mean_out,
                                     int32_t B, int32_t S, int64_t T, const float* sigma_mix, int32_t variant,
                                     void* stream);
int32_t diffsep_sde_predictor_update(const diffsep_sde_config* sde, int32_t N, const float* x, const float* t,
                                     const float* score, const float* z, float* x_out, float* x_mean_out,
                                     int32_t B, int32_t S, int64_t T, const float* sigma_mix,
                                     int32_t probability_flow, void* stream);
// ... 64 lines not shown
```

Before: 77.30 utterances/s.

## Precompute time-embedding projections per sampler run and fold GN finalize into resample kernels

The Fourier/MLP/dense time-embedding projection for all N time steps is now computed once before sampling and copied into a per-step buffer. A second captured graph variant skips the in-graph embedding MLP. Separately, the GroupNorm resample (up/down FIR) kernels can read raw accumulated statistics and build the per-block scale/shift table in LDS, which removes the separate GN finalize launch. This cuts small kernel launches per NFE, at the cost of extra memory, a per-step device copy, and more graph variants.

```diff
diff --git a/diffusion-separation_amd/csrc/common.h b/diffusion-separation_amd/csrc/common.h
--- a/diffusion-separation_amd/csrc/common.h
+++ b/diffusion-separation_amd/csrc/common.h
@@ -214,6 +214,8 @@
 #define DS_OPT_NO_SW_ROWS4 32768u
 #define DS_OPT_SW_ROWS4 65536u
 #define DS_OPT_NO_SWS 16384u
+#define DS_OPT_TEMB_PER_EVAL 262144u
+#define DS_OPT_GN_FINALIZE_LAUNCH 131072u
 #define DS_OPT_NO_WFRAG 32u
 unsigned ds_default_opts();
 int ds_num_cus();
@@ -285,10 +287,14 @@
 bool ds_gn_route_runs(GnRoute r, int mode, bool affine, int dtype, int H, int W, int C, int ldx, int ldy, int ldxr, bool has_xr);
 GnPlan ds_gn_route(int mode, bool affine, int dtype, int B, int H, int W, int C, int ldx, int ldy, int ldxr, bool has_xr, int cus);
 const char* ds_gn_kernel_name(const GnPlan& p, int mode, bool affine, int dtype);
+struct GnAccum { const long long* acc; const float* gamma; const float* beta; int groups; float inv_count; float eps; };
+bool ds_gn_route_takes_acc(const GnPlan& p, int mode, int dtype, int C, int groups);
 int ds_launch_gn_apply(const void* x, int ldx, const float* scale, const float* shift, int C, void* y, int ldy,
-                       void* xr, int ldxr, int B, int H, int W, int act, int mode, int dtype, hipStream_t st);
+                       void* xr, int ldxr, int B, int H, int W, int act, int mode, int dtype, hipStream_t st,
+                       const GnAccum* acc = nullptr);
 int ds_launch_gn_apply(const GnPlan& p, const void* x, int ldx, const float* scale, const float* shift, int C, void* y, int ldy,
-                       void* xr, int ldxr, int B, int H, int W, int act, int mode, int dtype, hipStream_t st);
+                       void* xr, int ldxr, int B, int H, int W, int act, int mode, int dtype, hipStream_t st,
+                       const GnAccum* acc = nullptr);
 int ds_launch_concat(const void* a, int lda, int Ca, const void* b, int ldb, int Cb, void* y, int ldy, long npix,
                      int dtype, hipStream_t st);
 int ds_launch_softmax(const void* x, void* y, long rows, int L, int ld, int dtype, hipStream_t st);
diff --git a/diffusion-separation_amd/csrc/engine.hip b/diffusion-separation_amd/csrc/engine.hip
--- a/diffusion-separation_amd/csrc/engine.hip
+++ b/diffusion-separation_amd/csrc/engine.hip
@@ -27,7 +27,9 @@
     {"no_sws", "DIFFSEP_NO_SWS", DS_OPT_NO_SWS},
     {"no_sw_rows4", "DIFFSEP_NO_SW_ROWS4", DS_OPT_NO_SW_ROWS4},
     {"sw_rows4", nullptr, DS_OPT_SW_ROWS4},
-    {"no_sw_rw", "DIFFSEP_NO_SW_RW", DS_OPT_NO_SW_RW}};
+    {"no_sw_rw", "DIFFSEP_NO_SW_RW", DS_OPT_NO_SW_RW},
+    {"gn_finalize_launch", "DIFFSEP_GN_FINALIZE_LAUNCH", DS_OPT_GN_FINALIZE_LAUNCH},
+    {"temb_per_eval", "DIFFSEP_TEMB_PER_EVAL", DS_OPT_TEMB_PER_EVAL}};
 static std::atomic<unsigned> g_opts{0};
 static std::once_flag g_opts_once;
 unsigned ds_default_opts() {
@@ -224,11 +226,18 @@
   const char* name = mode == 1 ? (aff ? "gn_fir_up (GroupNorm + SiLU + FIR x2 up of act and raw)" : "fir_up (pyramid)")
                                : (mode == 2 ? (aff ? "gn_fir_down (GroupNorm + SiLU + FIR x2 down of act and raw)" : "fir_down (pyramid)")
                                             : "gn_apply (GroupNorm affine + SiLU)");
+  const GnAccum acc = {aff ? aff->acc1 : nullptr, aff ? aff->gamma : nullptr, aff ? aff->beta : nullptr, aff ? aff->groups : 0,
+                       aff ? aff->inv_count : 0.f, 1e-6f};
   return prof_launch(e, st, hbm_rec(name, bytes, B, x.H, x.W, x.C), [&]() {
     return ds_launch_gn_apply(x.p, x.ld, aff ? aff->scale : nullptr, aff ? aff->shift : nullptr, x.C, y ? y->p : nullptr,
                               y ? y->ld : 0, xr ? xr->p : nullptr, xr ? xr->ld : 0, B, x.H, x.W, act, mode, e->cfg.dtype,
-                              st);
+                              st, &acc);
   });
+}
+static bool resample_takes_acc(const diffsep_engine* e, const Tn& x, int mode, int B) {
+  if (e->opts & DS_OPT_GN_FINALIZE_LAUNCH) return false;
+  const GnPlan p = ds_gn_route(mode, true, e->cfg.dtype, B, x.H, x.W, x.C, x.ld, x.C, x.C, true,  0);
+  return ds_gn_route_takes_acc(p, mode, e->cfg.dtype, x.C, gn_group_count(x.C));
 }
 
 static const float kInvSqrt2 = 0.70710678118654752440f;
@@ -285,7 +294,7 @@
       return conv(e, c2b, out, B, st);
     }
   }
-  if (gn_stats(e, x, P(e, m.gn0_w), P(e, m.gn0_b), B, a0, st, mode == 0)) return 1;
+  if (gn_stats(e, x, P(e, m.gn0_w), P(e, m.gn0_b), B, a0, st, mode == 0 || (!x.p2 && resample_takes_acc(e, x, mode, B)))) return 1;
   Tn h1 = e_tensor(e, B, Ho, Wo, m.out_ch);
   Tn xr = x, h0m;
   if (mode) {
@@ -411,10 +420,13 @@
   float* t1 = e_f32(e, (size_t)B * 4 * nf);
   float* temb = e_f32(e, (size_t)B * 4 * nf);
   float* proj = e_f32(e, (size_t)B * A.dense_total);
-  const Module& mf = A.mods[mi++];
-  const Module& l1 = A.mods[mi++];
-  const Module& l2 = A.mods[mi++];
-  if (!e->dry) {
+  mi += 3;
+  if (e->temb_ready) {
+    proj = e->st_proj;
+  } else if (!e->dry) {
+    const Module& mf = A.mods[0];
+    const Module& l1 = A.mods[1];
+    const Module& l2 = A.mods[2];
     if (ds_launch_fourier(t, P(e, mf.w0), emb, B, nf, st)) return 1;
     if (ds_launch_linear(emb, P(e, l1.w0), P(e, l1.b0), t1, B, 2 * nf, 4 * nf, 0, st)) return 1;
     if (ds_launch_linear(t1, P(e, l2.w0), P(e, l2.b0), temb, B, 4 * nf, 4 * nf, 1, st)) return 1;
@@ -511,6 +523,35 @@
   Conv co(pyramid, PK(e, A.pk_out), A.chan_out, 1);
   co.bias = P(e, A.out_b); co.div_b = t;
   return conv(e, co, yy, B, st);
+}
+
+int time_projection(diffsep_engine* e, const float* t, int rows, float* proj, float* ws, hipStream_t st) {
+  const Arch& A = e->arch;
+  const int nf = e->cfg.nf;
+  const Module& mf = A.mods[0];
+  const Module& l1 = A.mods[1];
+  const Module& l2 = A.mods[2];
+  float* emb = ws;
+  float* t1 = emb + (size_t)rows * 2 * nf;
+  float* temb = t1 + (size_t)rows * 4 * nf;
+  for (int r0 = 0; r0 < rows; r0 += 32768) {
+    const int n = rows - r0 < 32768 ? rows - r0 : 32768;
+    if (ds_launch_fourier(t + r0, P(e, mf.w0), emb + (size_t)r0 * 2 * nf, n, nf, st)) return 1;
+    if (ds_launch_linear(emb + (size_t)r0 * 2 * nf, P(e, l1.w0), P(e, l1.b0), t1 + (size_t)r0 * 4 * nf, n, 2 * nf, 4 * nf, 0, st)) return 1;
+    if (ds_launch_linear(t1 + (size_t)r0 * 4 * nf, P(e, l2.w0), P(e, l2.b0), temb + (size_t)r0 * 4 * nf, n, 4 * nf, 4 * nf, 1, st)) return 1;
+    if (ds_launch_linear_t(temb + (size_t)r0 * 4 * nf, e->d_dense_w, e->d_dense_b, proj + (size_t)r0 * A.dense_total, n, 4 * nf,
+                           A.dense_total, 1, st))
+      return 1;
+  }
+  return 0;
+}
+
+extern "C" int32_t diffsep_engine_time_projection(diffsep_engine* e, const float* t, int32_t rows, float* proj, void* workspace,
+                                                  int64_t workspace_bytes, void* stream) {
+  DS_CHECK(e && t && proj && workspace && rows >= 1, "time_projection: bad argument");
+  DS_CHECK(workspace_bytes >= (int64_t)rows * 10 * e->cfg.nf * 4, "time_projection: workspace too small");
+  StreamScope sc_(e, stream);
+  return time_projection(e, t, rows, proj, (float*)workspace, sc_.st);
 }
 
 static int score_forward_impl(diffsep_engine* e, const float* xt, const float* t, const float* mix, float* out, int B,
@@ -553,7 +594,7 @@
 static void drop_graph(diffsep_engine* e) {
   for (auto& kv : e->graphs) destroy_graph(kv.second);
   e->graphs.clear();
-  e->cur_graph = nullptr;
+  e->cur_graph[0] = e->cur_graph[1] = nullptr;
 }
 
 static void layout_state(diffsep_engine* e, int B, long T) {
@@ -564,6 +605,7 @@
   e->st_score = (float*)e_alloc(e, nst * 4);
   e->st_noise = (float*)e_alloc(e, nst * 4);
   e->st_t = (float*)e_alloc(e, (size_t)B * 4);
+  e->st_proj = (float*)e_alloc(e, (size_t)B * e->arch.dense_total * 4);
   e->st_mix = (float*)e_alloc(e, (size_t)B * T * 4);
   e->st_smix = (float*)e_alloc(e, (size_t)B * T * 4);
   e->st_ts = (float*)e_alloc(e, 4096 * (size_t)B * 4);
@@ -575,7 +617,7 @@
 int ensure_plan(diffsep_engine* e, int B, long T, hipStream_t st) {
   if (e->planB == B && e->planT == T && e->arena) return 0;
   DS_CHECK(B >= 1 && T >= 1, "empty batch or signal");
-  e->cur_graph = nullptr;
+  e->cur_graph[0] = e->cur_graph[1] = nullptr;
   e->planB = -1;
   e->planT = -1;
   e->dry = true;
@@ -601,10 +643,10 @@
   layout_state(e, B, T);
   e->planB = B;
   e->planT = T;
-  {
-    auto it = e->graphs.find(std::make_pair(B, T));
+  for (int v = 0; v < 2; ++v) {
+    auto it = e->graphs.find(std::make_pair(B | (v ? DS_GRAPH_TEMB_READY : 0), T));
     if (it != e->graphs.end()) {
-      e->cur_graph = &it->second;
+      e->cur_graph[v] = &it->second;
       it->second.used = ++e->graph_tick;
     }
   }
@@ -613,9 +655,16 @@
   return 0;
 }
 
-int run_nfe(diffsep_engine* e, int B, long T, hipStream_t st) {
+struct TembReadyScope {
+  diffsep_engine* e;
+  TembReadyScope(diffsep_engine* e_, bool v) : e(e_) { e->temb_ready = v; }
+  ~TembReadyScope() { e->temb_ready = false; }
+};
+int run_nfe(diffsep_engine* e, int B, long T, hipStream_t st, bool temb_ready) {
+  TembReadyScope trs(e, temb_ready);
+  const int gv = temb_ready ? 1 : 0;
   if (e->use_graph && e->warmed && !e->prof) {
-    if (!e->cur_graph) {
+    if (!e->cur_graph[gv]) {
       DS_HIP(hipStreamBeginCapture(st, hipStreamCaptureModeThreadLocal));
       const int rc = score_forward_impl(e, e->st_x, e->st_t, e->st_mix, e->st_score, B, T, st);
       diffsep_engine::GraphRec r{nullptr, nullptr, 0};
@@ -636,16 +685,17 @@
             auto lru = e->graphs.begin();
             for (auto it = e->graphs.begin(); it != e->graphs.end(); ++it)
               if (it->second.used < lru->second.used) lru = it;
+            if (&lru->second == e->cur_graph[1 - gv]) e->cur_graph[1 - gv] = nullptr;
             destroy_graph(lru->second);
             e->graphs.erase(lru);
           }
         }
         r.used = ++e->graph_tick;
-        e->cur_graph = &(e->graphs[std::make_pair(B, (long)T)] = r);
+        e->cur_graph[gv] = &(e->graphs[std::make_pair(B | (gv ? DS_GRAPH_TEMB_READY : 0), (long)T)] = r);
       }
     }
-    if (e->cur_graph) {
-      DS_HIP(hipGraphLaunch(e->cur_graph->x, st));
+    if (e->cur_graph[gv]) {
+      DS_HIP(hipGraphLaunch(e->cur_graph[gv]->x, st));
       return 0;
     }
   }
@@ -679,7 +729,7 @@
 diffsep_engine::~diffsep_engine() {
   drop_graph(this);
   hipFree(d_blob); hipFree(d_pack); hipFree(d_dense_w); hipFree(d_dense_b); hipFree(d_attn_b); hipFree(d_tab);
-  hipFree(arena); hipFree(ode_buf);
+  hipFree(arena); hipFree(ode_buf); hipFree(proj_all);
   if (own) hipStreamDestroy(own);
   if (ev_in) hipEventDestroy(ev_in);
   if (ev_out) hipEventDestroy(ev_out);
@@ -735,7 +785,7 @@
   return 0;
 }
 extern "C" int64_t diffsep_engine_device_bytes(const diffsep_engine* e) {
-  return e ? e->weight_bytes + (int64_t)e->cap + (int64_t)e->ode_cap : 0;
+  return e ? e->weight_bytes + (int64_t)e->cap + (int64_t)e->ode_cap + (int64_t)e->proj_all_cap : 0;
 }
 extern "C" int32_t diffsep_engine_set_graph(diffsep_engine* e, int32_t enable) {
   DS_CHECK(e, "null engine");
@@ -780,6 +830,7 @@
   if (!strcmp(name, "graph_cache")) return e->graph_cap;
   if (!strcmp(name, "graphs_cached")) return (int64_t)e->graphs.size();
   if (!strcmp(name, "ablate")) return e->ablate;
+  if (!strcmp(name, "dense_total")) return e->arch.dense_total;
   if (!opt_bit(name, &bit)) return (e->opts & bit) ? 1 : 0;
   return -1;
 }
diff --git a/diffusion-separation_amd/csrc/engine_host.h b/diffusion-separation_amd/csrc/engine_host.h
--- a/diffusion-separation_amd/csrc/engine_host.h
+++ b/diffusion-separation_amd/csrc/engine_host.h
@@ -248,12 +248,18 @@
   long planT = -1;
   float *st_x = nullptr, *st_xm = nullptr, *st_score = nullptr, *st_t = nullptr, *st_noise = nullptr,
         *st_ts = nullptr, *st_mix = nullptr, *st_smix = nullptr, *st_lang = nullptr;
+  float* st_proj = nullptr;
+  float* proj_all = nullptr;
+  size_t proj_all_cap = 0;
+  std::vector<float> proj_ts;
+  int proj_B = 0;
+  bool temb_ready = false;
   int* st_lens = nullptr;
   unsigned long long* st_seeds = nullptr;
   PinnedStage ext_pin;
   struct GraphRec { hipGraph_t g; hipGraphExec_t x; uint64_t used; };
   std::map<std::pair<int, long>, GraphRec> graphs;
-  GraphRec* cur_graph = nullptr;
+  GraphRec* cur_graph[2] = {nullptr, nullptr};
   int graph_cap = 12;
   uint64_t graph_tick = 0;
   int use_graph = 1;
@@ -333,7 +339,9 @@
 int attention_core(const Tn& q, const void* k, const void* vt, const Tn& o, int B, void* scores, void* probs, int dtype,
                    hipStream_t st, int split = 0);
 int ensure_plan(diffsep_engine* e, int B, long T, hipStream_t st);
-int run_nfe(diffsep_engine* e, int B, long T, hipStream_t st);
+int run_nfe(diffsep_engine* e, int B, long T, hipStream_t st, bool temb_ready = false);
+int time_projection(diffsep_engine* e, const float* t, int rows, float* proj, float* ws, hipStream_t st);
+#define DS_GRAPH_TEMB_READY (1 << 30)
 int ds_launch_mask_tail(float* v, int B, int rows, long T, const int* lens, hipStream_t st);
 
 #pragma GCC visibility pop
diff --git a/diffusion-separation_amd/csrc/norm.hip b/diffusion-separation_amd/csrc/norm.hip
--- a/diffusion-separation_amd/csrc/norm.hip
+++ b/diffusion-separation_amd/csrc/norm.hip
@@ -162,29 +162,64 @@
   return 0;
 }
 
+struct GnAccK { const long long* acc; const float* gamma; const float* beta; int cpg; float inv_count; float eps; };
+constexpr int GN_TAB_MAX = 512;
+__device__ inline __attribute__((always_inline)) void gn_block_table(const GnAccK& g, int b, int C, int c0, int n, float* tab,
+                                                                     long long* tmp) {
+  const int lo = (c0 / g.cpg) * g.cpg;
+  int hi = ((c0 + n + g.cpg - 1) / g.cpg) * g.cpg;
+  if (hi > C) hi = C;
+  for (int c = threadIdx.x; c < hi - lo; c += 256)
+    *reinterpret_cast<longlong2*>(tmp + 2 * c) = *reinterpret_cast<const longlong2*>(g.acc + ((long)b * C + lo + c) * 2);
+  sync_lds();
+  for (int c = threadIdx.x; c < n; c += 256) {
+    const int ch = c0 + c;
+    const long long* src = tmp + ((ch / g.cpg) * g.cpg - lo) * 2;
+    long long ssum = 0, ssq = 0;
+    for (int j = 0; j < g.cpg; ++j) {
+      ssum += src[2 * j];
+      ssq += src[2 * j + 1];
+    }
+    const double mean = (double)ssum * (1.0 / DS_STAT_SUM_SCALE) * (double)g.inv_count;
+    double var = (double)ssq * (1.0 / DS_STAT_SQ_SCALE) * (double)g.inv_count - mean * mean;
+    if (var < 0.0) var = 0.0;
+    const float sc = (float)(1.0 / sqrt(var + (double)g.eps)) * (g.gamma ? g.gamma[ch] : 1.f);
+    tab[c] = sc;
+    tab[n + c] = (g.beta ? g.beta[ch] : 0.f) - (float)mean * sc;
+  }
+}
+
 template <typename T, int MODE, bool AFFINE>
 __global__ __launch_bounds__(256) void gn_apply_kernel(const T* __restrict__ x, int ldx,
                                                        const float* __restrict__ scale,
                                                        const float* __restrict__ shift, int C, T* __restrict__ y,
                                                        int ldy, T* __restrict__ xr, int ldxr, int B, int H, int W,
-                                                       int act) {
+                                                       int act, GnAccK g) {
   const int Ho = MODE == 1 ? 2 * H : (MODE == 2 ? H / 2 : H);
   const int Wo = MODE == 1 ? 2 * W : (MODE == 2 ? W / 2 : W);
   const int ncg = C >> 3;
-  const long total = (long)B * Ho * Wo * ncg;
+  __shared__ float tab[AFFINE ? 2 * GN_TAB_MAX : 1];
+  __shared__ __attribute__((aligned(16))) long long tmp[AFFINE ? 2 * GN_TAB_MAX : 2];
+  const bool lazy = AFFINE && g.acc != nullptr;
+  const int bs = lazy ? (int)blockIdx.y : 0;
+  if (lazy) {
+    gn_block_table(g, bs, C, 0, C, tab, tmp);
+    __syncthreads();
+  }
+  const long total = (long)(lazy ? 1 : B) * Ho * Wo * ncg;
   for (long i = (long)blockIdx.x * 256 + threadIdx.x; i < total; i += (long)gridDim.x * 256) {
     const int cg = (int)(i % ncg);
     long r = i / ncg;
     const int ox = (int)(r % Wo);
     r /= Wo;
     const int oy = (int)(r % Ho);
-    const int b = (int)(r / Ho);
+    const int b = bs + (int)(r / Ho);
     float sc[8], sf[8];
     if (AFFINE) {
 #pragma unroll
       for (int j = 0; j < 8; ++j) {
-        sc[j] = scale[(long)b * C + cg * 8 + j];
-        sf[j] = shift[(long)b * C + cg * 8 + j];
+        sc[j] = lazy ? tab[cg * 8 + j] : scale[(long)b * C + cg * 8 + j];
+        sf[j] = lazy ? tab[C + cg * 8 + j] : shift[(long)b * C + cg * 8 + j];
       }
     }
     const T* xb = x + (long)b * H * W * ldx + cg * 8;
@@ -247,24 +282,32 @@
                                                              const float* __restrict__ scale,
                                                              const float* __restrict__ shift, int C, T* __restrict__ y,
                                                              int ldy, T* __restrict__ xr, int ldxr, int B, int H, int W,
-                                                             int act) {
+                                                             int act, GnAccK g) {
   constexpr int NR = MODE == 1 ? 3 : 6;
   const int Hb = MODE == 1 ? H : H / 4, Wb = MODE == 1 ? W : W / 4;
   const int Ho = MODE == 1 ? 2 * H : H / 2, Wo = MODE == 1 ? 2 * W : W / 2;
   const int ncg = C >> 3;
-  const long total = (long)B * Hb * Wb * ncg;
+  __shared__ float tab[2 * GN_TAB_MAX];
+  __shared__ __attribute__((aligned(16))) long long tmp[2 * GN_TAB_MAX];
+  const bool lazy = g.acc != nullptr;
+  const int bs = lazy ? (int)blockIdx.y : 0;
+  if (lazy) {
+    gn_block_table(g, bs, C, 0, C, tab, tmp);
+    __syncthreads();
+  }
+  const long total = (long)(lazy ? 1 : B) * Hb * Wb * ncg;
   for (long i = (long)blockIdx.x * 256 + threadIdx.x; i < total; i += (long)gridDim.x * 256) {
     const int cg = (int)(i % ncg);
     long r = i / ncg;
     const int bx = (int)(r % Wb);
     r /= Wb;
     const int by = (int)(r % Hb);
-    const int b = (int)(r / Hb);
+    const int b = bs + (int)(r / Hb);
     float sc[8], sf[8];
 #pragma unroll
     for (int j = 0; j < 8; ++j) {
-      sc[j] = scale[(long)b * C + cg * 8 + j];
-      sf[j] = shift[(long)b * C + cg * 8 + j];
+      sc[j] = lazy ? tab[cg * 8 + j] : scale[(long)b * C + cg * 8 + j];
+      sf[j] = lazy ? tab[C + cg * 8 + j] : shift[(long)b * C + cg * 8 + j];
     }
     const T* xb = x + (long)b * H * W * ldx + cg * 8;
     const int iy0 = MODE == 1 ? by - 1 : 4 * by - 1, ix0 = MODE == 1 ? bx - 1 : 4 * bx - 1;
@@ -331,18 +374,22 @@
                                                                 const float* __restrict__ scale,
                                                                 const float* __restrict__ shift, int C,
                                                                 bf16_t* __restrict__ y, int ldy, bf16_t* __restrict__ xr,
-                                                                int ldxr, int B, int H, int W, int act) {
+                                                                int ldxr, int B, int H, int W, int act, GnAccK g) {
   const int Ho = H / 2, Wo = W / 2, ncg = C >> 3, ntx = Wo / 2, nst = (Ho + RS - 1) / RS;
-  const long total = (long)B * nst * ntx * ncg;
+  __shared__ float tab[2 * GN_TAB_MAX];
+  __shared__ __attribute__((aligned(16))) long long tmp[2 * GN_TAB_MAX];
+  const bool lazy = g.acc != nullptr;
+  const long total = (long)(lazy ? 1 : B) * nst * ntx * ncg;
   const long i = (long)blockIdx.x * 256 + threadIdx.x;
-  if (i >= total) return;
+  const bool live = i < total;
+  if (!lazy && !live) return;
   const int cg = (int)(i % ncg);
   long r = i / ncg;
   const int tx = (int)(r % ntx);
   r /= ntx;
-  const int st = (int)(r % nst), b = (int)(r / nst);
+  const int st = (int)(r % nst), b = lazy ? (int)blockIdx.y : (int)(r / nst);
   float sc[8], sf[8];
-  {
+  if (!lazy) {
     const float4 s0 = *reinterpret_cast<const float4*>(scale + (long)b * C + cg * 8), s1 = *reinterpret_cast<const float4*>(scale + (long)b * C + cg * 8 + 4);
     const float4 h0 = *reinterpret_cast<const float4*>(shift + (long)b * C + cg * 8), h1 = *reinterpret_cast<const float4*>(shift + (long)b * C + cg * 8 + 4);
     sc[0] = s0.x; sc[1] = s0.y; sc[2] = s0.z; sc[3] = s0.w; sc[4] = s1.x; sc[5] = s1.y; sc[6] = s1.z; sc[7] = s1.w;
@@ -389,7 +436,14 @@
 #pragma unroll
     for (int j = 0; j < 8; ++j) { pa[q][j] = 0.f; px[q][j] = 0.f; qa[q][j] = 0.f; qx[q][j] = 0.f; }
   uint4 cur[6], nxt[6];
-  load_row(iy0, cur);
+  if (live) load_row(iy0, cur);
+  if (lazy) {
+    gn_block_table(g, b, C, 0, C, tab, tmp);
+    sync_lds();
+    if (!live) return;
+#pragma unroll
+    for (int j = 0; j < 8; ++j) { sc[j] = tab[cg * 8 + j]; sf[j] = tab[C + cg * 8 + j]; }
+  }
 #pragma unroll
   for (int k = 0; k < 2 * RS + 2; ++k) {
     if (k + 1 < 2 * RS + 2) load_row(iy0 + k + 1, nxt);
@@ -434,9 +488,11 @@
                                                                 const float* __restrict__ scale,
                                                                 const float* __restrict__ shift, int C,
                                                                 bf16_t* __restrict__ y, int ldy, bf16_t* __restrict__ xr,
-                                                                int ldxr, int B, int H, int W, int act, int tiles_x, int strips) {
+                                                                int ldxr, int B, int H, int W, int act, int tiles_x, int strips,
+                                                                GnAccK g) {
   constexpr int CP = 144, NCOL = 34, TB = NCOL * CP;
   __shared__ __attribute__((aligned(16))) char sm[2][2][TB];
+  __shared__ float tab[2 * 64];
   const int tid = threadIdx.x, cg = tid & 7, col = tid >> 3;
   const int ncgb = C >> 6;
   int bid = blockIdx.x;
@@ -447,7 +503,7 @@
   const int ch0 = cgb * 64 + cg * 8;
   const int Ho = H >> 1, Wo = W >> 1;
   float sc[8], sf[8];
-  {
+  if (!g.acc) {
     const float4 s0 = *reinterpret_cast<const float4*>(scale + (long)b * C + ch0), s1 = *reinterpret_cast<const float4*>(scale + (long)b * C + ch0 + 4);
     const float4 h0 = *reinterpret_cast<const float4*>(shift + (long)b * C + ch0), h1 = *reinterpret_cast<const float4*>(shift + (long)b * C + ch0 + 4);
     sc[0] = s0.x; sc[1] = s0.y; sc[2] = s0.z; sc[3] = s0.w; sc[4] = s1.x; sc[5] = s1.y; sc[6] = s1.z; sc[7] = s1.w;
@@ -533,6 +589,12 @@
   load_row(iy0, r0, h0);
   load_row(iy0 + 1, r1, h1);
   load_row(iy0 + 2, r2, h2);
+  if (g.acc) {
+    gn_block_table(g, b, C, cgb * 64, 64, tab, reinterpret_cast<long long*>(&sm[0][0][0]));
+    sync_lds();
+#pragma unroll
+    for (int j = 0; j < 8; ++j) { sc[j] = tab[cg * 8 + j]; sf[j] = tab[64 + cg * 8 + j]; }
+  }
   for (int k = 0; k < NR; k += 4) {
     if (k + 3 < NR) load_row(iy0 + k + 3, r3, h3);
     do_row(k, r0, h0, false);
@@ -558,12 +620,13 @@
                                                                    const float* __restrict__ shift, int C,
                                                                    T* __restrict__ y, int ldy, T* __restrict__ xr,
                                                                    int ldxr, int B, int H, int W, int act, int tiles_x,
-                                                                   int tiles_y) {
+                                                                   int tiles_y, GnAccK g) {
   constexpr int TH_ = 4, TW_ = 8, CG = 8;
   constexpr int IH = TH_ + 2, IW = TW_ + 2;
   constexpr int RAWB = 8 * (int)sizeof(T);
   constexpr int PITCH = 32 + RAWB;
   extern __shared__ __attribute__((aligned(16))) char sm[];
+  __shared__ float tab[2 * 64];
   const int tid = threadIdx.x;
   const int ncgb = (C >> 3) / CG;
   int bid = blockIdx.x;
@@ -573,37 +636,57 @@
   const int b = bid / tiles_y;
   const int cg = tid & 7;
   const int ch0 = (cgb * CG + cg) * 8;
-  float sc[8], sf[8];
-#pragma unroll
-  for (int j = 0; j < 8; ++j) {
-    sc[j] = scale[(long)b * C + ch0 + j];
-    sf[j] = shift[(long)b * C + ch0 + j];
-  }
   const int iy0 = ty * TH_ - 1, ix0 = tx * TW_ - 1;
   const T* xb = x + (long)b * H * W * ldx + ch0;
-  for (int i = tid; i < IH * IW * CG; i += 256) {
-    const int pix = i >> 3;
+  constexpr int NIT = (IH * IW * CG + 255) / 256, NV = sizeof(T) == 4 ? 2 : 1;
+  uint4 raw[NIT][NV];
+  bool ok[NIT];
+#pragma unroll
+  for (int it = 0; it < NIT; ++it) {
+    const int i = tid + 256 * it, pix = i >> 3;
     const int r = pix / IW, c = pix - r * IW;
     const int iy = iy0 + r, ix = ix0 + c;
+    ok[it] = i < IH * IW * CG && iy >= 0 && iy < H && ix >= 0 && ix < W;
+#pragma unroll
+    for (int q = 0; q < NV; ++q)
+      raw[it][q] = ok[it] ? reinterpret_cast<const uint4*>(xb + ((long)iy * W + ix) * ldx)[q] : make_uint4(0, 0, 0, 0);
+  }
+  float sc[8], sf[8];
+  if (g.acc) {
+    gn_block_table(g, b, C, cgb * 64, 64, tab, reinterpret_cast<long long*>(sm));
+    sync_lds();
+  }
+#pragma unroll
+  for (int j = 0; j < 8; ++j) {
+    sc[j] = g.acc ? tab[cg * 8 + j] : scale[(long)b * C + ch0 + j];
+    sf[j] = g.acc ? tab[64 + cg * 8 + j] : shift[(long)b * C + ch0 + j];
+  }
+#pragma unroll
+  for (int it = 0; it < NIT; ++it) {
+    const int i = tid + 256 * it, pix = i >> 3;
+    if (i >= IH * IW * CG) break;
     char* dst = sm + (pix * CG + cg) * PITCH;
     float v[8];
-    if (iy >= 0 && iy < H && ix >= 0 && ix < W) {
-      const T* src = xb + ((long)iy * W + ix) * ldx;
+    if (ok[it]) {
       float f[8];
-      load8<T>(src, f);
+      if constexpr (sizeof(T) == 4) {
+        f[0] = __uint_as_float(raw[it][0].x); f[1] = __uint_as_float(raw[it][0].y); f[2] = __uint_as_float(raw[it][0].z); f[3] = __uint_as_float(raw[it][0].w);
+        f[4] = __uint_as_float(raw[it][NV - 1].x); f[5] = __uint_as_float(raw[it][NV - 1].y); f[6] = __uint_as_float(raw[it][NV - 1].z); f[7] = __uint_as_float(raw[it][NV - 1].w);
+      } else {
+        f[0] = h_lo(raw[it][0].x); f[1] = h_hi(raw[it][0].x); f[2] = h_lo(raw[it][0].y); f[3] = h_hi(raw[it][0].y);
+        f[4] = h_lo(raw[it][0].z); f[5] = h_hi(raw[it][0].z); f[6] = h_lo(raw[it][0].w); f[7] = h_hi(raw[it][0].w);
+      }
 #pragma unroll
       for (int j = 0; j < 8; ++j) {
         const float u = f[j] * sc[j] + sf[j];
         v[j] = act ? silu_t<T>(u) : u;
       }
-      *reinterpret_cast<uint4*>(dst + 32) = reinterpret_cast<const uint4*>(src)[0];
-      if (sizeof(T) == 4) *reinterpret_cast<uint4*>(dst + 48) = reinterpret_cast<const uint4*>(src)[1];
     } else {
 #pragma unroll
       for (int j = 0; j < 8; ++j) v[j] = 0.f;
-      *reinterpret_cast<uint4*>(dst + 32) = make_uint4(0, 0, 0, 0);
-      if (sizeof(T) == 4) *reinterpret_cast<uint4*>(dst + 48) = make_uint4(0, 0, 0, 0);
-    }
+    }
+    *reinterpret_cast<uint4*>(dst + 32) = raw[it][0];
+    if (sizeof(T) == 4) *reinterpret_cast<uint4*>(dst + 48) = raw[it][NV - 1];
     *reinterpret_cast<float4*>(dst) = make_float4(v[0], v[1], v[2], v[3]);
     *reinterpret_cast<float4*>(dst + 16) = make_float4(v[4], v[5], v[6], v[7]);
   }
@@ -679,6 +762,15 @@
   return false;
 }
 
+bool ds_gn_route_takes_acc(const GnPlan& p, int mode, int dtype, int C, int groups) {
+  (void)dtype;
+  if (mode == 0 || C > GN_TAB_MAX || groups <= 0 || C % groups != 0) return false;
+  switch (p.route) {
+    case GnRoute::APPLY: case GnRoute::BLOCK2X2: case GnRoute::DOWN_STRIP: case GnRoute::DOWN_TILED: case GnRoute::UP_TILED: return true;
+  }
+  return false;
+}
+
 #ifndef FD_RS_MAX
 #define FD_RS_MAX 8
 #endif
@@ -723,21 +815,24 @@
 
 template <typename T>
 static int gn_launch_typed(const GnPlan& p, const void* x, int ldx, const float* scale, const float* shift, int C, void* y, int ldy,
-                           void* xr, int ldxr, int B, int H, int W, int act, int mode, hipStream_t st) {
+                           void* xr, int ldxr, int B, int H, int W, int act, int mode, hipStream_t st, const GnAccum* acc) {
   const int Ho = mode == 1 ? 2 * H : (mode == 2 ? H / 2 : H);
   const int Wo = mode == 1 ? 2 * W : (mode == 2 ? W / 2 : W);
-  const long total = (long)B * Ho * Wo * (C >> 3);
+  const int Bx = acc ? 1 : B, By = acc ? B : 1;
+  GnAccK g = {nullptr, nullptr, nullptr, 1, 0.f, 0.f};
+  if (acc) g = {acc->acc, acc->gamma, acc->beta, C / acc->groups, acc->inv_count, acc->eps};
+  const long total = (long)Bx * Ho * Wo * (C >> 3);
   long nb = (total + 255) / 256;
   if (nb > 16384) nb = 16384;
   if (nb < 1) nb = 1;
-  const bool aff = scale != nullptr;
-  const long tot2 = (mode == 1 ? (long)B * H * W : (long)B * (H / 4) * (W / 4)) * (C >> 3);
+  const bool aff = scale != nullptr || acc != nullptr;
+  const long tot2 = (mode == 1 ? (long)Bx * H * W : (long)Bx * (H / 4) * (W / 4)) * (C >> 3);
   if (p.route == GnRoute::UP_TILED) {
     const int th = cdiv(H, 4), tw = cdiv(W, 8);
     const long nblk = (long)B * th * tw * (C / 64);
     DS_FUNC_LDS_ONCE((gn_resample_up_tiled_kernel<T>), gn_resample_up_tiled_lds<T>());
     hipLaunchKernelGGL((gn_resample_up_tiled_kernel<T>), dim3((unsigned)nblk), dim3(256), gn_resample_up_tiled_lds<T>(), st,
-                       (const T*)x, ldx, scale, shift, C, (T*)y, ldy, (T*)xr, ldxr, B, H, W, act, tw, th);
+                       (const T*)x, ldx, scale, shift, C, (T*)y, ldy, (T*)xr, ldxr, B, H, W, act, tw, th, g);
     DS_LAUNCH_CHECK();
     ds_set_last_conv_kernel(sizeof(T) == 4 ? "gn_resample_up_tiled_kernel<f32>" : "gn_resample_up_tiled_kernel<" DS_HALF_NAME ">");
     return 0;
@@ -751,7 +846,7 @@
 #define FD(RS_)                                                                                                                          \
   do {                                                                                                                                   \
     hipLaunchKernelGGL((gn_fir_down_tiled_kernel<RS_>), dim3(nblk), dim3(256), 0, st, (const bf16_t*)x, ldx, scale, shift, C, (bf16_t*)y, \
-                       ldy, (bf16_t*)xr, ldxr, B, H, W, act, tiles_x, strips);                                                           \
+                       ldy, (bf16_t*)xr, ldxr, B, H, W, act, tiles_x, strips, g);                                                        \
     ds_set_last_conv_kernel("gn_fir_down_tiled_kernel<" #RS_ ">");                                                                       \
   } while (0)
       if (rs == 16) FD(16); else if (rs == 8) FD(8); else FD(4);
@@ -761,18 +856,18 @@
     }
 #endif
     if (p.route == GnRoute::DOWN_STRIP) {
-      const long per_row = (long)B * (W / 4) * (C >> 3);
+      const long per_row = (long)Bx * (W / 4) * (C >> 3);
       if (p.rs == 8) {
         constexpr int RS = 8;
         const long tot3 = per_row * cdiv(H / 2, RS);
-        hipLaunchKernelGGL((gn_fir_down_strip_kernel<RS>), dim3((unsigned)cdiv(tot3, 256)), dim3(256), 0, st, (const bf16_t*)x, ldx, scale,
-                           shift, C, (bf16_t*)y, ldy, (bf16_t*)xr, ldxr, B, H, W, act);
+        hipLaunchKernelGGL((gn_fir_down_strip_kernel<RS>), dim3((unsigned)cdiv(tot3, 256), By), dim3(256), 0, st, (const bf16_t*)x, ldx, scale,
+                           shift, C, (bf16_t*)y, ldy, (bf16_t*)xr, ldxr, B, H, W, act, g);
         ds_set_last_conv_kernel("gn_fir_down_strip_kernel<8>");
       } else {
         constexpr int RS = 4;
         const long tot3 = per_row * cdiv(H / 2, RS);
-        hipLaunchKernelGGL((gn_fir_down_strip_kernel<RS>), dim3((unsigned)cdiv(tot3, 256)), dim3(256), 0, st, (const bf16_t*)x, ldx, scale,
-                           shift, C, (bf16_t*)y, ldy, (bf16_t*)xr, ldxr, B, H, W, act);
+        hipLaunchKernelGGL((gn_fir_down_strip_kernel<RS>), dim3((unsigned)cdiv(tot3, 256), By), dim3(256), 0, st, (const bf16_t*)x, ldx, scale,
+                           shift, C, (bf16_t*)y, ldy, (bf16_t*)xr, ldxr, B, H, W, act, g);
         ds_set_last_conv_kernel("gn_fir_down_strip_kernel<4>");
       }
       DS_LAUNCH_CHECK();
@@ -785,12 +880,12 @@
     if (nb2 > 16384) nb2 = 16384;
     if (nb2 < 1) nb2 = 1;
     if (mode == 1) {
-      hipLaunchKernelGGL((gn_resample2x2_kernel<T, 1>), dim3((unsigned)nb2), dim3(256), 0, st, (const T*)x, ldx, scale,
-                         shift, C, (T*)y, ldy, (T*)xr, ldxr, B, H, W, act);
+      hipLaunchKernelGGL((gn_resample2x2_kernel<T, 1>), dim3((unsigned)nb2, By), dim3(256), 0, st, (const T*)x, ldx, scale,
+                         shift, C, (T*)y, ldy, (T*)xr, ldxr, B, H, W, act, g);
       ds_set_last_conv_kernel(sizeof(T) == 4 ? "gn_resample2x2_kernel<f32,1>" : "gn_resample2x2_kernel<" DS_HALF_NAME ",1>");
     } else {
-      hipLaunchKernelGGL((gn_resample2x2_kernel<T, 2>), dim3((unsigned)nb2), dim3(256), 0, st, (const T*)x, ldx, scale,
-                         shift, C, (T*)y, ldy, (T*)xr, ldxr, B, H, W, act);
+      hipLaunchKernelGGL((gn_resample2x2_kernel<T, 2>), dim3((unsigned)nb2, By), dim3(256), 0, st, (const T*)x, ldx, scale,
+                         shift, C, (T*)y, ldy, (T*)xr, ldxr, B, H, W, act, g);
       ds_set_last_conv_kernel(sizeof(T) == 4 ? "gn_resample2x2_kernel<f32,2>" : "gn_resample2x2_kernel<" DS_HALF_NAME ",2>");
     }
     DS_LAUNCH_CHECK();
@@ -798,8 +893,8 @@
   }
 #define GA(M, A, N)                                                                                                  \
   do {                                                                                                               \
-    hipLaunchKernelGGL((gn_apply_kernel<T, M, A>), dim3((unsigned)nb), dim3(256), 0, st, (const T*)x, ldx, scale, shift, \
-                       C, (T*)y, ldy, (T*)xr, ldxr, B, H, W, act);                                                   \
+    hipLaunchKernelGGL((gn_apply_kernel<T, M, A>), dim3((unsigned)nb, By), dim3(256), 0, st, (const T*)x, ldx, scale, shift, \
+                       C, (T*)y, ldy, (T*)xr, ldxr, B, H, W, act, g);                                                \
     ds_set_last_conv_kernel("gn_apply_kernel<" #M "," N ">");                                                        \
   } while (0)
   if (mode == 0) { if (aff) GA(0, true, "affine"); else GA(0, false, "raw"); }
@@ -811,21 +906,27 @@
 }
 
 int ds_launch_gn_apply(const GnPlan& p, const void* x, int ldx, const float* scale, const float* shift, int C, void* y, int ldy,
-                       void* xr, int ldxr, int B, int H, int W, int act, int mode, int dtype, hipStream_t st) {
+                       void* xr, int ldxr, int B, int H, int W, int act, int mode, int dtype, hipStream_t st, const GnAccum* acc) {
+  if (acc && !acc->acc) acc = nullptr;
+  const bool aff = scale != nullptr || acc != nullptr;
   DS_CHECK(C % 8 == 0, "gn_apply: C must be a multiple of 8");
   DS_CHECK(mode >= 0 && mode <= 2, "gn_apply: bad resample mode");
   DS_CHECK(mode != 2 || (H % 2 == 0 && W % 2 == 0), "gn_apply: FIR down needs even H, W");
-  DS_CHECK(scale != nullptr || (mode != 0 && xr != nullptr), "gn_apply: nothing to do");
-  DS_CHECK(ds_gn_route_runs(p.route, mode, scale != nullptr, dtype, H, W, C, ldx, ldy, ldxr, xr != nullptr),
+  DS_CHECK(aff || (mode != 0 && xr != nullptr), "gn_apply: nothing to do");
+  DS_CHECK(!acc || scale == nullptr, "gn_apply: a table or accumulators, not both");
+  DS_CHECK(ds_gn_route_runs(p.route, mode, aff, dtype, H, W, C, ldx, ldy, ldxr, xr != nullptr),
            "gn_apply: the routed kernel cannot run this shape");
-  if (dtype == DS_F32) return gn_launch_typed<float>(p, x, ldx, scale, shift, C, y, ldy, xr, ldxr, B, H, W, act, mode, st);
-  return gn_launch_typed<bf16_t>(p, x, ldx, scale, shift, C, y, ldy, xr, ldxr, B, H, W, act, mode, st);
+  DS_CHECK(!acc || (ds_gn_route_takes_acc(p, mode, dtype, C, acc->groups) && B <= 65535),
+           "gn_apply: the routed kernel builds no table from accumulators for this launch");
+  if (dtype == DS_F32) return gn_launch_typed<float>(p, x, ldx, scale, shift, C, y, ldy, xr, ldxr, B, H, W, act, mode, st, acc);
+  return gn_launch_typed<bf16_t>(p, x, ldx, scale, shift, C, y, ldy, xr, ldxr, B, H, W, act, mode, st, acc);
 }
 
 int ds_launch_gn_apply(const void* x, int ldx, const float* scale, const float* shift, int C, void* y, int ldy,
-                       void* xr, int ldxr, int B, int H, int W, int act, int mode, int dtype, hipStream_t st) {
-  const GnPlan p = ds_gn_route(mode, scale != nullptr, dtype, B, H, W, C, ldx, ldy, ldxr, xr != nullptr,  0);
-  return ds_launch_gn_apply(p, x, ldx, scale, shift, C, y, ldy, xr, ldxr, B, H, W, act, mode, dtype, st);
+                       void* xr, int ldxr, int B, int H, int W, int act, int mode, int dtype, hipStream_t st, const GnAccum* acc) {
+  const bool aff = scale != nullptr || (acc && acc->acc);
+  const GnPlan p = ds_gn_route(mode, aff, dtype, B, H, W, C, ldx, ldy, ldxr, xr != nullptr,  0);
+  return ds_launch_gn_apply(p, x, ldx, scale, shift, C, y, ldy, xr, ldxr, B, H, W, act, mode, dtype, st, acc);
 }
 
 template <typename T>
diff --git a/diffusion-separation_amd/csrc/sampler.hip b/diffusion-separation_amd/csrc/sampler.hip
--- a/diffusion-separation_amd/csrc/sampler.hip
+++ b/diffusion-separation_amd/csrc/sampler.hip
@@ -94,6 +94,27 @@
     e->ts_dev = ts;
     e->ts_B = B;
   }
+  auto all_projections = [&](diffsep_engine* g) -> int {
+    if ((g->opts & DS_OPT_TEMB_PER_EVAL) || (g->proj_ts == ts && g->proj_B == B)) return 0;
+    const size_t rows = (size_t)N * B, need = rows * ((size_t)g->arch.dense_total + 10 * (size_t)g->cfg.nf) * 4;
+    g->proj_ts.clear();
+    if (need > g->proj_all_cap) {
+      DS_HIP(hipStreamSynchronize(st));
+      if (g->proj_all) { DS_HIP(hipFree(g->proj_all)); }
+      g->proj_all = nullptr;
+      g->proj_all_cap = 0;
+      DS_HIP(hipMalloc((void**)&g->proj_all, need));
+      g->proj_all_cap = need;
+    }
+    if (time_projection(g, e->st_ts, (int)rows, g->proj_all, g->proj_all + rows * g->arch.dense_total, st)) return 1;
+    g->proj_ts = ts;
+    g->proj_B = B;
+    return 0;
+  };
+  if (all_projections(e)) return 1;
+  if (tail && all_projections(tail)) return 1;
+  const bool once = !(e->opts & DS_OPT_TEMB_PER_EVAL), tail_once = tail && !(tail->opts & DS_OPT_TEMB_PER_EVAL);
+  const size_t nproj = (size_t)B * e->arch.dense_total;
   DS_HIP(hipMemcpyAsync(e->st_mix, mix_norm, (size_t)B * T * 4, hipMemcpyDeviceToDevice, st));
   const int* lens = nullptr;
   if (lengths || seeds) {
@@ -146,14 +167,16 @@
       }
       DS_HIP(hipMemcpyAsync(tail->st_x, e->st_x, nst * 4, hipMemcpyDeviceToDevice, st));
       DS_HIP(hipMemcpyAsync(tail->st_t, e->st_t, (size_t)B * 4, hipMemcpyDeviceToDevice, st));
+      if (tail_once) { DS_HIP(hipMemcpyAsync(tail->st_proj, tail->proj_all + (size_t)i * nproj, nproj * 4, hipMemcpyDeviceToDevice, st)); }
       score = tail->st_score;
-      return run_nfe(tail, B, T, st);
+      return run_nfe(tail, B, T, st, tail_once);
     }
     score = e->st_score;
-    return run_nfe(e, B, T, st);
+    return run_nfe(e, B, T, st, once);
   };
   for (int i = 0; i < N; ++i) {
     DS_HIP(hipMemcpyAsync(e->st_t, e->st_ts + (size_t)i * B, (size_t)B * 4, hipMemcpyDeviceToDevice, st));
+    if (once) { DS_HIP(hipMemcpyAsync(e->st_proj, e->proj_all + (size_t)i * nproj, nproj * 4, hipMemcpyDeviceToDevice, st)); }
     for (int k = 0; k < csteps; ++k) {
       if (eval_score(i)) return 1;
       if (next_noise(&z)) return 1;
diff --git a/diffusion-separation_amd/csrc/unit.hip b/diffusion-separation_amd/csrc/unit.hip
--- a/diffusion-separation_amd/csrc/unit.hip
+++ b/diffusion-separation_amd/csrc/unit.hip
@@ -77,6 +77,24 @@
            "16-bit, table, down, W % 4 == 0; row tiles: half-precision build, 16-bit, table, down, W % 32 == 0, C % 64 == 0, ld % 8 == 0; "
            "up tiles: table, up, C % 64 == 0)");
   return ds_launch_gn_apply(p, x, ldx, scale, shift, C, y, ldy, xr, ldxr, B, H, W, act, mode, dtype, st);
+}
+extern "C" int32_t diffsep_gn_apply_acc(const void* x, const int64_t* acc, const float* gamma, const float* beta, int32_t groups,
+                                        float eps, void* y, void* xr, int32_t B, int32_t H, int32_t W, int32_t C, int32_t ldx,
+                                        int32_t ldy, int32_t ldxr, int32_t act, int32_t mode, int32_t dtype, int32_t route,
+                                        void* stream) {
+  DS_CHECK(x && acc && y, "gn_apply_acc: null pointer");
+  DS_CHECK(mode == 1 || mode == 2, "gn_apply_acc: a resampling launch (mode 1 / 2)");
+  if (gn_unit_shape(B, H, W, C, ldx, ldy, ldxr, true, xr != nullptr, mode, dtype)) return 1;
+  DS_CHECK(groups > 0 && C % groups == 0, "gn_apply_acc: bad group count");
+  const GnAccum a = {(const long long*)acc, gamma, beta, groups, gn_inv_count((long)H * W, C, groups), eps};
+  hipStream_t st = (hipStream_t)stream;
+  if (route == DIFFSEP_GN_AUTO)
+    return ds_launch_gn_apply(x, ldx, nullptr, nullptr, C, y, ldy, xr, ldxr, B, H, W, act, mode, dtype, st, &a);
+  GnPlan p;
+  DS_CHECK(!gn_forced_plan(route, &p), "gn_apply_acc: unknown route code");
+  DS_CHECK(ds_gn_route_runs(p.route, mode, true, dtype, H, W, C, ldx, ldy, ldxr, xr != nullptr),
+           "gn_apply_acc: the forced kernel's shape preconditions do not hold");
+  return ds_launch_gn_apply(p, x, ldx, nullptr, nullptr, C, y, ldy, xr, ldxr, B, H, W, act, mode, dtype, st, &a);
 }
 extern "C" const char* diffsep_gn_route_name(int32_t mode, int32_t affine, int32_t dtype, int32_t B, int32_t H, int32_t W, int32_t C,
                                              int32_t ldx, int32_t ldy, int32_t ldxr, int32_t has_xr, int32_t cus) {
diff --git a/diffusion-separation_amd/diffsep_amd/_lib.py b/diffusion-separation_amd/diffsep_amd/_lib.py
--- a/diffusion-separation_amd/diffsep_amd/_lib.py
+++ b/diffusion-separation_amd/diffsep_amd/_lib.py
@@ -124,6 +124,8 @@
     "diffsep_last_conv_kernel": (C.c_char_p, []),
     "diffsep_gn_finalize_acc": (_I, [_P, _I, _P, _I, _I, _L, _I, _F, _P, _P, _P, _P, _P]),
     "diffsep_gn_apply": (_I, [_P, _P, _P, _P, _P, _I, _I, _I, _I, _I, _I, _I, _I, _I, _I, _I, _P]),
+    "diffsep_engine_time_projection": (_I, [_P, _P, _I, _P, _P, _L, _P]),
+    "diffsep_gn_apply_acc": (_I, [_P, _P, _P, _P, _I, _F, _P, _P, _I, _I, _I, _I, _I, _I, _I, _I, _I, _I, _I, _P]),
     "diffsep_gn_route_name": (C.c_char_p, [_I, _I, _I, _I, _I, _I, _I, _I, _I, _I, _I, _I]),
     "diffsep_conv3x3_streamed": (_I, [_P, _P, _I, _P, _P, _P, _P, _P, _P, _P, _I, _I, _P, _P, _I, _I, _I, _I, _I, _F, _I, _P, _P,
                                       _P, _P, _P, _P, _P, _I, _P]),
diff --git a/diffusion-separation_amd/diffsep_amd/engine.py b/diffusion-separation_amd/diffsep_amd/engine.py
--- a/diffusion-separation_amd/diffsep_amd/engine.py
+++ b/diffusion-separation_amd/diffsep_amd/engine.py
@@ -101,6 +101,14 @@
 
     def get_option(self, name):
         return int(self._L.diffsep_engine_get_option(self._h, str(name).encode()))
+
+    def time_projection(self, t):
+        rows, dense = t.numel(), self.get_option("dense_total")
+        out = torch.empty((rows, dense), dtype=torch.float32, device=t.device)
+        ws = torch.empty(rows * 10 * self.cfg.nf, dtype=torch.float32, device=t.device)
+        check(self._L.diffsep_engine_time_projection(self._h, _ptr(t), rows, _ptr(out), _ptr(ws), ws.numel() * 4,
+                                                     _stream_ptr(self.device)), self._L)
+        return out
 
     CONV_CLASSES = ("conv3x3_8x32xN64", "conv3x3_8x32xN32", "conv3x3_8x8xN64", "gemm1x1_256xN64", "gemm1x1_256xN32",
                     "gemm1x1_64xN64", "conv3x3_ws_64to64", "conv3x3_small_16couts", "conv3x3_rw_regweights", "attention_fused",
diff --git a/diffusion-separation_amd/diffsep_amd/ops.py b/diffusion-separation_amd/diffsep_amd/ops.py
--- a/diffusion-separation_amd/diffsep_amd/ops.py
+++ b/diffusion-separation_amd/diffsep_amd/ops.py
@@ -151,6 +151,16 @@
     check(_L(x).diffsep_gn_apply(_ptr(xb), _ptr(scale), _ptr(shift), _ptr(yb), _ptr(xrb), B, H, W, Cc, Cc + pad[0], Cc + pad[1],
                                  Cc + pad[2], int(act), resample, _dt(x), GN_ROUTES[route or "auto"], _stream_ptr()), _L(x))
     return (yb[..., :Cc] if want_y else None, xrb[..., :Cc] if want_xr else None, yb, xrb)
+
+
+def gn_apply_acc(x, acc, gamma, beta, groups, resample, act=1, want_xr=True, route=None, eps=1e-6):
+    B, H, W, Cc = x.shape
+    Ho, Wo = {1: (2 * H, 2 * W), 2: (H // 2, W // 2)}[resample]
+    y = torch.full((B, Ho, Wo, Cc), float("nan"), dtype=x.dtype, device=x.device)
+    xr = torch.full_like(y, float("nan")) if want_xr else None
+    check(_L(x).diffsep_gn_apply_acc(_ptr(x), _ptr(acc), _ptr(gamma), _ptr(beta), groups, eps, _ptr(y), _ptr(xr), B, H, W, Cc, Cc,
+                                     Cc, Cc, int(act), resample, _dt(x), GN_ROUTES[route or "auto"], _stream_ptr()), _L(x))
+    return y, xr
 
 
 def gn_route_name(kind, resample, affine, dtype, B, H, W, C, pad=(0, 0, 0), has_xr=True, cus=256):
diff --git a/include/diffsep_hip.h b/include/diffsep_hip.h
--- a/include/diffsep_hip.h
+++ b/include/diffsep_hip.h
@@ -199,6 +199,11 @@
 int32_t diffsep_gn_apply(const void* x, const float* scale, const float* shift, void* y, void* xr, int32_t B, int32_t H, int32_t W,
                          int32_t C, int32_t ldx, int32_t ldy, int32_t ldxr, int32_t act, int32_t mode, int32_t dtype, int32_t route,
                          void* stream);
+int32_t diffsep_engine_time_projection(diffsep_engine* e, const float* t, int32_t rows, float* proj, void* workspace,
+                                       int64_t workspace_bytes, void* stream);
+int32_t diffsep_gn_apply_acc(const void* x, const int64_t* acc, const float* gamma, const float* beta, int32_t groups, float eps,
+                             void* y, void* xr, int32_t B, int32_t H, int32_t W, int32_t C, int32_t ldx, int32_t ldy, int32_t ldxr,
+                             int32_t act, int32_t mode, int32_t dtype, int32_t route, void* stream);
 const char* diffsep_gn_route_name(int32_t mode, int32_t affine, int32_t dtype, int32_t B, int32_t H, int32_t W, int32_t C,
                                   int32_t ldx, int32_t ldy, int32_t ldxr, int32_t has_xr, int32_t cus);
 int32_t diffsep_conv3x3_streamed(const void* x, const void* x2, int32_t C1, const float* gn_scale, const float* gn_shift,
```

Result: no change. 77.45 utterances/s (median of 3 runs) (+0.2%).
